# jie0530/act-plus-plus

Hardware: AMD Instinct MI355X
Metric: policy steps/sec (4x480x640 cams, chunk=100, bs=8) (higher is better)
Workload: dtype f32 (f16x3 split products: 3 fp16 MFMAs per fp32 product, fp32 accumulate); 1 GPU; ACT eval policy query: 4 cams 480x640 u8, chunk 100, hidden 512, ff 3200, 4 enc + 7 dec layers (layer 0 live), per-GPU batch 8, + temporal ensemble; per_gpu_batch=8, global_batch=8, parallelism=replicas x1

## Files before the change

act-plus-plus_amd/actmi/lib.py:

```python
import ctypes as C
import os

import torch

_HERE = os.path.dirname(os.path.abspath(__file__))
LIB_PATH = os.environ.get("ACTMI_LIB") or os.path.join(_HERE, "libactmi.so")

IMG_U8_NHWC = 0
IMG_F32_NCHW = 1


class ActmiConfig(C.Structure):
    _fields_ = [("struct_size", C.c_uint32)] + [(n, C.c_int32) for n in (
        "num_cams", "image_h", "image_w", "base_width", "hidden_dim", "nheads", "dim_feedforward", "enc_layers",
        "dec_layers", "num_queries", "state_dim", "action_dim", "latent_dim", "has_cvae_encoder", "max_batch",
        "enable_training")] + [("kl_weight", C.c_float)] + [(n, C.c_int32) for n in ("vq", "vq_class", "vq_dim")]


class GemmDesc(C.Structure):
    _fields_ = [
        ("A", C.c_void_p), ("lda", C.c_int64), ("mode", C.c_int32),
        ("H", C.c_int32), ("W", C.c_int32), ("Cin", C.c_int32), ("KH", C.c_int32), ("KW", C.c_int32),
        ("stride", C.c_int32), ("pad", C.c_int32), ("Ho", C.c_int32), ("Wo", C.c_int32),
        ("img_stride", C.c_int64),
        ("A_add", C.c_void_p), ("ld_add", C.c_int64), ("add_mod", C.c_int32), ("add_ncols", C.c_int32),
        ("Bw", C.c_void_p), ("ldb", C.c_int64),
        ("scale", C.c_void_p), ("bias", C.c_void_p), ("res", C.c_void_p), ("ldres", C.c_int64),
        ("res_mod", C.c_int32), ("relu", C.c_int32),
        ("C", C.c_void_p), ("ldc", C.c_int64), ("rowmap", C.c_void_p),
        ("M", C.c_int32), ("N", C.c_int32), ("K", C.c_int32), ("groups", C.c_int32),
        ("gA", C.c_int64), ("gB", C.c_int64), ("gSB", C.c_int64), ("gC", C.c_int64), ("gRes", C.c_int64),
        ("ta", C.c_int32), ("tb", C.c_int32), ("a_rowmap", C.c_void_p),
        ("B_add", C.c_void_p), ("ld_badd", C.c_int64), ("badd_mod", C.c_int32), ("splitk", C.c_int32),
        ("mask", C.c_void_p), ("ldmask", C.c_int64), ("C2", C.c_void_p), ("scale2", C.c_void_p),
        ("alpha", C.c_float), ("groups_inner", C.c_int32),
        ("gA2", C.c_int64), ("gB2", C.c_int64), ("gC2", C.c_int64), ("gRes2", C.c_int64),
        ("gMask", C.c_int64), ("gC2out", C.c_int64),
        ("drop_p", C.c_float), ("drop_seed", C.c_uint64), ("stamps", C.c_void_p), ("prec", C.c_int32), ("b_split", C.c_int32), ("b_scale", C.c_float), ("a_scale", C.c_float), ("a_scale_dev", C.c_void_p), ("b_scale_dev", C.c_void_p),
        ("split_stride", C.c_int64), ("amax_out", C.c_void_p),
        ("epi", C.c_int32), ("epi_scale", C.c_float), ("epi_row", C.c_void_p), ("gRow", C.c_int64), ("gRow2", C.c_int64),
        ("epi_colkill", C.c_void_p), ("gColkill", C.c_int64), ("tile_hint", C.c_int32),
        ("finite_flag", C.c_void_p), ("finite_bit", C.c_uint32),
        ("Ax", C.c_void_p), ("kx_begin", C.c_int32), ("Hx", C.c_int32), ("Wx", C.c_int32), ("Cx", C.c_int32),
        ("stride_x", C.c_int32), ("gAx", C.c_int64),
        ("A_alt", C.c_void_p), ("alt_ncols", C.c_int32), ("k_tap_inner", C.c_int32),
    ]


class AttnBwdDesc(C.Structure):
    _fields_ = [("q", C.c_void_p), ("k", C.c_void_p), ("v", C.c_void_p), ("o", C.c_void_p), ("d_o", C.c_void_p), ("lse", C.c_void_p),
                ("dq", C.c_void_p), ("dk", C.c_void_p), ("dv", C.c_void_p)] + \
               [(n, C.c_int64) for n in ("q_bs", "q_rs", "k_bs", "k_rs", "v_bs", "v_rs", "dq_bs", "dq_rs", "dk_bs", "dk_rs", "dv_bs", "dv_rs")] + \
               [("kpm", C.c_void_p), ("kpm_bs", C.c_int64)] + [(n, C.c_int32) for n in ("B", "H", "Nq", "Nk", "HD")] + \
               [("drop_p", C.c_float), ("drop_seed", C.c_uint64), ("delta_ws", C.c_void_p), ("do_scale", C.c_void_p), ("amax_out", C.c_void_p)]


class AttnDesc(C.Structure):
    _fields_ = [
        ("Q", C.c_void_p), ("q_bs", C.c_int64), ("q_rs", C.c_int64),
        ("K", C.c_void_p), ("k_bs", C.c_int64), ("k_rs", C.c_int64),
        ("V", C.c_void_p), ("v_bs", C.c_int64), ("v_rs", C.c_int64),
        ("O", C.c_void_p), ("o_bs", C.c_int64), ("o_rs", C.c_int64),
        ("kpm", C.c_void_p), ("kpm_bs", C.c_int64), ("lse", C.c_void_p),
        ("B", C.c_int32), ("H", C.c_int32), ("Nq", C.c_int32), ("Nk", C.c_int32), ("HD", C.c_int32),
        ("scale", C.c_float), ("ws", C.c_void_p), ("ws_floats", C.c_int64),
        ("drop_p", C.c_float), ("drop_seed", C.c_uint64), ("prec", C.c_int32), ("causal", C.c_int32),
    ]


_lib = None


def load():
    global _lib
    if _lib is not None:
        return _lib
    if not os.path.isfile(LIB_PATH):
        raise RuntimeError(
            f"{LIB_PATH} is missing: build the HIP extension first (python -c 'import __graft_entry__ as g; g.build()' "
            "or make -C act-plus-plus_amd/csrc). There is no CPU fallback for the ACT path.")
    lib = C.CDLL(LIB_PATH)
    vp, i32, i64, f32, f64 = C.c_void_p, C.c_int32, C.c_int64, C.c_float, C.c_double
    sigs = {
        "actmi_version": ([], i32),
        "actmi_create": ([C.POINTER(ActmiConfig), C.POINTER(vp)], i32),
        "actmi_destroy": ([vp], i32),
        "actmi_last_error": ([vp], C.c_char_p),
        "actmi_num_params": ([vp], i32),
        "actmi_param_info": ([vp, i32, C.POINTER(C.c_char_p), C.POINTER(i64), C.POINTER(i32), C.POINTER(i32)], i32),
        "actmi_set_param": ([vp, C.c_char_p, vp, C.POINTER(i64), i32, i32], i32),
        "actmi_get_param": ([vp, C.c_char_p, vp, i64, i32], i32),
        "actmi_param_ptr": ([vp, C.c_char_p, C.POINTER(vp), C.POINTER(i64)], i32),
        "actmi_finalize": ([vp, vp], i32),
        "actmi_set_forward_phase": ([vp, i32], i32),
        "actmi_forward_infer_vq": ([vp, vp, vp, i32, i32, vp, vp, vp], i32),
        "actmi_forward_infer": ([vp, vp, vp, i32, i32, vp, vp], i32),
        "actmi_forward_train": ([vp, vp, vp, i32, vp, vp, vp, C.c_uint64, f32, i32, vp, vp, vp, vp, vp], i32),
        "actmi_backward": ([vp, f32, vp], i32),
        "actmi_zero_grad": ([vp, vp], i32),
        "actmi_adamw_step": ([vp, f32, f32, f32, f32, f32, f32, i64, vp], i32),
        "actmi_adamw_step_range": ([vp, f32, f32, f32, f32, f32, f32, i64, i64, i64, vp], i32),
        "actmi_refresh_weights": ([vp, vp], i32),
        "actmi_param_arena": ([vp, C.POINTER(vp), C.POINTER(i64)], i32),
        "actmi_grad_ptr": ([vp, C.c_char_p, C.POINTER(vp), C.POINTER(i64)], i32),
        "actmi_grad_arena": ([vp, C.POINTER(vp), C.POINTER(i64)], i32),
        "actmi_grad_phase_range": ([vp, i32, C.POINTER(i64), C.POINTER(i64)], i32),
        "actmi_wait_grad_phase": ([vp, i32, vp], i32),
        "actmi_ensemble_step": ([vp, vp, vp, f64, vp, vp, i32, i32, i32, vp], i32),
        "actmi_op_gemm": ([C.POINTER(GemmDesc), vp], i32),
        "actmi_op_split16": ([vp, vp, C.c_int64, C.c_float, vp], i32),
        "actmi_op_permute_conv_k": ([vp, vp, C.c_int64, i32, i32, i32, vp], i32),
        "actmi_op_sample_onehot": ([vp, i32, i32, C.c_float, C.c_uint64, vp, vp, vp], i32),
        "actmi_op_pow2_scale": ([vp, C.c_int64, i32, i32, vp, vp], i32),
        "actmi_op_splitk_combine": ([vp, i32, C.c_int64, C.c_int64, i32, i32, vp, vp, vp, C.c_int64, i32, vp, C.c_int64, vp], i32),
        "actmi_op_attention": ([C.POINTER(AttnDesc), vp], i32),
        "actmi_op_attention_bwd": ([C.POINTER(AttnBwdDesc), vp], i32),
        "actmi_op_layernorm": ([vp, vp, i32, vp, vp, vp, vp, vp, i32, i32, f32, vp], i32),
        "actmi_op_maxpool3x3s2": ([vp, vp, i32, i32, i32, i32, vp], i32),
        "actmi_op_conv1": ([vp, i32, vp, vp, vp, vp, vp, i32, i32, i32, i32, i32, i32, vp], i32),
        "actmi_op_conv1_workspace_floats": ([i32, i32], C.c_int64),
        "actmi_op_conv1_prepare": ([vp, vp, i32, i32, i32, vp], i32),
        "actmi_op_conv1_prepared": ([vp, vp, vp, vp, vp, i32, i32, i32, i32, i32, i32, vp], i32),
        "actmi_op_conv3x3_c64": ([vp, vp, C.c_float, vp, vp, vp, vp, i32, i32, i32, i32, i32, vp], i32),
        "actmi_op_wgrad7x7s2": ([vp, vp, vp, vp, C.c_int64, vp, i32, i32, i32, i32, vp], i32),
        "actmi_op_wgrad3x3_c64": ([vp, vp, vp, vp, C.c_int64, vp, i32, i32, i32, i32, vp], i32),
        "actmi_op_groupnorm": ([vp, vp, vp, vp, vp, vp, vp, i32, i32, i32, i32, f32, i32, i32, vp, C.c_int64, vp], i32),
        "actmi_op_spatial_softmax": ([vp, vp, i32, i32, i32, i32, f32, vp], i32),
        "actmi_op_unfold1d": ([vp, vp, i32, i32, i32, i32, i32, i32, i32, i32, vp], i32),
        "actmi_op_ddim_step": ([vp, vp, C.c_int64, f32, f32, f32, f32, i32, vp], i32),
        "actmi_op_mish": ([vp, vp, C.c_int64, vp], i32),
        "actmi_op_gelu": ([vp, vp, C.c_int64, vp], i32),
        "actmi_op_gelu_bwd": ([vp, vp, vp, C.c_int64, vp], i32),
        "actmi_op_dropout": ([vp, vp, C.c_int64, C.c_float, C.c_uint64, vp], i32),
        "actmi_op_small_attention": ([vp, vp, i32, i32, i32, i32, i32, C.c_float, C.c_uint64, vp], i32),
        "actmi_op_small_attention_bwd": ([vp, vp, vp, i32, i32, i32, i32, i32, C.c_float, C.c_uint64, vp], i32),
        "actmi_op_soft_ce_dim1": ([vp, vp, i32, i32, i32, vp, vp, vp, vp], i32),
        "actmi_op_argmax_l1": ([vp, vp, i32, i32, vp, vp, vp], i32),
        "actmi_op_layernorm_bwd": ([vp, vp, vp, vp, vp, vp, vp, i32, i32, C.c_float, vp, C.c_int64, vp], i32),
        "actmi_op_colsum": ([vp, C.c_int64, vp, i32, i32, vp, C.c_int64, vp], i32),
        "actmi_op_sum_batch": ([vp, C.c_int64, C.c_int64, vp, i32, i32, i32, i32, vp], i32),
        "actmi_op_adamw": ([vp, vp, vp, vp, C.c_int64, C.c_float, C.c_float, C.c_float, C.c_float, C.c_float, C.c_int64, vp], i32),
        "actmi_op_u8_to_nhwc4": ([vp, vp, i32, i32, i32, i32, vp], i32),
        "actmi_op_last_error": ([], C.c_char_p),
        "actmi_debug_tensor": ([vp, C.c_char_p, C.POINTER(vp), C.POINTER(i64)], i32),
        "actmi_debug_stop_after": ([vp, C.c_char_p], i32),
        "actmi_set_gemm_prec": ([vp, i32], i32),
        "actmi_set_train_prec": ([vp, i32], i32),
        "actmi_get_flags": ([vp, C.POINTER(C.c_uint32), i32, vp], i32),
        "actmi_flags_ptr": ([vp, C.POINTER(vp)], i32),
        "actmi_profile_enable": ([i32], i32),
        "actmi_profile_reset": ([], i32),
        "actmi_profile_report": ([C.c_char_p, i32], i32),
    }
    for name, (args, res) in sigs.items():
        fn = getattr(lib, name)
        fn.argtypes = args
        fn.restype = res
    _lib = lib
    return lib


def declared_symbols(header_path):
    import re
    txt = open(header_path).read()
    return sorted(set(re.findall(r"\b(actmi_[a-z0-9_]+)\s*\(", txt)))


def current_stream_ptr():
    return C.c_void_p(torch.cuda.current_stream().cuda_stream)


def check(rc, handle=None, what=""):
    if rc != 0:
        lib = load()
        msg = lib.actmi_last_error(handle) if handle is not None else lib.actmi_op_last_error()
        raise RuntimeError(f"libactmi {what} failed (code {rc}): {msg.decode() if msg else ''}")


def profile_enable(on: bool):
    lib = load()
    lib.actmi_profile_reset() if on else None
    lib.actmi_profile_enable(1 if on else 0)


def profile_report():
    import json
    lib = load()
    buf = C.create_string_buffer(1 << 18)
    rc = lib.actmi_profile_report(buf, len(buf))
    if rc != 0:
        raise RuntimeError(f"actmi_profile_report failed ({rc})")
    return json.loads(buf.value.decode())
```

act-plus-plus_amd/actmi/ops.py:

```python
import ctypes as C

import torch

from . import lib as L


def _p(t):
    return C.c_void_p(t.data_ptr()) if t is not None else C.c_void_p(0)


PREC = {None: 0, "f32": 1, "f16x3": 2, "bf16": 3}


def split16(w, scale=1.0):
    lib = L.load()
    w = w.contiguous()
    out = torch.empty_like(w)
    L.check(lib.actmi_op_split16(_p(w), _p(out), w.numel(), float(scale), L.current_stream_ptr()), None, "op_split16")
    return out


def permute_conv_k(w_rows, taps, cin):
    lib = L.load()
    w_rows = w_rows.contiguous()
    out = torch.empty_like(w_rows)
    rows, ld = w_rows.numel() // w_rows.shape[-1], w_rows.shape[-1]
    L.check(lib.actmi_op_permute_conv_k(_p(w_rows), _p(out), rows, int(taps), int(cin), int(ld), L.current_stream_ptr()), None,
            "op_permute_conv_k")
    return out


def pow2_scale(x):
    lib = L.load()
    assert x.dim() == 2 and x.stride(1) == 1
    out = torch.zeros(2, dtype=torch.float32, device=x.device)
    L.check(lib.actmi_op_pow2_scale(_p(x), x.stride(0), x.shape[0], x.shape[1], _p(out), L.current_stream_ptr()), None,
            "op_pow2_scale")
    return out


def auto_splitk(M, N, K):
    tiles = ((M + 63) // 64) * ((N + 63) // 64)
    nk = (K + 31) // 32
    if tiles >= 768 or nk < 24:
        return 0
    s = min(8, (1536 + tiles - 1) // tiles, nk // 12)
    while s >= 2 and (s - 1) * ((nk + s - 1) // s) >= nk:
        s -= 1
    return s if s >= 2 else 0


def gemm(A, W, bias=None, scale=None, res=None, res_mod=0, relu=False, a_add=None, add_mod=0, add_ncols=0, rowmap=None,
         out=None, out_rows=None, drop_p=0.0, drop_seed=0, prec=None, w_split=False, a_scale=0.0, b_scale=0.0,
         a_scale_dev=None, b_scale_dev=None, splitk=0):
    lib = L.load()
    M, K = A.shape
    N = W.shape[0]
    if splitk == "auto":
        splitk = auto_splitk(M, N, K) if (rowmap is None and not res_mod and not drop_p and N % 4 == 0 and a_scale_dev is None
                                          and b_scale_dev is None) else 0
    if splitk and splitk > 1:
        assert rowmap is None and not res_mod and not drop_p
        part = torch.empty((splitk, M, N), dtype=torch.float32, device=A.device)
        d = L.GemmDesc()
        d.A, d.lda, d.mode = A.data_ptr(), A.stride(0), 0
        if a_add is not None:
            d.A_add, d.ld_add, d.add_mod, d.add_ncols = a_add.data_ptr(), a_add.stride(0), add_mod, add_ncols
        d.Bw, d.ldb = W.data_ptr(), W.stride(0)
        d.C, d.ldc = part.data_ptr(), N
        d.M, d.N, d.K, d.groups = M, N, K, 1
        d.splitk, d.split_stride = int(splitk), M * N
        d.prec, d.b_split, d.b_scale = PREC[prec], 1 if w_split else 0, float(w_split) if w_split else float(b_scale)
        d.a_scale = float(a_scale)
        L.check(lib.actmi_op_gemm(C.byref(d), L.current_stream_ptr()), None, "op_gemm")
        if out is None:
            out = torch.empty((M, N), dtype=torch.float32, device=A.device)
        L.check(lib.actmi_op_splitk_combine(part.data_ptr(), int(splitk), M * N, N, M, N, _p(scale), _p(bias), _p(res),
                                            res.stride(0) if res is not None else 0,
                                            2 if relu == "gelu" else (1 if relu else 0), out.data_ptr(), out.stride(0),
                                            L.current_stream_ptr()), None, "op_splitk_combine")
        return out
    if out is None:
        out = torch.zeros((out_rows or M, N), dtype=torch.float32, device=A.device)
    d = L.GemmDesc()
    d.A, d.lda, d.mode = A.data_ptr(), A.stride(0), 0
    if a_add is not None:
        d.A_add, d.ld_add, d.add_mod, d.add_ncols = a_add.data_ptr(), a_add.stride(0), add_mod, add_ncols
    d.Bw, d.ldb = W.data_ptr(), W.stride(0)
    d.scale = scale.data_ptr() if scale is not None else None
    d.bias = bias.data_ptr() if bias is not None else None
    if res is not None:
        d.res, d.ldres, d.res_mod = res.data_ptr(), res.stride(0), res_mod
    d.relu = 2 if relu == "gelu" else (1 if relu else 0)
    d.C, d.ldc = out.data_ptr(), out.stride(0)
    d.rowmap = rowmap.data_ptr() if rowmap is not None else None
    d.M, d.N, d.K, d.groups = M, N, K, 1
    d.drop_p, d.drop_seed = float(drop_p), int(drop_seed)
    d.prec, d.b_split, d.b_scale = PREC[prec], 1 if w_split else 0, float(w_split) if w_split else float(b_scale)
    d.a_scale = float(a_scale)
    d.a_scale_dev = a_scale_dev.data_ptr() if a_scale_dev is not None else None
    d.b_scale_dev = b_scale_dev.data_ptr() if b_scale_dev is not None else None
    L.check(lib.actmi_op_gemm(C.byref(d), L.current_stream_ptr()), None, "op_gemm")
    return out


def conv2d_with_second_source(y1, x, wf_split, w_scale, bias, stride_x=2, relu=True, splitk=0, k_tap_inner=False):
    lib = L.load()
    G, B, H, W, Cc = y1.shape
    _, _, Hx, Wx, Cx = x.shape
    Cout = wf_split.shape[1]
    Kf = 9 * Cc + Cx
    assert wf_split.numel() == G * Cout * Kf
    M = B * H * W

    def desc(C_ptr, ldc, gC):
        d = L.GemmDesc()
        d.A, d.mode = y1.data_ptr(), 1
        d.H, d.W, d.Cin, d.KH, d.KW, d.stride, d.pad, d.Ho, d.Wo = H, W, Cc, 3, 3, 1, 1, H, W
        d.img_stride = H * W * Cc
        d.Ax, d.kx_begin, d.Hx, d.Wx, d.Cx, d.stride_x, d.gAx = x.data_ptr(), 9 * Cc, Hx, Wx, Cx, stride_x, B * Hx * Wx * Cx
        d.Bw, d.ldb = wf_split.data_ptr(), Kf
        d.C, d.ldc = C_ptr, ldc
        d.M, d.N, d.K, d.groups = M, Cout, Kf, G
        d.gA, d.gB, d.gSB, d.gC = B * H * W * Cc, Cout * Kf, Cout, gC
        d.prec, d.b_split, d.b_scale = PREC["f16x3"], 1, float(w_scale)
        d.k_tap_inner = 1 if k_tap_inner else 0
        return d
    out = torch.empty((G, B, H, W, Cout), dtype=torch.float32, device=y1.device)
    if splitk and splitk > 1:
        part = torch.empty((G, splitk, M, Cout), dtype=torch.float32, device=y1.device)
        d = desc(part.data_ptr(), Cout, splitk * M * Cout)
        d.splitk, d.split_stride = int(splitk), M * Cout
        L.check(lib.actmi_op_gemm(C.byref(d), L.current_stream_ptr()), None, "op_gemm(conv + second source, split)")
        for g in range(G):
            L.check(lib.actmi_op_splitk_combine(part[g].data_ptr(), int(splitk), M * Cout, Cout, M, Cout, None, _p(bias[g]), None, 0,
                                                1 if relu else 0, out[g].data_ptr(), Cout, L.current_stream_ptr()), None, "combine")
        return out
    d = desc(out.data_ptr(), Cout, M * Cout)
    d.bias = bias.data_ptr()
    d.relu = 1 if relu else 0
    L.check(lib.actmi_op_gemm(C.byref(d), L.current_stream_ptr()), None, "op_gemm(conv + second source)")
    return out


def conv2d_nhwc(x, w_ohwi, scale=None, bias=None, res=None, relu=False, stride=1, pad=1, prec=None, w_split=False, b_scale=0.0,
                k_tap_inner=False):
    lib = L.load()
    G, B, H, W, Cin = x.shape
    _, Cout, KH, KW, _ = w_ohwi.shape
    Ho, Wo = (H + 2 * pad - KH) // stride + 1, (W + 2 * pad - KW) // stride + 1
    out = torch.empty((G, B, Ho, Wo, Cout), dtype=torch.float32, device=x.device)
    d = L.GemmDesc()
    d.A, d.mode = x.data_ptr(), 1
    d.H, d.W, d.Cin, d.KH, d.KW, d.stride, d.pad, d.Ho, d.Wo = H, W, Cin, KH, KW, stride, pad, Ho, Wo
    d.img_stride = H * W * Cin
    d.Bw, d.ldb = w_ohwi.data_ptr(), KH * KW * Cin
    d.scale = scale.data_ptr() if scale is not None else None
    d.bias = bias.data_ptr() if bias is not None else None
    if res is not None:
        d.res, d.ldres = res.data_ptr(), Cout
    d.relu = 1 if relu else 0
    d.C, d.ldc = out.data_ptr(), Cout
    d.M, d.N, d.K, d.groups = B * Ho * Wo, Cout, KH * KW * Cin, G
    d.gA, d.gB, d.gSB = B * H * W * Cin, Cout * KH * KW * Cin, Cout
    d.gC = d.gRes = B * Ho * Wo * Cout
    d.prec, d.b_split, d.b_scale = PREC[prec], 1 if w_split else 0, float(w_split) if w_split else float(b_scale)
    d.k_tap_inner = 1 if k_tap_inner else 0
    L.check(lib.actmi_op_gemm(C.byref(d), L.current_stream_ptr()), None, "op_gemm(conv)")
    return out


def sample_onehot(logits, temperature=1.0, seed=0, want_probs=False):
    lib = L.load()
    logits = logits.contiguous()
    n, V = logits.shape
    code = torch.empty_like(logits)
    probs = torch.empty_like(logits) if want_probs else None
    L.check(lib.actmi_op_sample_onehot(_p(logits), n, V, float(temperature), C.c_uint64(int(seed)), _p(probs), _p(code),
                                       L.current_stream_ptr()), None, "op_sample_onehot")
    return (code, probs) if want_probs else code


def conv1_prepare(w_oihw, lut_mode=1):
    lib = L.load()
    w_oihw = w_oihw.contiguous()
    Cc, Cout = w_oihw.shape[0], w_oihw.shape[1]
    ws = torch.zeros(int(lib.actmi_op_conv1_workspace_floats(Cc, Cout)), dtype=torch.float32, device=w_oihw.device)
    L.check(lib.actmi_op_conv1_prepare(_p(w_oihw), _p(ws), Cc, Cout, int(lut_mode), L.current_stream_ptr()), None, "op_conv1_prepare")
    return ws


def conv1_prepared(image_u8, ws, Cout, relu=False, scale=None, bias=None):
    lib = L.load()
    image_u8 = image_u8.contiguous()
    B, Cc, H, W, _ = image_u8.shape
    out = torch.empty((Cc, B, (H - 1) // 2 + 1, (W - 1) // 2 + 1, Cout), dtype=torch.float32, device=image_u8.device)
    L.check(lib.actmi_op_conv1_prepared(_p(image_u8), _p(ws), _p(scale), _p(bias), _p(out), B, Cc, H, W, Cout, 1 if relu else 0,
                                        L.current_stream_ptr()), None, "op_conv1_prepared")
    return out


def conv3x3_c64(x, w_ohwi, scale=None, bias=None, res=None, relu=False, w_scale=256.0, w16=None):
    lib = L.load()
    G, B, H, W, Cin = x.shape
    assert Cin == 64 and tuple(w_ohwi.shape[1:]) == (64, 3, 3, 64)
    out = torch.empty_like(x)
    if w16 is None:
        w16 = split16(w_ohwi, w_scale)
    scale = scale if scale is not None else torch.ones(G, 64, device=x.device)
    bias = bias if bias is not None else torch.zeros(G, 64, device=x.device)
    L.check(lib.actmi_op_conv3x3_c64(_p(x.contiguous()), _p(w16), float(w_scale), _p(scale.contiguous()), _p(bias.contiguous()),
                                     _p(res), _p(out), G, B, H, W, 1 if relu else 0, L.current_stream_ptr()), None,
            "op_conv3x3_c64")
    return out


def wgrad3x3_c64(dy, x, dy_scale=None):
    G, B, H, W, Cc = x.shape
    assert Cc == 64 and dy.shape == x.shape
    nwg = max(1, min(256 // G, B * ((W + 31) // 32)))
    ws = torch.empty(G * nwg * 64 * 576, device=x.device, dtype=torch.float32)
    dw = torch.empty(G, 64, 3, 3, 64, device=x.device, dtype=torch.float32)
    lib = L.load()
    L.check(lib.actmi_op_wgrad3x3_c64(_p(dy.contiguous()), _p(x.contiguous()), _p(dw), _p(ws), ws.numel(),
                                      _p(dy_scale) if dy_scale is not None else None, G, B, H, W, L.current_stream_ptr()),
            None, "op_wgrad3x3_c64")
    return dw


def wgrad7x7s2(dy, x4, dy_scale=None):
    G, B, H, W, Cc = x4.shape
    Ho, Wo = (H - 1) // 2 + 1, (W - 1) // 2 + 1
    assert Cc == 4 and tuple(dy.shape) == (G, B, Ho, Wo, 64)
    nwg = max(1, min(512 // G, B * ((Wo + 31) // 32)))
    ws = torch.empty(G * nwg * 64 * 196, device=x4.device, dtype=torch.float32)
    dw = torch.empty(G, 64, 7, 7, 4, device=x4.device, dtype=torch.float32)
    lib = L.load()
    L.check(lib.actmi_op_wgrad7x7s2(_p(dy.contiguous()), _p(x4.contiguous()), _p(dw), _p(ws), ws.numel(),
                                    _p(dy_scale) if dy_scale is not None else None, G, B, H, W, L.current_stream_ptr()),
            None, "op_wgrad7x7s2")
    return dw



def attention(q, k, v, nheads, kpm=None, q_shared=False, want_lse=False, split=True, drop_p=0.0, drop_seed=0, prec=None,
              causal=False):
    lib = L.load()
    B, Nk, D = k.shape
    Nq = q.shape[-2]
    hd = D // nheads
    out = torch.zeros((B, Nq, D), dtype=torch.float32, device=k.device)
    lse = torch.zeros((B, nheads, Nq), dtype=torch.float32, device=k.device) if want_lse else None
    d = L.AttnDesc()
    d.Q, d.q_bs, d.q_rs = q.data_ptr(), (0 if q_shared else q.stride(0)), q.stride(-2)
    d.K, d.k_bs, d.k_rs = k.data_ptr(), k.stride(0), k.stride(1)
    d.V, d.v_bs, d.v_rs = v.data_ptr(), v.stride(0), v.stride(1)
    d.O, d.o_bs, d.o_rs = out.data_ptr(), out.stride(0), out.stride(1)
    if kpm is not None:
        d.kpm, d.kpm_bs = kpm.data_ptr(), kpm.stride(0)
    d.lse = lse.data_ptr() if lse is not None else None
    if split:
        ws = torch.empty(8 * B * Nq * (D + 2 * nheads), dtype=torch.float32, device=k.device)
        d.ws, d.ws_floats = ws.data_ptr(), ws.numel()
    d.B, d.H, d.Nq, d.Nk, d.HD = B, nheads, Nq, Nk, hd
    d.scale = 1.0 / (hd ** 0.5)
    d.drop_p, d.drop_seed = float(drop_p), int(drop_seed)
    d.prec = PREC[prec]
    d.causal = 1 if causal else 0
    L.check(lib.actmi_op_attention(C.byref(d), L.current_stream_ptr()), None, "op_attention")
    return (out, lse) if want_lse else out


def attention_bwd(q, k, v, out, lse, dout, nheads, kpm=None, drop_p=0.0, drop_seed=0, do_scale=None, want_amax=False):
    lib = L.load()
    B, Nk, D = k.shape
    Nq = q.shape[1]
    dq = torch.empty((B, Nq, D), dtype=torch.float32, device=k.device)
    dk = torch.empty((B, Nk, D), dtype=torch.float32, device=k.device)
    dv = torch.empty((B, Nk, D), dtype=torch.float32, device=k.device)
    ws = torch.empty(B * nheads * Nq, dtype=torch.float32, device=k.device)
    amax = torch.zeros(1, dtype=torch.int32, device=k.device) if want_amax else None
    d = L.AttnBwdDesc()
    d.q, d.q_bs, d.q_rs = q.data_ptr(), q.stride(0), q.stride(1)
    d.k, d.k_bs, d.k_rs = k.data_ptr(), k.stride(0), k.stride(1)
    d.v, d.v_bs, d.v_rs = v.data_ptr(), v.stride(0), v.stride(1)
    d.o, d.d_o, d.lse = out.data_ptr(), dout.data_ptr(), lse.data_ptr()
    d.dq, d.dq_bs, d.dq_rs = dq.data_ptr(), dq.stride(0), dq.stride(1)
    d.dk, d.dk_bs, d.dk_rs = dk.data_ptr(), dk.stride(0), dk.stride(1)
    d.dv, d.dv_bs, d.dv_rs = dv.data_ptr(), dv.stride(0), dv.stride(1)
    if kpm is not None:
        d.kpm, d.kpm_bs = kpm.data_ptr(), kpm.stride(0)
    d.B, d.H, d.Nq, d.Nk, d.HD = B, nheads, Nq, Nk, D // nheads
    d.drop_p, d.drop_seed = float(drop_p), int(drop_seed)
    d.delta_ws = ws.data_ptr()
    d.do_scale = do_scale.data_ptr() if do_scale is not None else None
    d.amax_out = amax.data_ptr() if amax is not None else None
    L.check(lib.actmi_op_attention_bwd(C.byref(d), L.current_stream_ptr()), None, "op_attention_bwd")
    return (dq, dk, dv, amax) if want_amax else (dq, dk, dv)


def layernorm(x, w, b, res=None, res_mod=0, w2=None, b2=None, eps=1e-5):
    lib = L.load()
    M, D = x.shape
    y = torch.empty_like(x)
    L.check(lib.actmi_op_layernorm(_p(x), _p(res), res_mod, _p(w), _p(b), _p(w2), _p(b2), _p(y), M, D, eps,
                                   L.current_stream_ptr()), None, "op_layernorm")
    return y


def maxpool3x3s2(x):
    lib = L.load()
    n, H, W, Cc = x.shape
    Ho, Wo = (H + 2 - 3) // 2 + 1, (W + 2 - 3) // 2 + 1
    y = torch.empty((n, Ho, Wo, Cc), dtype=torch.float32, device=x.device)
    L.check(lib.actmi_op_maxpool3x3s2(_p(x), _p(y), n, H, W, Cc, L.current_stream_ptr()), None, "op_maxpool")
    return y


def conv1(image, w_oihw, scale, bias, prec=None):
    lib = L.load()
    image = image.contiguous()
    if image.dtype == torch.uint8:
        B, Cn, H, W, _ = image.shape
        fmt = L.IMG_U8_NHWC
    else:
        B, Cn, _, H, W = image.shape
        fmt = L.IMG_F32_NCHW
    Cout = w_oihw.shape[1]
    Ho, Wo = (H + 6 - 7) // 2 + 1, (W + 6 - 7) // 2 + 1
    out = torch.zeros((Cn, B, Ho, Wo, Cout), dtype=torch.float32, device=image.device)
    ws = torch.empty(Cn * Cout * 148 + 768, dtype=torch.float32, device=image.device)
    L.check(lib.actmi_op_conv1(_p(image), fmt, _p(w_oihw), _p(scale), _p(bias), _p(out), _p(ws), B, Cn, H, W, Cout,
                               PREC[prec], L.current_stream_ptr()), None, "op_conv1")
    return out


ACT = {None: 0, "none": 0, "relu": 1, "mish": 2}


_GN_WS = {}


def groupnorm(x, weight, bias, groups, eps=1e-5, act=None, res=None, res_after=False, film=None, out=None):
    lib = L.load()
    x = x.contiguous()
    n, Cc = x.shape[0], x.shape[-1]
    P = x.numel() // (n * Cc)
    if out is None:
        out = torch.empty_like(x)
    assert out.is_contiguous() and out.shape == x.shape
    fs, fb = (film[0].contiguous(), film[1].contiguous()) if film is not None else (None, None)
    rm = 0 if res is None else (2 if res_after else 1)
    key = (x.device, torch.cuda.current_stream(x.device).cuda_stream)
    ws = _GN_WS.get(key)
    if ws is None:
        ws = _GN_WS[key] = torch.empty(1 << 20, dtype=torch.float32, device=x.device)
    L.check(lib.actmi_op_groupnorm(_p(x), _p(res.contiguous() if res is not None else None), _p(fs), _p(fb), _p(weight), _p(bias),
                                   _p(out), n, P, Cc, int(groups), float(eps), ACT[act], rm, _p(ws), ws.numel(),
                                   L.current_stream_ptr()), None, "op_groupnorm")
    return out


def spatial_softmax(logits, H, W, temperature=1.0):
    lib = L.load()
    logits = logits.contiguous()
    n, P, K = logits.shape
    assert P == H * W
    out = torch.empty((n, K, 2), dtype=torch.float32, device=logits.device)
    L.check(lib.actmi_op_spatial_softmax(_p(logits), _p(out), n, H, W, K, float(temperature), L.current_stream_ptr()), None,
            "op_spatial_softmax")
    return out


def unfold1d(x, k, stride=1, pad=0, transposed=False):
    lib = L.load()
    x = x.contiguous()
    B, T, Cc = x.shape
    To = (T - 1) * stride - 2 * pad + k if transposed else (T + 2 * pad - k) // stride + 1
    out = torch.empty((B, To, k * Cc), dtype=torch.float32, device=x.device)
    L.check(lib.actmi_op_unfold1d(_p(x), _p(out), B, T, Cc, k, stride, pad, To, 1 if transposed else 0, L.current_stream_ptr()),
            None, "op_unfold1d")
    return out


def ddim_step(x, eps, alpha_t, alpha_prev, clip=True):
    lib = L.load()
    assert x.is_contiguous() and eps.is_contiguous() and x.numel() == eps.numel()
    L.check(lib.actmi_op_ddim_step(_p(x), _p(eps), x.numel(), float(alpha_t ** -0.5), float((1.0 - alpha_t) ** 0.5),
                                   float(alpha_prev ** 0.5), float(max(0.0, 1.0 - alpha_prev) ** 0.5), 1 if clip else 0,
                                   L.current_stream_ptr()), None, "op_ddim_step")
    return x


def mish(x):
    lib = L.load()
    x = x.contiguous()
    y = torch.empty_like(x)
    L.check(lib.actmi_op_mish(_p(x), _p(y), x.numel(), L.current_stream_ptr()), None, "op_mish")
    return y


def u8_to_nhwc4(image_u8):
    lib = L.load()
    image_u8 = image_u8.contiguous()
    B, Cam, H, W, _ = image_u8.shape
    out = torch.empty((Cam, B, H, W, 4), dtype=torch.float32, device=image_u8.device)
    L.check(lib.actmi_op_u8_to_nhwc4(_p(image_u8), _p(out), B, Cam, H, W, L.current_stream_ptr()), None, "op_u8_to_nhwc4")
    return out


def gemm_t(A, Bm, ta=False, tb=False, bias=None, res=None, out=None, prec="f32"):
    lib = L.load()
    if ta:
        K, M = A.shape
    else:
        M, K = A.shape
    N = Bm.shape[1] if tb else Bm.shape[0]
    assert (Bm.shape[0] if tb else Bm.shape[1]) == K, (A.shape, Bm.shape, ta, tb)
    if out is None:
        out = torch.empty((M, N), dtype=torch.float32, device=A.device)
    d = L.GemmDesc()
    d.A, d.lda, d.mode, d.ta = A.data_ptr(), A.stride(0), 0, 1 if ta else 0
    d.Bw, d.ldb, d.tb = Bm.data_ptr(), Bm.stride(0), 1 if tb else 0
    d.bias = bias.data_ptr() if bias is not None else None
    if res is not None:
        d.res, d.ldres = res.data_ptr(), res.stride(0)
    d.C, d.ldc = out.data_ptr(), out.stride(0)
    d.M, d.N, d.K, d.groups = M, N, K, 1
    d.prec = PREC[prec]
    L.check(lib.actmi_op_gemm(C.byref(d), L.current_stream_ptr()), None, "op_gemm")
    return out


def gelu(x):
    y = torch.empty_like(x)
    L.check(L.load().actmi_op_gelu(_p(x), _p(y), x.numel(), L.current_stream_ptr()), None, "op_gelu")
    return y


def gelu_bwd(x, dy):
    dx = torch.empty_like(x)
    L.check(L.load().actmi_op_gelu_bwd(_p(x), _p(dy), _p(dx), x.numel(), L.current_stream_ptr()), None, "op_gelu_bwd")
    return dx


def dropout(x, p, seed):
    y = torch.empty_like(x)
    L.check(L.load().actmi_op_dropout(_p(x), _p(y), x.numel(), float(p), int(seed), L.current_stream_ptr()), None, "op_dropout")
    return y
# ... 87 lines not shown
```

act-plus-plus_amd/csrc/attn.hip:

```cpp
#include "common.h"
#include "dropout.h"
#include "split16.h"
#include <cstdio>
#include <cstdlib>

namespace {

constexpr bool ATTN_NOPF = true;
constexpr int KT = 64;
typedef _Float16 h16x8 __attribute__((ext_vector_type(8)));

__device__ __forceinline__ void attn_block_coords(int& bx, int& by, int& bz) {
    const int gx = gridDim.x, gy = gridDim.y;
    const int total = gx * gy * (int)gridDim.z;
    const int lin = ((int)blockIdx.z * gy + (int)blockIdx.y) * gx + (int)blockIdx.x;
    const int xcd = lin & 7, q = total >> 3, r = total & 7;
    const int base = (xcd < r) ? xcd * (q + 1) : r * (q + 1) + (xcd - r) * q;
    const int flat = base + (lin >> 3);
    bx = flat % gx;
    const int rest = flat / gx;
    by = rest % gy;
    bz = rest / gy;
}

template <int HD>
__global__ __launch_bounds__(256) void attn_f32_kernel(AttnArgs p, int nsplit, int chunk) {
    constexpr int HH = HD / 2;
    constexpr int DT = (HD + 31) / 32;
    constexpr int VD = DT * 32;
    constexpr int KS = HD + 4;
    __shared__ __attribute__((aligned(16))) float s_k[KT * KS];
    __shared__ __attribute__((aligned(16))) float s_v[KT * VD];

    const int t = threadIdx.x, lane = t & 63, wave = t >> 6;
    const int li = lane & 31, lh = lane >> 5;
    int bx, h, b;
    attn_block_coords(bx, h, b);
    const int split = bx % nsplit;
    const int q = (bx / nsplit) * 128 + wave * 32 + li;
    const int k_begin = split * chunk;
    const int k_end = (k_begin + chunk < p.Nk) ? k_begin + chunk : p.Nk;
    const bool qok = q < p.Nq;

    const float qscale = p.scale * 1.4426950408889634f;
    const float* Qp = p.Q + (int64_t)b * p.q_bs + (int64_t)(qok ? q : 0) * p.q_rs + h * HD + lh * HH;
    float qreg[HH];
#pragma unroll
    for (int s = 0; s < HH; s += 4) {
        f32x4 v = *reinterpret_cast<const f32x4*>(Qp + s);
#pragma unroll
        for (int j = 0; j < 4; ++j) qreg[s + j] = qok ? v[j] * qscale : 0.f;
    }
    const float* Kb = p.K + (int64_t)b * p.k_bs + h * HD;
    const float* Vb = p.V + (int64_t)b * p.v_bs + h * HD;
    const uint8_t* kpm = p.kpm ? p.kpm + (int64_t)b * p.kpm_bs : nullptr;

    f32x16 O[DT];
#pragma unroll
    for (int d = 0; d < DT; ++d)
#pragma unroll
        for (int e = 0; e < 16; ++e) O[d][e] = 0.f;
    float m_run = -INFINITY, l_run = 0.f;

    if (HD < VD) {
        for (int e = t; e < KT * VD; e += 256) s_v[e] = 0.f;
        __syncthreads();
    }

    __shared__ uint8_t s_dead[KT];
    constexpr int C4 = HD / 4;
    constexpr int NLD = (KT * C4 + 255) / 256;
    f32x4 pk[NLD], pv[NLD];
    auto fetch = [&](int kt0) {
#pragma unroll
        for (int i = 0; i < NLD; ++i) {
            const int e = t + 256 * i;
            const int kr = e / C4, c = e - kr * C4;
            const int key = kt0 + kr;
            const bool ok = e < KT * C4 && key < k_end;
            const int64_t koff = ok ? (int64_t)key * p.k_rs + c * 4 : 0;
            const int64_t voff = ok ? (int64_t)key * p.v_rs + c * 4 : 0;
            const f32x4 kv = *reinterpret_cast<const f32x4*>(Kb + koff);
            const f32x4 vv = *reinterpret_cast<const f32x4*>(Vb + voff);
            const f32x4 z = {0.f, 0.f, 0.f, 0.f};
            pk[i] = ok ? kv : z;
            pv[i] = ok ? vv : z;
        }
    };
    fetch(k_begin);
    for (int kt0 = k_begin; kt0 < k_end; kt0 += KT) {
#pragma unroll
        for (int i = 0; i < NLD; ++i) {
            const int e = t + 256 * i;
            if (e < KT * C4) {
                const int kr = e / C4, c = e - kr * C4;
                *reinterpret_cast<f32x4*>(&s_k[kr * KS + c * 4]) = pk[i];
                *reinterpret_cast<f32x4*>(&s_v[kr * VD + c * 4]) = pv[i];
            }
        }
        const bool ragged = kt0 + KT > k_end || kpm != nullptr;
        if (ragged && t < KT) {
            const int key = kt0 + t;
            s_dead[t] = (key >= k_end) || (kpm && kpm[key] != 0);
        }
        __syncthreads();
        if (kt0 + KT < k_end) fetch(kt0 + KT);
#pragma unroll
        for (int sub = 0; sub < KT / 32; ++sub) {
            const int kb = kt0 + sub * 32;
            if (kb < k_end) {
                f32x16 S;
#pragma unroll
                for (int e = 0; e < 16; ++e) S[e] = 0.f;
                const float* krow = &s_k[(sub * 32 + li) * KS + lh * HH];
#pragma unroll
                for (int s = 0; s < HH; s += 4) {
                    const f32x4 kv = *reinterpret_cast<const f32x4*>(krow + s);
#pragma unroll
                    for (int j = 0; j < 4; ++j)
                        S = __builtin_amdgcn_mfma_f32_32x32x2f32(kv[j], qreg[s + j], S, 0, 0, 0);
                }
                if (ragged) {
#pragma unroll
                    for (int e = 0; e < 16; ++e)
                        if (s_dead[sub * 32 + (e & 3) + 8 * (e >> 2) + 4 * lh]) S[e] = -INFINITY;
                }
                if (p.causal) {
#pragma unroll
                    for (int e = 0; e < 16; ++e)
                        if (kb + (e & 3) + 8 * (e >> 2) + 4 * lh > q) S[e] = -INFINITY;
                }
                float mt = S[0];
#pragma unroll
                for (int e = 1; e < 16; ++e) mt = fmaxf(mt, S[e]);
                mt = fmaxf(mt, __shfl_xor(mt, 32, 64));
                const float m_new = fmaxf(m_run, mt);
                const float m_safe = (m_new == -INFINITY) ? 0.f : m_new;
                const float alpha = __builtin_amdgcn_exp2f(m_run - m_safe);
                float rs = 0.f;
#pragma unroll
                for (int e = 0; e < 16; ++e) {
                    S[e] = __builtin_amdgcn_exp2f(S[e] - m_safe);
                    rs += S[e];
                }
                rs += __shfl_xor(rs, 32, 64);
                l_run = l_run * alpha + rs;
                m_run = m_new;
                if (p.drop_p > 0.f) {
                    const float ds = 1.f / (1.f - p.drop_p);
                    const uint64_t rowbase = (((uint64_t)b * p.H + h) * p.Nq + (qok ? q : 0)) * (uint64_t)p.Nk;
#pragma unroll
                    for (int e = 0; e < 16; ++e) {
                        const int key = kb + (e & 3) + 8 * (e >> 2) + 4 * lh;
                        S[e] = actmi_keep(p.drop_seed, rowbase + key, p.drop_p) ? S[e] * ds : 0.f;
                    }
                }
#pragma unroll
                for (int d = 0; d < DT; ++d)
#pragma unroll
                    for (int e = 0; e < 16; ++e) O[d][e] *= alpha;
#pragma unroll
                for (int e = 0; e < 16; ++e) {
                    const int kl = sub * 32 + (e & 3) + 8 * (e >> 2) + 4 * lh;
#pragma unroll
                    for (int d = 0; d < DT; ++d) {
                        const float vv = s_v[kl * VD + d * 32 + li];
                        O[d] = __builtin_amdgcn_mfma_f32_32x32x2f32(vv, S[e], O[d], 0, 0, 0);
                    }
                }
            }
        }
        __syncthreads();
    }
    if (qok) {
        if (nsplit == 1) {
            const float inv = 1.f / l_run;
            float* Op = p.O + (int64_t)b * p.o_bs + (int64_t)q * p.o_rs + h * HD;
#pragma unroll
            for (int d = 0; d < DT; ++d)
#pragma unroll
                for (int g = 0; g < 4; ++g) {
                    const int d0 = d * 32 + 8 * g + 4 * lh;
                    if (d0 < HD) {
                        f32x4 o = {O[d][4 * g] * inv, O[d][4 * g + 1] * inv, O[d][4 * g + 2] * inv, O[d][4 * g + 3] * inv};
                        *reinterpret_cast<f32x4*>(Op + d0) = o;
                    }
                }
            if (p.lse && lh == 0) p.lse[((int64_t)b * p.H + h) * p.Nq + q] = m_run * 0.6931471805599453f + logf(l_run);
        } else {
            const int64_t row = (((int64_t)split * p.B + b) * p.H + h) * p.Nq + q;
            float* Op = p.ws + row * HD;
            float* ml = p.ws + (int64_t)nsplit * p.B * p.H * p.Nq * HD + row * 2;
#pragma unroll
            for (int d = 0; d < DT; ++d)
#pragma unroll
                for (int g = 0; g < 4; ++g) {
                    const int d0 = d * 32 + 8 * g + 4 * lh;
                    if (d0 < HD) {
                        f32x4 o = {O[d][4 * g], O[d][4 * g + 1], O[d][4 * g + 2], O[d][4 * g + 3]};
                        *reinterpret_cast<f32x4*>(Op + d0) = o;
                    }
                }
            if (lh == 0) { ml[0] = m_run; ml[1] = l_run; }
        }
    }
}

template <int HD>
__global__ __launch_bounds__(256, 3) void attn_f16x3_kernel(AttnArgs p, int nsplit, int chunk) {
    constexpr int NS = HD / 16;
    constexpr int DT = (HD + 31) / 32;
    constexpr int VD = DT * 32;
    constexpr int KROW = 4 * HD + 16;
    constexpr int VROW = 4 * KT + 16;
    __shared__ __attribute__((aligned(16))) unsigned char s_k[KT * KROW];
    __shared__ __attribute__((aligned(16))) unsigned char s_vt[VD * VROW];
    __shared__ uint8_t s_dead[KT];

    const int t = threadIdx.x, lane = t & 63, wave = t >> 6;
    const int li = lane & 31, lh = lane >> 5;
    int bx, h, b;
    attn_block_coords(bx, h, b);
    const int split = bx % nsplit;
    const int q = (bx / nsplit) * 128 + wave * 32 + li;
    const int k_begin = split * chunk;
    const int k_end = (k_begin + chunk < p.Nk) ? k_begin + chunk : p.Nk;
    const bool qok = q < p.Nq;

    const float qscale = p.scale * 1.4426950408889634f;
    const float* Qp = p.Q + (int64_t)b * p.q_bs + (int64_t)(qok ? q : 0) * p.q_rs + h * HD + lh * 8;
    h16x8 qh[NS], ql[NS];
#pragma unroll
    for (int s = 0; s < NS; ++s) {
        f32x4 v0 = *reinterpret_cast<const f32x4*>(Qp + s * 16);
        f32x4 v1 = *reinterpret_cast<const f32x4*>(Qp + s * 16 + 4);
        const float sc = qok ? qscale : 0.f;
        v0 *= sc; v1 *= sc;
        uint2 h0, l0, h1, l1;
        split16(v0, h0, l0);
        split16(v1, h1, l1);
        qh[s] = __builtin_bit_cast(h16x8, uint4{h0.x, h0.y, h1.x, h1.y});
        ql[s] = __builtin_bit_cast(h16x8, uint4{l0.x, l0.y, l1.x, l1.y});
    }
    const float* Kb = p.K + (int64_t)b * p.k_bs + h * HD;
    const float* Vb = p.V + (int64_t)b * p.v_bs + h * HD;
    const uint8_t* kpm = p.kpm ? p.kpm + (int64_t)b * p.kpm_bs : nullptr;

    f32x16 O[DT];
#pragma unroll
    for (int d = 0; d < DT; ++d)
#pragma unroll
        for (int e = 0; e < 16; ++e) O[d][e] = 0.f;
    float m_run = -INFINITY, l_run = 0.f;

    if (HD < VD) {
        for (int e = t; e < VD * VROW / 4; e += 256) reinterpret_cast<uint32_t*>(s_vt)[e] = 0u;
        __syncthreads();
    }

    constexpr int C4 = HD / 4;
    constexpr int NLK = (KT * C4 + 255) / 256;
    constexpr int NLV = (KT / 2 * C4 + 255) / 256;
    f32x4 pk[NLK], pv[NLV][2];
    auto vc = [&](int e) { return ((e >> 5) % (C4 / 4)) * 4 + (e & 3); };
    auto vkp = [&](int e) { return ((e >> 5) / (C4 / 4)) * 8 + ((e >> 2) & 7); };
    auto fetch = [&](int kt0) {
        const f32x4 z = {0.f, 0.f, 0.f, 0.f};
#pragma unroll
        for (int i = 0; i < NLK; ++i) {
            const int e = t + 256 * i;
            const int kr = e / C4, c = e - kr * C4;
            const int key = kt0 + kr;
            const bool ok = e < KT * C4 && key < k_end;
            const f32x4 kv = *reinterpret_cast<const f32x4*>(Kb + (ok ? (int64_t)key * p.k_rs + c * 4 : 0));
            pk[i] = ok ? kv : z;
        }
#pragma unroll
        for (int i = 0; i < NLV; ++i) {
            const int e = t + 256 * i;
            const int kp = vkp(e), c = vc(e);
#pragma unroll
            for (int u = 0; u < 2; ++u) {
                const int key = kt0 + 2 * kp + u;
                const bool ok = e < KT / 2 * C4 && key < k_end;
                const f32x4 vv = *reinterpret_cast<const f32x4*>(Vb + (ok ? (int64_t)key * p.v_rs + c * 4 : 0));
                pv[i][u] = ok ? vv : z;
            }
        }
    };
    if (!ATTN_NOPF) fetch(k_begin);
    for (int kt0 = k_begin; kt0 < k_end; kt0 += KT) {
        if (ATTN_NOPF) fetch(kt0);
#pragma unroll
        for (int i = 0; i < NLK; ++i) {
            const int e = t + 256 * i;
            if (e < KT * C4) {
                const int kr = e / C4, c = e - kr * C4;
                uint2 hi, lo;
                split16(pk[i], hi, lo);
                *reinterpret_cast<uint2*>(s_k + kr * KROW + c * 8) = hi;
                *reinterpret_cast<uint2*>(s_k + kr * KROW + 2 * HD + c * 8) = lo;
            }
        }
#pragma unroll
        for (int i = 0; i < NLV; ++i) {
            const int e = t + 256 * i;
            if (e < KT / 2 * C4) {
                const int kp = vkp(e), c = vc(e);
                uint2 ha, la, hb, lb;
                split16(pv[i][0], ha, la);
                split16(pv[i][1], hb, lb);
                const int kl = 2 * kp, r = kl & 15;
                const int pos = (kl & ~15) | (r & 3) | ((r & 8) >> 1) | ((r & 4) << 1);
                unsigned char* dst = s_vt + (c * 4) * VROW + pos * 2;
                *reinterpret_cast<uint32_t*>(dst + 0 * VROW) = (ha.x & 0xffffu) | (hb.x << 16);
                *reinterpret_cast<uint32_t*>(dst + 1 * VROW) = (ha.x >> 16) | (hb.x & 0xffff0000u);
                *reinterpret_cast<uint32_t*>(dst + 2 * VROW) = (ha.y & 0xffffu) | (hb.y << 16);
                *reinterpret_cast<uint32_t*>(dst + 3 * VROW) = (ha.y >> 16) | (hb.y & 0xffff0000u);
                *reinterpret_cast<uint32_t*>(dst + 0 * VROW + 2 * KT) = (la.x & 0xffffu) | (lb.x << 16);
                *reinterpret_cast<uint32_t*>(dst + 1 * VROW + 2 * KT) = (la.x >> 16) | (lb.x & 0xffff0000u);
                *reinterpret_cast<uint32_t*>(dst + 2 * VROW + 2 * KT) = (la.y & 0xffffu) | (lb.y << 16);
                *reinterpret_cast<uint32_t*>(dst + 3 * VROW + 2 * KT) = (la.y >> 16) | (lb.y & 0xffff0000u);
            }
        }
        const bool ragged = kt0 + KT > k_end || kpm != nullptr;
        if (ragged && t < KT) {
            const int key = kt0 + t;
            s_dead[t] = (key >= k_end) || (kpm && kpm[key] != 0);
        }
        __syncthreads();
        if (!ATTN_NOPF && kt0 + KT < k_end) fetch(kt0 + KT);
#pragma unroll
        for (int sub = 0; sub < KT / 32; ++sub) {
            const int kb = kt0 + sub * 32;
            if (kb < k_end) {
                f32x16 S;
#pragma unroll
                for (int e = 0; e < 16; ++e) S[e] = 0.f;
                const unsigned char* krow = s_k + (sub * 32 + li) * KROW + lh * 16;
#pragma unroll
                for (int s = 0; s < NS; ++s) {
                    const h16x8 kh = __builtin_bit_cast(h16x8, *reinterpret_cast<const f32x4*>(krow + s * 32));
                    const h16x8 kl = __builtin_bit_cast(h16x8, *reinterpret_cast<const f32x4*>(krow + 2 * HD + s * 32));
                    S = __builtin_amdgcn_mfma_f32_32x32x16_f16(kl, qh[s], S, 0, 0, 0);
                    S = __builtin_amdgcn_mfma_f32_32x32x16_f16(kh, ql[s], S, 0, 0, 0);
                    S = __builtin_amdgcn_mfma_f32_32x32x16_f16(kh, qh[s], S, 0, 0, 0);
                }
                if (ragged) {
#pragma unroll
                    for (int e = 0; e < 16; ++e)
                        if (s_dead[sub * 32 + (e & 3) + 8 * (e >> 2) + 4 * lh]) S[e] = -INFINITY;
                }
                if (p.causal) {
#pragma unroll
                    for (int e = 0; e < 16; ++e)
                        if (kb + (e & 3) + 8 * (e >> 2) + 4 * lh > q) S[e] = -INFINITY;
                }
                float mt = S[0];
#pragma unroll
                for (int e = 1; e < 16; ++e) mt = fmaxf(mt, S[e]);
                mt = fmaxf(mt, __shfl_xor(mt, 32, 64));
                const float m_new = fmaxf(m_run, mt);
                const float m_safe = (m_new == -INFINITY) ? 0.f : m_new;
                const float alpha = __builtin_amdgcn_exp2f(m_run - m_safe);
                float rs = 0.f;
#pragma unroll
                for (int e = 0; e < 16; ++e) {
                    S[e] = __builtin_amdgcn_exp2f(S[e] - m_safe);
                    rs += S[e];
                }
                rs += __shfl_xor(rs, 32, 64);
                l_run = l_run * alpha + rs;
                m_run = m_new;
                if (p.drop_p > 0.f) {
                    const float ds = 1.f / (1.f - p.drop_p);
                    const uint64_t rowbase = (((uint64_t)b * p.H + h) * p.Nq + (qok ? q : 0)) * (uint64_t)p.Nk;
#pragma unroll
                    for (int e = 0; e < 16; ++e) {
                        const int key = kb + (e & 3) + 8 * (e >> 2) + 4 * lh;
                        S[e] = actmi_keep(p.drop_seed, rowbase + key, p.drop_p) ? S[e] * ds : 0.f;
                    }
                }
                h16x8 ph[2], pl[2];
#pragma unroll
                for (int g2 = 0; g2 < 2; ++g2) {
                    const f32x4 a0 = {S[8 * g2], S[8 * g2 + 1], S[8 * g2 + 2], S[8 * g2 + 3]};
                    const f32x4 a1 = {S[8 * g2 + 4], S[8 * g2 + 5], S[8 * g2 + 6], S[8 * g2 + 7]};
                    uint2 h0, l0, h1, l1;
                    split16(a0, h0, l0);
                    split16(a1, h1, l1);
                    ph[g2] = __builtin_bit_cast(h16x8, uint4{h0.x, h0.y, h1.x, h1.y});
                    pl[g2] = __builtin_bit_cast(h16x8, uint4{l0.x, l0.y, l1.x, l1.y});
                }
#pragma unroll
                for (int d = 0; d < DT; ++d) {
#pragma unroll
                    for (int e = 0; e < 16; ++e) O[d][e] *= alpha;
                    const unsigned char* vrow = s_vt + (d * 32 + li) * VROW + sub * 64 + lh * 16;
#pragma unroll
                    for (int g2 = 0; g2 < 2; ++g2) {
                        const h16x8 vh = __builtin_bit_cast(h16x8, *reinterpret_cast<const f32x4*>(vrow + g2 * 32));
                        const h16x8 vl = __builtin_bit_cast(h16x8, *reinterpret_cast<const f32x4*>(vrow + 2 * KT + g2 * 32));
                        O[d] = __builtin_amdgcn_mfma_f32_32x32x16_f16(vl, ph[g2], O[d], 0, 0, 0);
                        O[d] = __builtin_amdgcn_mfma_f32_32x32x16_f16(vh, pl[g2], O[d], 0, 0, 0);
                        O[d] = __builtin_amdgcn_mfma_f32_32x32x16_f16(vh, ph[g2], O[d], 0, 0, 0);
                    }
                }
            }
        }
        __syncthreads();
    }
    if (qok) {
        if (nsplit == 1) {
            const float inv = 1.f / l_run;
            float* Op = p.O + (int64_t)b * p.o_bs + (int64_t)q * p.o_rs + h * HD;
#pragma unroll
            for (int d = 0; d < DT; ++d)
#pragma unroll
                for (int g = 0; g < 4; ++g) {
                    const int d0 = d * 32 + 8 * g + 4 * lh;
                    if (d0 < HD) {
                        f32x4 o = {O[d][4 * g] * inv, O[d][4 * g + 1] * inv, O[d][4 * g + 2] * inv, O[d][4 * g + 3] * inv};
                        *reinterpret_cast<f32x4*>(Op + d0) = o;
                    }
                }
            if (p.lse && lh == 0) p.lse[((int64_t)b * p.H + h) * p.Nq + q] = m_run * 0.6931471805599453f + logf(l_run);
        } else {
            const int64_t row = (((int64_t)split * p.B + b) * p.H + h) * p.Nq + q;
            float* Op = p.ws + row * HD;
            float* ml = p.ws + (int64_t)nsplit * p.B * p.H * p.Nq * HD + row * 2;
#pragma unroll
            for (int d = 0; d < DT; ++d)
#pragma unroll
                for (int g = 0; g < 4; ++g) {
                    const int d0 = d * 32 + 8 * g + 4 * lh;
                    if (d0 < HD) {
                        f32x4 o = {O[d][4 * g], O[d][4 * g + 1], O[d][4 * g + 2], O[d][4 * g + 3]};
                        *reinterpret_cast<f32x4*>(Op + d0) = o;
                    }
                }
            if (lh == 0) { ml[0] = m_run; ml[1] = l_run; }
        }
    }
}


__global__ void attn_combine_kernel(AttnArgs p, int nsplit, int HD) {
    const int64_t idx = (int64_t)blockIdx.x * blockDim.x + threadIdx.x;
    const int D4 = HD / 4;
    const int64_t total = (int64_t)p.B * p.H * p.Nq * D4;
    if (idx >= total) return;
    const int d4 = (int)(idx % D4);
    const int64_t bhq = idx / D4;
    const int q = (int)(bhq % p.Nq);
    const int h = (int)((bhq / p.Nq) % p.H);
    const int b = (int)(bhq / ((int64_t)p.Nq * p.H));
    const int64_t per = (int64_t)p.B * p.H * p.Nq;
    const float* mlb = p.ws + (int64_t)nsplit * per * HD;
    float m = -INFINITY;
    for (int s = 0; s < nsplit; ++s) m = fmaxf(m, mlb[(s * per + bhq) * 2]);
    const float msafe = (m == -INFINITY) ? 0.f : m;
    float L = 0.f;
    f32x4 acc = {0.f, 0.f, 0.f, 0.f};
    for (int s = 0; s < nsplit; ++s) {
        const float w = __builtin_amdgcn_exp2f(mlb[(s * per + bhq) * 2] - msafe);
        L += mlb[(s * per + bhq) * 2 + 1] * w;
        acc += *reinterpret_cast<const f32x4*>(p.ws + (s * per + bhq) * HD + d4 * 4) * w;
    }
    const float inv = 1.f / L;
    *reinterpret_cast<f32x4*>(p.O + (int64_t)b * p.o_bs + (int64_t)q * p.o_rs + h * HD + d4 * 4) = acc * inv;
    if (p.lse && d4 == 0) p.lse[bhq] = msafe * 0.6931471805599453f + logf(L);
}

}

int launch_attention(const AttnArgs& a, hipStream_t st, std::string* err) {
    auto fail = [&](const char* m) { if (err) *err = std::string("attention: ") + m; return -2; };
    if (a.B <= 0 || a.Nq <= 0) return 0;
    if (a.Nk <= 0) return fail("Nk must be positive");
    if (a.causal && a.Nq != a.Nk) return fail("causal needs Nq == Nk");
    if ((a.q_rs & 3) || (a.k_rs & 3) || (a.v_rs & 3) || (a.o_rs & 3) || (a.q_bs & 3) || (a.k_bs & 3) || (a.v_bs & 3) ||
        (a.o_bs & 3))
        return fail("strides must be multiples of 4 floats");
    if (((uintptr_t)a.Q & 15) || ((uintptr_t)a.K & 15) || ((uintptr_t)a.V & 15) || ((uintptr_t)a.O & 15))
        return fail("pointers must be 16-byte aligned");
    static const int env_prec = env_gemm_prec(ACTMI_PREC_F32);
    const int prec = a.prec ? a.prec : env_prec;
    if (prec != ACTMI_PREC_F32 && prec != ACTMI_PREC_F16X3) return fail("bad prec");
    const bool f16 = prec == ACTMI_PREC_F16X3;
    const int qblocks = (a.Nq + 127) / 128;
    const int tiles = (a.Nk + KT - 1) / KT;
    int nsplit = 1;
    if (a.ws) {
        const long blocks = (long)qblocks * a.H * a.B;
        static const long target = getenv("ACTMI_ATTN_SPLIT_TARGET") ? atol(getenv("ACTMI_ATTN_SPLIT_TARGET")) : 1024;
        nsplit = (int)((target + blocks - 1) / blocks);
        if (nsplit < 1) nsplit = 1;
        if (nsplit > 8) nsplit = 8;
        if (nsplit > tiles / 2) nsplit = tiles / 2 > 0 ? tiles / 2 : 1;
        while (nsplit > 1 && (int64_t)nsplit * a.B * a.Nq * ((int64_t)a.H * a.HD + 2 * a.H) > a.ws_floats) --nsplit;
    }
    const int chunk = ((tiles + nsplit - 1) / nsplit) * KT;
    dim3 grid(qblocks * nsplit, a.H, a.B);
    if (prof_enabled()) {
        char nm[48];
        snprintf(nm, sizeof(nm), "attn_%s_kernel<%d>", f16 ? "f16x3" : "f32", a.HD);
        prof_begin(nm, 4.0 * a.B * a.H * (double)a.Nq * a.Nk * a.HD,
                   4.0 * a.B * a.H * a.HD * (2.0 * a.Nq + 2.0 * a.Nk), st);
    }
    if (f16) {
        switch (a.HD) {
            case 64: hipLaunchKernelGGL(attn_f16x3_kernel<64>, grid, dim3(256), 0, st, a, nsplit, chunk); break;
            case 32: hipLaunchKernelGGL(attn_f16x3_kernel<32>, grid, dim3(256), 0, st, a, nsplit, chunk); break;
            case 16: hipLaunchKernelGGL(attn_f16x3_kernel<16>, grid, dim3(256), 0, st, a, nsplit, chunk); break;
            default: return fail("head_dim must be 16, 32 or 64");
        }
    } else
    switch (a.HD) {
        case 64: hipLaunchKernelGGL(attn_f32_kernel<64>, grid, dim3(256), 0, st, a, nsplit, chunk); break;
        case 32: hipLaunchKernelGGL(attn_f32_kernel<32>, grid, dim3(256), 0, st, a, nsplit, chunk); break;
        case 16: hipLaunchKernelGGL(attn_f32_kernel<16>, grid, dim3(256), 0, st, a, nsplit, chunk); break;
        default: return fail("head_dim must be 16, 32 or 64");
    }
    if (nsplit > 1) {
        const int64_t total = (int64_t)a.B * a.H * a.Nq * (a.HD / 4);
        hipLaunchKernelGGL(attn_combine_kernel, dim3((unsigned)((total + 255) / 256)), dim3(256), 0, st, a, nsplit, a.HD);
    }
    prof_end(st);
    hipError_t e = hipGetLastError();
    if (e != hipSuccess) { if (err) *err = std::string("attention launch: ") + hipGetErrorString(e); return -3; }
    return 0;
}
```

act-plus-plus_amd/csrc/capi.hip:

```cpp
#include "engine.h"

#include <cstring>
#include <vector>

namespace {
thread_local std::string g_op_error;
inline hipStream_t S(void* s) { return reinterpret_cast<hipStream_t>(s); }
int bad(actmi_ctx* h, const std::string& m, int code = ACTMI_E_INVALID) { h->err = m; return code; }
struct DevGuard {
    int prev = -1, want;
    explicit DevGuard(int dev) : want(dev) {
        if (hipGetDevice(&prev) != hipSuccess) prev = -1;
        if (prev != want) (void)hipSetDevice(want);
    }
    ~DevGuard() { if (prev >= 0 && prev != want) (void)hipSetDevice(prev); }
};
#define ENTER(h) (h)->err.clear(); DevGuard _dev_guard((h)->device)
}

extern "C" {

int actmi_version(void) { return ACTMI_VERSION; }

int actmi_create(const actmi_config* cfg, actmi_handle* out) {
// ... 96 lines not shown
    if (!h->cfg.vq) return bad(h, "handle was not created with vq = 1");
    return engine_forward_infer(h, qpos, image, image_fmt, B, a_hat, S(stream), vq_sample);
}

int actmi_forward_train(actmi_handle h, const float* qpos, const void* image, int image_fmt, const float* actions,
                        const uint8_t* is_pad, const float* eps, uint64_t dropout_seed, float dropout_p, int B, float* losses,
                        float* a_hat, float* mu, float* logvar, void* stream) {
    if (!h) return ACTMI_E_INVALID;
    ENTER(h);
    if (!qpos || !image || !actions || !is_pad) return bad(h, "null pointer");
    return train_forward(h, qpos, image, image_fmt, actions, is_pad, eps, dropout_seed, dropout_p, B, losses, a_hat, mu, logvar,
                         S(stream));
}
int actmi_backward(actmi_handle h, float loss_scale, void* stream) {
    if (!h) return ACTMI_E_INVALID;
    ENTER(h);
    return train_backward(h, loss_scale, S(stream));
}
int actmi_zero_grad(actmi_handle h, void* stream) {
    if (!h) return ACTMI_E_INVALID;
    ENTER(h);
    return train_zero_grad(h, S(stream));
}
int actmi_adamw_step(actmi_handle h, float lr, float lr_backbone, float weight_decay, float beta1, float beta2, float eps,
                     int64_t step, void* stream) {
    if (!h) return ACTMI_E_INVALID;
    ENTER(h);
    return train_adamw_step(h, lr, lr_backbone, weight_decay, beta1, beta2, eps, step, S(stream));
}
int actmi_adamw_step_range(actmi_handle h, float lr, float lr_backbone, float weight_decay, float beta1, float beta2, float eps,
                           int64_t step, int64_t offset, int64_t count, void* stream) {
    if (!h) return ACTMI_E_INVALID;
    ENTER(h);
    return train_adamw_range(h, lr, lr_backbone, weight_decay, beta1, beta2, eps, step, offset, count, S(stream));
}
int actmi_refresh_weights(actmi_handle h, void* stream) {
    if (!h) return ACTMI_E_INVALID;
    ENTER(h);
    if (!h->finalized) return bad(h, "refresh_weights before finalize", ACTMI_E_STATE);
    return engine_prepare_weights(h, S(stream), true);
}
int actmi_param_arena(actmi_handle h, void** dev_ptr, int64_t* nfloats) {
    if (!h) return ACTMI_E_INVALID;
    if (dev_ptr) *dev_ptr = h->pbase;
    if (nfloats) *nfloats = h->ptotal;
    return 0;
}
int actmi_grad_ptr(actmi_handle h, const char* key, void** dev_ptr, int64_t* numel) {
    if (!h || !key) return ACTMI_E_INVALID;
    ENTER(h);
    if (!h->train) return bad(h, "handle was created without enable_training", ACTMI_E_STATE);
    auto it = h->index.find(key);
    if (it == h->index.end()) return bad(h, std::string("unknown state_dict key: ") + key);
    const Param& p = h->params[it->second];
    if (dev_ptr) *dev_ptr = h->train->gbase + p.off;
    if (numel) *numel = p.numel;
    return 0;
}

int actmi_grad_arena(actmi_handle h, void** dev_ptr, int64_t* nfloats) {
    if (!h) return ACTMI_E_INVALID;
    ENTER(h);
    if (!h->train) return bad(h, "handle was created without enable_training", ACTMI_E_STATE);
    if (dev_ptr) *dev_ptr = h->train->gbase;
    if (nfloats) *nfloats = h->ptotal;
    return 0;
}

int actmi_grad_phase_range(actmi_handle h, int phase, int64_t* offset, int64_t* count) {
    if (!h || !offset || !count || (phase != 1 && phase != 2)) return ACTMI_E_INVALID;
    ENTER(h);
    if (!h->train) return bad(h, "handle was created without enable_training", ACTMI_E_STATE);
    int64_t split = h->ptotal;
    for (const Param& p : h->params)
        if (p.key != "pos_table" && p.key.rfind("transformer.", 0) != 0) { split = p.off; break; }
    *offset = phase == 1 ? 0 : split;
    *count = phase == 1 ? split : h->ptotal - split;
    return 0;
}

int actmi_wait_grad_phase(actmi_handle h, int phase, void* stream) {
    if (!h || phase != 1) return ACTMI_E_INVALID;
    ENTER(h);
    if (!h->train || !h->train->ev_phase1) return bad(h, "handle was created without enable_training", ACTMI_E_STATE);
    hipError_t e = hipStreamWaitEvent(S(stream), h->train->ev_phase1, 0);
    if (e != hipSuccess) return bad(h, std::string("hipStreamWaitEvent: ") + hipGetErrorString(e), ACTMI_E_LAUNCH);
    return 0;
}

int actmi_ensemble_step(float* ring, int32_t* tcount, const float* chunk, double k, double* out, uint8_t* populated, int E,
                        int Q, int A, void* stream) {
    if (!ring || !tcount || !chunk || !out || Q < 1 || A < 1 || A > 64) return ACTMI_E_INVALID;
    return launch_ensemble(ring, tcount, chunk, k, out, populated, E, Q, A, S(stream));
}

int actmi_op_gemm(const actmi_gemm_desc* d, void* stream) {
    if (!d) return ACTMI_E_INVALID;
    g_op_error.clear();
    return launch_gemm(*d, S(stream), &g_op_error);
}

int actmi_op_split16(const float* src, float* dst, int64_t nfloats, float scale, void* stream) {
    g_op_error.clear();
    const int rc = launch_split16(src, dst, nfloats, scale, S(stream));
    if (rc != 0) g_op_error = "split16: nfloats must be a multiple of 4 and both pointers 16-byte aligned";
    return rc == 0 ? 0 : ACTMI_E_INVALID;
}

int actmi_op_permute_conv_k(const float* src, float* dst, int64_t rows, int taps, int cin, int ld, void* stream) {
    g_op_error.clear();
    const int rc = launch_permute_conv_k(src, dst, rows, taps, cin, ld, S(stream));
    if (rc != 0) g_op_error = "permute_conv_k: cin must be a multiple of 32, ld >= taps*cin, src != dst";
    return rc == 0 ? 0 : (rc == -2 ? ACTMI_E_INVALID : ACTMI_E_LAUNCH);
}




int actmi_op_pow2_scale(const float* x, int64_t ld, int M, int N, float* out, void* stream) {
    g_op_error.clear();
    return launch_pow2_scale(x, ld, M, N, out, S(stream)) == 0 ? 0 : ACTMI_E_LAUNCH;
}

int actmi_op_splitk_combine(const float* part, int nsplit, int64_t split_stride, int64_t ldp, int M, int N, const float* scale,
                            const float* bias, const float* res, int64_t ldres, int relu, float* out, int64_t ldc, void* stream) {
    g_op_error.clear();
    if (!part || !out || nsplit < 1 || M < 0 || N < 0 || ldp < N || ldc < N || (res && ldres < N) || relu < 0 || relu > 2) {
        g_op_error = "splitk_combine: bad argument";
        return ACTMI_E_INVALID;
    }
    SplitCombineArgs c{};
    c.part = part; c.nsplit = nsplit; c.split_stride = split_stride; c.ldp = ldp;
    c.scale = scale; c.bias = bias; c.res = res; c.ldres = ldres; c.relu = relu;
    c.C = out; c.ldc = ldc; c.M = M; c.N = N; c.groups = 1;
    return launch_splitk_combine(c, S(stream)) == 0 ? 0 : ACTMI_E_LAUNCH;
}

int actmi_op_sample_onehot(const float* logits, int n, int V, float temperature, uint64_t seed, float* probs, float* code,
                           void* stream) {
    g_op_error.clear();
    if (!logits || !code || n < 1 || V < 1 || !(temperature > 0.f)) { g_op_error = "sample_onehot: bad argument"; return ACTMI_E_INVALID; }
    return launch_vq_code(logits, nullptr, seed, probs, code, n, 1, V, S(stream), temperature) == 0 ? 0 : ACTMI_E_LAUNCH;
}

int actmi_op_attention(const actmi_attn_desc* d, void* stream) {
    if (!d) return ACTMI_E_INVALID;
    g_op_error.clear();
    return launch_attention(*d, S(stream), &g_op_error);
}

int actmi_op_attention_bwd(const actmi_attn_bwd_desc* d, void* stream) {
    g_op_error.clear();
    if (!d || !d->o || !d->delta_ws) { g_op_error = "attention_bwd: null descriptor / output / scratch"; return ACTMI_E_INVALID; }
    AttnBwdArgs a{};
    a.Q = d->q; a.K = d->k; a.V = d->v; a.dO = d->d_o; a.lse = d->lse; a.dO_scale = d->do_scale;
    a.dQ = d->dq; a.dK = d->dk; a.dV = d->dv;
    a.q_bs = d->q_bs; a.q_rs = d->q_rs; a.k_bs = d->k_bs; a.k_rs = d->k_rs; a.v_bs = d->v_bs; a.v_rs = d->v_rs;
    a.dq_bs = d->dq_bs; a.dq_rs = d->dq_rs; a.dk_bs = d->dk_bs; a.dk_rs = d->dk_rs; a.dv_bs = d->dv_bs; a.dv_rs = d->dv_rs;
    a.kpm = d->kpm; a.kpm_bs = d->kpm_bs;
    a.B = d->B; a.H = d->H; a.Nq = d->Nq; a.Nk = d->Nk; a.HD = d->HD;
    a.drop_p = d->drop_p; a.drop_seed = d->drop_seed; a.amax_out = d->amax_out;
    const int rc = launch_attention_bwd_dense(a, d->o, d->delta_ws, S(stream), &g_op_error);
    return rc == 0 ? ACTMI_OK : (rc == -2 ? ACTMI_E_SHAPE : ACTMI_E_LAUNCH);
}

int actmi_op_layernorm(const float* x, const float* res, int res_mod, const float* w, const float* b, const float* w2,
                       const float* b2, float* y, int M, int D, float eps, void* stream) {
    g_op_error.clear();
    return launch_layernorm(x, res, res_mod, w, b, w2, b2, y, M, D, eps, S(stream), &g_op_error);
}

int actmi_op_maxpool3x3s2(const float* in, float* out, int nimg, int H, int W, int C, void* stream) {
    return launch_maxpool(in, out, nimg, H, W, C, (H + 2 - 3) / 2 + 1, (W + 2 - 3) / 2 + 1, S(stream));
}

int actmi_op_conv1(const void* image, int image_fmt, const float* w_oihw, const float* scale, const float* bias,
                   float* out, float* workspace, int B, int C, int H, int W, int Cout, int prec, void* stream) {
    g_op_error.clear();
    float* wp = workspace;
    float* lut = workspace + (int64_t)C * Cout * 148;
    int rc = launch_repack_conv_w(w_oihw, wp, C, Cout, 3, 7, 7, (int64_t)Cout * 147, (int64_t)Cout * 148, 148, S(stream));
    if (rc) return rc;
    float hl[768];
    u8_lut(hl, true);
    if (hipMemcpyAsync(lut, hl, sizeof(hl), hipMemcpyHostToDevice, S(stream)) != hipSuccess) return ACTMI_E_LAUNCH;
    if (hipStreamSynchronize(S(stream)) != hipSuccess) return ACTMI_E_LAUNCH;
    Conv1Args a;
    a.image = image; a.fmt = image_fmt; a.lut = lut; a.w = wp; a.scale = scale; a.bias = bias; a.out = out;
    a.B = B; a.C = C; a.H = H; a.W = W; a.Ho = (H + 6 - 7) / 2 + 1; a.Wo = (W + 6 - 7) / 2 + 1; a.Cout = Cout;
    a.prec = prec;
    return launch_conv1(a, S(stream), &g_op_error);
}

static int64_t conv1_ws_off_lut(int C, int Cout) { return (int64_t)C * Cout * 148; }
int64_t actmi_op_conv1_workspace_floats(int C, int Cout) {
    return conv1_ws_off_lut(C, Cout) + 768 + 2 * (int64_t)C * Cout + (int64_t)C * ((conv1_wimg_bytes() + 3) / 4) + 16;
}
int actmi_op_conv1_prepare(const float* w_oihw, float* workspace, int C, int Cout, int lut_mode, void* stream) {
    g_op_error.clear();
    if (!w_oihw || !workspace || C < 1 || Cout < 1 || Cout > 64) { g_op_error = "conv1_prepare: bad argument"; return ACTMI_E_INVALID; }
    float* lut = workspace + conv1_ws_off_lut(C, Cout);
    float* ones = lut + 768;
    float* zeros = ones + (int64_t)C * Cout;
    float* wimg = zeros + (int64_t)C * Cout;
    wimg = reinterpret_cast<float*>((reinterpret_cast<uintptr_t>(wimg) + 15) & ~(uintptr_t)15);
    int rc = launch_repack_conv_w(w_oihw, workspace, C, Cout, 3, 7, 7, (int64_t)Cout * 147, (int64_t)Cout * 148, 148, S(stream));
    if (rc) return ACTMI_E_LAUNCH;
    std::vector<float> host(768 + 2 * (size_t)C * Cout);
    u8_lut(host.data(), lut_mode == 0);
    for (int i = 0; i < C * Cout; ++i) { host[768 + i] = 1.f; host[768 + C * Cout + i] = 0.f; }
    if (hipMemcpyAsync(lut, host.data(), host.size() * sizeof(float), hipMemcpyHostToDevice, S(stream)) != hipSuccess) return ACTMI_E_LAUNCH;
    rc = launch_conv1_wimg(workspace, wimg, C, Cout, S(stream), 256.f);
    if (rc) return ACTMI_E_LAUNCH;
    if (hipStreamSynchronize(S(stream)) != hipSuccess) return ACTMI_E_LAUNCH;
    return 0;
}
int actmi_op_conv1_prepared(const void* image_u8, const float* workspace, const float* scale, const float* bias, float* out, int B,
                            int C, int H, int W, int Cout, int relu, void* stream) {
    g_op_error.clear();
    if (!image_u8 || !workspace || !out) { g_op_error = "conv1_prepared: null pointer"; return ACTMI_E_INVALID; }
    const float* lut = workspace + conv1_ws_off_lut(C, Cout);
    const float* ones = lut + 768;
    const float* zeros = ones + (int64_t)C * Cout;
    const float* wimg = zeros + (int64_t)C * Cout;
    wimg = reinterpret_cast<const float*>((reinterpret_cast<uintptr_t>(wimg) + 15) & ~(uintptr_t)15);
    Conv1Args a;
    a.image = image_u8; a.fmt = ACTMI_IMG_U8_NHWC; a.lut = lut; a.w = workspace; a.scale = scale ? scale : ones; a.bias = bias ? bias : zeros;
    a.out = out; a.B = B; a.C = C; a.H = H; a.W = W; a.Ho = (H + 6 - 7) / 2 + 1; a.Wo = (W + 6 - 7) / 2 + 1; a.Cout = Cout;
    a.prec = ACTMI_PREC_F16X3; a.wimg = reinterpret_cast<const unsigned char*>(wimg); a.wscale = 256.f;
    a.relu_floor = relu ? 0.f : -__builtin_inff();
    return launch_conv1(a, S(stream), &g_op_error);
}

int actmi_op_conv3x3_c64(const float* x, const float* w16, float w_scale, const float* scale, const float* bias,
                         const float* res, float* out, int G, int B, int H, int W, int relu, void* stream) {
    g_op_error.clear();
    Conv3Args a;
    a.x = x; a.w16 = w16; a.scale = scale; a.bias = bias; a.res = res; a.out = out;
    a.G = G; a.B = B; a.H = H; a.W = W; a.relu = relu; a.w_scale = w_scale;
    return launch_conv3x3_c64(a, S(stream), &g_op_error);
}


int actmi_op_wgrad3x3_c64(const float* dy, const float* x, float* dw, float* ws, int64_t ws_floats, const float* dy_scale_dev, int G,
                          int B, int H, int W, void* stream) {
    g_op_error.clear();
    const int rc = launch_wgrad3x3_c64(dy, x, dw, 0, ws, ws_floats, dy_scale_dev, G, B, H, W, S(stream));
    if (rc != 0) { g_op_error = "wgrad3x3_c64: bad arguments or launch failure"; return rc == -2 ? ACTMI_E_INVALID : ACTMI_E_LAUNCH; }
    return 0;
}

int actmi_op_wgrad7x7s2(const float* dy, const float* x4, float* dw, float* ws, int64_t ws_floats, const float* dy_scale_dev, int G,
                        int B, int H, int W, void* stream) {
    g_op_error.clear();
    const int Ho = (H - 1) / 2 + 1, Wo = (W - 1) / 2 + 1;
    const int rc = launch_wgrad7x7s2(dy, x4, dw, 0, ws, ws_floats, dy_scale_dev, G, B, H, W, Ho, Wo, S(stream));
    if (rc != 0) { g_op_error = "wgrad7x7s2: bad arguments or launch failure"; return rc == -2 ? ACTMI_E_INVALID : ACTMI_E_LAUNCH; }
    return 0;
}

const char* actmi_op_last_error(void) { return g_op_error.c_str(); }

int actmi_set_gemm_prec(actmi_handle h, int prec) {
    if (!h) return ACTMI_E_INVALID;
    ENTER(h);
    if (prec != ACTMI_PREC_F32 && prec != ACTMI_PREC_F16X3) { h->err = "prec must be ACTMI_PREC_F32 or ACTMI_PREC_F16X3"; return ACTMI_E_INVALID; }
    h->gemm_prec = prec;
    h->finalized = false;
    return 0;
}

int actmi_set_train_prec(actmi_handle h, int prec) {
    if (!h) return ACTMI_E_INVALID;
    ENTER(h);
    if (prec != 0 && prec != ACTMI_PREC_BF16 && prec != ACTMI_PREC_F16X3 && prec != ACTMI_PREC_F32) { h->err = "train prec must be 0 or ACTMI_PREC_*"; return ACTMI_E_INVALID; }
    h->train_prec = (prec == h->gemm_prec) ? 0 : prec;
    if (h->train_prec != 0 && h->train_prec != ACTMI_PREC_BF16) { h->err = "only ACTMI_PREC_BF16 differs from the handle precision"; h->train_prec = 0; return ACTMI_E_INVALID; }
    return 0;
}

int actmi_get_flags(actmi_handle h, uint32_t* host_flags, int clear, void* stream) {
    if (!h || !host_flags) return ACTMI_E_INVALID;
    ENTER(h);
    hipError_t e = hipMemcpyAsync(host_flags, h->flags, sizeof(uint32_t), hipMemcpyDeviceToHost, S(stream));
    if (e == hipSuccess) e = hipStreamSynchronize(S(stream));
    if (e == hipSuccess && clear && *host_flags) e = hipMemsetAsync(h->flags, 0, sizeof(uint32_t), S(stream));
    if (e != hipSuccess) return bad(h, std::string("get_flags: ") + hipGetErrorString(e), ACTMI_E_LAUNCH);
    return 0;
}

int actmi_flags_ptr(actmi_handle h, void** dev_ptr) {
    if (!h || !dev_ptr) return ACTMI_E_INVALID;
    *dev_ptr = h->flags;
    return 0;
}

int actmi_debug_stop_after(actmi_handle h, const char* stage) {
    if (!h) return ACTMI_E_INVALID;
    h->stop_stage = stage ? stage : "";
    return 0;
}

int actmi_debug_tensor(actmi_handle h, const char* name, const float** dev_ptr, int64_t* numel) {
    if (!h || !name) return ACTMI_E_INVALID;
    ENTER(h);
    auto it = h->dbg.find(name);
// ... 66 lines not shown
```

act-plus-plus_amd/csrc/engine.hip:

```cpp
#include "engine.h"

#include <algorithm>
#include <cmath>
#include <cstdio>
#include <cstring>

namespace {

thread_local std::string g_create_error;

int conv_out(int x, int k, int s, int p) { return (x + 2 * p - k) / s + 1; }

void add_param(actmi_ctx* c, const std::string& key, std::vector<int64_t> shape, bool is_buffer) {
    Param p;
    p.key = key;
    p.shape = shape;
    p.numel = 1;
    for (auto d : shape) p.numel *= d;
    p.off = c->ptotal;
    p.is_buffer = is_buffer;
    c->ptotal += (p.numel + 63) & ~int64_t(63);
    c->index[key] = (int)c->params.size();
    c->params.push_back(p);
}

void add_mha(actmi_ctx* c, const std::string& p, int D) {
    add_param(c, p + "in_proj_weight", {3 * D, D}, false);
    add_param(c, p + "in_proj_bias", {3 * D}, false);
    add_param(c, p + "out_proj.weight", {D, D}, false);
    add_param(c, p + "out_proj.bias", {D}, false);
}

void add_ffn_norms(actmi_ctx* c, const std::string& p, int D, int F, int nnorm) {
    add_param(c, p + "linear1.weight", {F, D}, false);
    add_param(c, p + "linear1.bias", {F}, false);
    add_param(c, p + "linear2.weight", {D, F}, false);
    add_param(c, p + "linear2.bias", {D}, false);
    for (int i = 1; i <= nnorm; ++i) {
        add_param(c, p + "norm" + std::to_string(i) + ".weight", {D}, false);
        add_param(c, p + "norm" + std::to_string(i) + ".bias", {D}, false);
    }
}

void add_fbn(actmi_ctx* c, const std::string& p, int n) {
    for (const char* s : {"weight", "bias", "running_mean", "running_var"}) add_param(c, p + s, {n}, true);
}

void build_spec(actmi_ctx* c) {
    const actmi_config& g = c->cfg;
    const int D = g.hidden_dim, F = g.dim_feedforward, Q = g.num_queries, S = g.state_dim, A = g.action_dim,
              L = g.latent_dim, w0 = g.base_width;
    add_param(c, "pos_table", {1, Q + 2, D}, true);
    for (int i = 0; i < g.enc_layers; ++i) {
        std::string p = "transformer.encoder.layers." + std::to_string(i) + ".";
        add_mha(c, p + "self_attn.", D);
        add_ffn_norms(c, p, D, F, 2);
    }
    for (int i = 0; i < g.dec_layers; ++i) {
        std::string p = "transformer.decoder.layers." + std::to_string(i) + ".";
        add_mha(c, p + "self_attn.", D);
        add_mha(c, p + "multihead_attn.", D);
        add_ffn_norms(c, p, D, F, 3);
    }
    add_param(c, "transformer.decoder.norm.weight", {D}, false);
    add_param(c, "transformer.decoder.norm.bias", {D}, false);
    if (g.has_cvae_encoder) {
        for (int i = 0; i < g.enc_layers; ++i) {
            std::string p = "encoder.layers." + std::to_string(i) + ".";
            add_mha(c, p + "self_attn.", D);
            add_ffn_norms(c, p, D, F, 2);
        }
    }
    add_param(c, "action_head.weight", {A, D}, false);
    add_param(c, "action_head.bias", {A}, false);
    add_param(c, "is_pad_head.weight", {1, D}, false);
    add_param(c, "is_pad_head.bias", {1}, false);
    add_param(c, "query_embed.weight", {Q, D}, false);
    add_param(c, "input_proj.weight", {D, 8 * w0, 1, 1}, false);
    add_param(c, "input_proj.bias", {D}, false);
    for (int cam = 0; cam < g.num_cams; ++cam) {
        std::string p = "backbones." + std::to_string(cam) + ".0.body.";
        add_param(c, p + "conv1.weight", {w0, 3, 7, 7}, false);
        add_fbn(c, p + "bn1.", w0);
        int cin = w0;
        for (int li = 1; li <= 4; ++li) {
            const int cout = w0 << (li - 1);
            for (int bi = 0; bi < 2; ++bi) {
                std::string bp = p + "layer" + std::to_string(li) + "." + std::to_string(bi) + ".";
                add_param(c, bp + "conv1.weight", {cout, cin, 3, 3}, false);
                add_fbn(c, bp + "bn1.", cout);
                add_param(c, bp + "conv2.weight", {cout, cout, 3, 3}, false);
                add_fbn(c, bp + "bn2.", cout);
                if (bi == 0 && li > 1) {
                    add_param(c, bp + "downsample.0.weight", {cout, cin, 1, 1}, false);
                    add_fbn(c, bp + "downsample.1.", cout);
                }
                cin = cout;
            }
        }
    }
    add_param(c, "input_proj_robot_state.weight", {D, S}, false);
    add_param(c, "input_proj_robot_state.bias", {D}, false);
    add_param(c, "cls_embed.weight", {1, D}, false);
    add_param(c, "encoder_action_proj.weight", {D, A}, false);
    add_param(c, "encoder_action_proj.bias", {D}, false);
    add_param(c, "encoder_joint_proj.weight", {D, S}, false);
    add_param(c, "encoder_joint_proj.bias", {D}, false);
    const int Lp = g.vq ? g.vq_class * g.vq_dim : 2 * L, Li = g.vq ? g.vq_class * g.vq_dim : L;
    add_param(c, "latent_proj.weight", {Lp, D}, false);
    add_param(c, "latent_proj.bias", {Lp}, false);
    add_param(c, "latent_out_proj.weight", {D, Li}, false);
    add_param(c, "latent_out_proj.bias", {D}, false);
    add_param(c, "additional_pos_embed.weight", {2, D}, false);
}

}

int dev_alloc(actmi_ctx* ctx, float** p, int64_t nfloats) {
    void* q = nullptr;
    hipError_t e = hipMalloc(&q, (size_t)(nfloats > 0 ? nfloats : 1) * sizeof(float));
    if (e != hipSuccess) {
        ctx->err = std::string("hipMalloc: ") + hipGetErrorString(e);
        return ACTMI_E_NOMEM;
    }
    ctx->allocs.push_back(q);
    *p = reinterpret_cast<float*>(q);
    return 0;
}

int ctx_gemm(actmi_ctx* ctx, GemmArgs a, hipStream_t st, int ws_half, LnFuse* ln) {
    if (ln) ln->done = false;
    a.prec = ctx->prec_override ? ctx->prec_override : ctx->gemm_prec;
    const int64_t ws_part = (ctx->splitk_ws_floats / ctx->nbranch) & ~(int64_t)3;
    float* const ws = ctx->splitk_ws ? ctx->splitk_ws + (ws_half > 0 ? ws_half * ws_part : 0) : nullptr;
    const int64_t ws_floats = ws_half >= 0 ? ws_part : ctx->splitk_ws_floats;
    if (a.prec == ACTMI_PREC_F16X3 && a.tb == 0) {
        if (a.Bw >= ctx->pbase && a.Bw < ctx->pbase + ctx->ptotal) {
            a.b_scale = engine_weight_scale(ctx, a.Bw);
            a.Bw = ctx->p16base + (a.Bw - ctx->pbase);
            a.b_split = 1;
        } else {
            for (const ConvLayer& cl : ctx->convs) {
                if (a.Bw >= cl.w && a.Bw < cl.w + (int64_t)ctx->cfg.num_cams * cl.cout * cl.K) {
                    a.Bw = cl.w16 + (a.Bw - cl.w); a.b_split = 1; a.b_scale = cl.w16_scale; a.k_tap_inner = cl.k_tap_inner ? 1 : 0; break;
                }
                if (cl.wf && a.Bw >= cl.wf && a.Bw < cl.wf + (int64_t)ctx->cfg.num_cams * cl.cout * (cl.K + cl.Kx)) {
                    a.Bw = cl.wf16 + (a.Bw - cl.wf); a.b_split = 1; a.b_scale = cl.wf16_scale; a.k_tap_inner = cl.k_tap_inner ? 1 : 0; break;
                }
            }
        }
    }
    constexpr int sk_target = 1536, sk_minnk = 12, sk_maxtiles = 768;
    constexpr int sk_target_long = 4864, sk_maxtiles_long = 1300, sk_long_nk = 128;
    if (ctx->fwd_splitk && ctx->splitk_ws && a.splitk <= 1 && a.tb == 0 && a.ta == 0 && (a.mode == 0 || a.mode == 1) &&
        !a.rowmap && !a.C2 && !a.mask && a.drop_p == 0.f && a.res_mod == 0 && a.groups_inner == 0 && !a.stamps) {
        const int groups = a.groups > 0 ? a.groups : 1;
        const int64_t tiles = (int64_t)((a.M + 63) / 64) * ((a.N + 63) / 64) * groups * (ws_half >= 0 ? ctx->policy_mult : 1);
        const int nk = (a.K + 31) / 32;
        int S = tiles < sk_maxtiles ? (int)((sk_target + tiles - 1) / tiles) : 1;
        if (S == 1 && tiles < sk_maxtiles_long && nk >= sk_long_nk) S = (int)((sk_target_long + tiles - 1) / tiles);
        if (ln && S == 1 && ctx->ln_split > 1 && nk >= 64 && tiles < 2 * sk_maxtiles) S = ctx->ln_split;
        if (S > 8) S = 8;
        if (S > nk / sk_minnk) S = nk / sk_minnk;
        while (S >= 2 && (S - 1) * ((nk + S - 1) / S) >= nk) --S;
        if (S >= 2 && (int64_t)a.M * a.N * groups * S <= ws_floats && (a.N & 3) == 0) return gemm_slices(ctx, a, S, ws, st, ln);
    }
    return launch_gemm(a, st, &ctx->err);
}

int gemm_slices(actmi_ctx* ctx, const GemmArgs& a, int S, float* ws, hipStream_t st, LnFuse* ln) {
    const int groups = a.groups > 0 ? a.groups : 1;
    const int64_t slice = (int64_t)a.M * a.N;
    GemmArgs p = a;
    p.scale = p.bias = p.res = nullptr;
    p.relu = 0;
    p.C = ws;
    p.ldc = a.N;
    p.gC = slice * S;
    p.splitk = S;
    p.split_stride = slice;
    int rc = launch_gemm(p, st, &ctx->err);
    if (rc) return rc;
    if (ln && groups == 1 && !a.scale && !a.relu && (!a.res || a.ldres == a.N)) {
        rc = launch_layernorm(ws, a.res, 0, ln->w, ln->b, ln->w2, ln->b2, ln->out, a.M, a.N, ln->eps, st, &ctx->err, S, slice,
                              a.bias, ln->extra);
        ln->done = rc == 0;
        return rc;
    }
    SplitCombineArgs c{};
    c.part = ws; c.nsplit = S; c.split_stride = slice; c.gP = slice * S; c.ldp = a.N;
    c.scale = a.scale; c.bias = a.bias; c.gSB = a.gSB;
    c.res = a.res; c.ldres = a.ldres; c.gRes = a.gRes;
    c.relu = a.relu;
    c.C = a.C; c.ldc = a.ldc; c.gC = a.gC;
    c.M = a.M; c.N = a.N; c.groups = groups;
    rc = launch_splitk_combine(c, st);
    if (rc) ctx->err = "splitk combine launch failed";
    return rc;
}

float engine_weight_scale(const actmi_ctx* ctx, const float* w) {
    const int64_t off = w - ctx->pbase;
    size_t lo = 0, hi = ctx->params.size();
    while (hi - lo > 1) {
        const size_t mid = (lo + hi) / 2;
        if (ctx->params[mid].off <= off) lo = mid; else hi = mid;
    }
    return lo < ctx->pscale.size() ? ctx->pscale[lo] : W16_SCALE;
}

int engine_calibrate_weight_scales(actmi_ctx* ctx, hipStream_t st) {
    const int np = (int)ctx->params.size();
    ctx->pscale.assign(np, W16_SCALE);
    if (ctx->gemm_prec != ACTMI_PREC_F16X3) return 0;
    CHK(launch_seg_amax(ctx->pbase, ctx->poff_dev, ctx->pnumel_dev, np, ctx->pamax_dev, st));
    std::vector<unsigned> bits(np);
    HIPCHK(hipMemcpyAsync(bits.data(), ctx->pamax_dev, np * sizeof(unsigned), hipMemcpyDeviceToHost, st));
    HIPCHK(hipStreamSynchronize(st));
    float gmax = 0.f;
    for (int i = 0; i < np; ++i) {
        float amax;
        memcpy(&amax, &bits[i], 4);
        if (!(amax <= 3.0e38f)) {
            ctx->err = "parameter " + ctx->params[i].key + " is not finite";
            return ACTMI_E_INVALID;
        }
        float sc = 4096.f;
        if (amax > 0.f) {
            int e;
            frexpf(amax, &e);
            const float fit = ldexpf(1.f, 14 - e);
            sc = fit < 4096.f ? fit : 4096.f;
        }
        if (!(sc >= 1.17549435e-38f) || !(amax * sc < 65504.f)) {
            ctx->err = "parameter " + ctx->params[i].key + " is too large for the f16x3 path (use gemm_prec f32)";
            return ACTMI_E_INVALID;
        }
        ctx->pscale[i] = sc;
        if (!ctx->params[i].is_buffer && amax > gmax) gmax = amax;
    }
    HIPCHK(hipMemcpyAsync(ctx->pscale_dev, ctx->pscale.data(), np * sizeof(float), hipMemcpyHostToDevice, st));
    auto key_scale = [&](const std::string& key) {
        auto it = ctx->index.find(key);
        return it == ctx->index.end() ? W16_SCALE : ctx->pscale[it->second];
    };
    ctx->conv1_wscale = 4096.f;
    for (auto& cl : ctx->convs) cl.w16_scale = 4096.f;
    for (int cam = 0; cam < ctx->cfg.num_cams; ++cam) {
        const std::string p = "backbones." + std::to_string(cam) + ".0.body.";
        ctx->conv1_wscale = std::min(ctx->conv1_wscale, key_scale(p + "conv1.weight"));
        for (auto& cl : ctx->convs) cl.w16_scale = std::min(cl.w16_scale, key_scale(p + cl.name + ".weight"));
    }
    ctx->bwd_wscale = W16_SCALE;
    while (gmax * ctx->bwd_wscale >= 16384.f && ctx->bwd_wscale > 1.f / 65536.f) ctx->bwd_wscale *= 0.5f;
    HIPCHK(hipStreamSynchronize(st));
    return 0;
}

namespace {

MhaW mha_w(actmi_ctx* c, const std::string& p) {
    MhaW m;
    m.in_w = c->P(p + "in_proj_weight");
    m.in_b = c->P(p + "in_proj_bias");
    m.out_w = c->P(p + "out_proj.weight");
    m.out_b = c->P(p + "out_proj.bias");
    return m;
}

void resolve_layers(actmi_ctx* c) {
    const actmi_config& g = c->cfg;
    auto enc = [&](const std::string& p) {
        EncW e;
        e.attn = mha_w(c, p + "self_attn.");
        e.l1w = c->P(p + "linear1.weight"); e.l1b = c->P(p + "linear1.bias");
        e.l2w = c->P(p + "linear2.weight"); e.l2b = c->P(p + "linear2.bias");
        e.n1w = c->P(p + "norm1.weight"); e.n1b = c->P(p + "norm1.bias");
        e.n2w = c->P(p + "norm2.weight"); e.n2b = c->P(p + "norm2.bias");
        return e;
    };
    c->enc.clear(); c->cvae.clear(); c->dec.clear();
    for (int i = 0; i < g.enc_layers; ++i) c->enc.push_back(enc("transformer.encoder.layers." + std::to_string(i) + "."));
    if (g.has_cvae_encoder)
        for (int i = 0; i < g.enc_layers; ++i) c->cvae.push_back(enc("encoder.layers." + std::to_string(i) + "."));
    for (int i = 0; i < g.dec_layers; ++i) {
        std::string p = "transformer.decoder.layers." + std::to_string(i) + ".";
        DecW d;
        d.self_attn = mha_w(c, p + "self_attn.");
        d.cross = mha_w(c, p + "multihead_attn.");
        d.l1w = c->P(p + "linear1.weight"); d.l1b = c->P(p + "linear1.bias");
        d.l2w = c->P(p + "linear2.weight"); d.l2b = c->P(p + "linear2.bias");
        d.n1w = c->P(p + "norm1.weight"); d.n1b = c->P(p + "norm1.bias");
        d.n2w = c->P(p + "norm2.weight"); d.n2b = c->P(p + "norm2.bias");
        d.n3w = c->P(p + "norm3.weight"); d.n3b = c->P(p + "norm3.bias");
        c->dec.push_back(d);
    }
}

}

GemmArgs linear_args(const float* A, int64_t lda, int M, int K, const float* W, int N, const float* bias, float* C,
                     int64_t ldc) {
    GemmArgs a;
    memset(&a, 0, sizeof(a));
    a.A = A; a.lda = lda; a.M = M; a.K = K; a.N = N; a.Bw = W; a.ldb = K; a.bias = bias; a.C = C; a.ldc = ldc;
    a.groups = 1;
    return a;
}
// ... 495 lines not shown

int engine_backbone(actmi_ctx* ctx, const void* image, int fmt, int B, hipStream_t st) {
    const actmi_config& g = ctx->cfg;
    const int C = g.num_cams, w0 = g.base_width, D = g.hidden_dim;
    Conv1Args c1 = stem_args(ctx, image, fmt, B);
    const bool vpool = ctx->conv1_vpool && ctx->stop_stage != "conv1" && ctx->gemm_prec == ACTMI_PREC_F16X3 && (ctx->H1 & 1) == 0 &&
                       (w0 & 3) == 0 && ctx->H2 == ctx->H1 / 2;
    c1.vpool = vpool ? 1 : 0;
    CHK(launch_conv1(c1, st, &ctx->err));
    if (vpool) CHK(launch_hpool(ctx->act1, ctx->buf[0], C * B * ctx->H2, ctx->W1, w0, ctx->W2, st));
    else CHK(launch_maxpool(ctx->act1, ctx->buf[0], C * B, ctx->H1, ctx->W1, w0, ctx->H2, ctx->W2, st));
    ctx->dbg.clear();
    ctx->dbg["conv1"] = {ctx->act1, (int64_t)C * B * ctx->H1 * ctx->W1 * w0};
    ctx->dbg["maxpool"] = {ctx->buf[0], (int64_t)C * B * ctx->H2 * ctx->W2 * w0};
    if (ctx->stop_stage == "conv1" || ctx->stop_stage == "maxpool") return 1;
    auto run_conv_on = [&](const ConvLayer& cl, const float* in, float* out, const float* res, int relu, hipStream_t cs, int c0,
                           int nc, int half) -> int {
        const int cl_index = (int)(&cl - ctx->convs.data());
        if (ctx->calibrating) {
            float sc = 1.f;
            CHK(engine_measure_act_scale(ctx, in, (int64_t)nc * B * cl.H * cl.W, cl.cin, cs, &sc));
            const_cast<ConvLayer&>(cl).a_scale = sc;
            HIPCHK(hipMemcpyAsync(ctx->act_scale_dev + cl_index, &cl.a_scale, sizeof(float), hipMemcpyHostToDevice, cs));
            HIPCHK(hipStreamSynchronize(cs));
        }
        if (ctx->gemm_prec == ACTMI_PREC_F16X3 && cl.direct) {
            Conv3Args c3 = conv3_args(cl, B, c0, nc, in, out, res, relu);
            if (cl.a_scale != 1.f) c3.x_scale_dev = ctx->act_scale_dev + cl_index;
            return launch_conv3x3_c64(c3, cs, &ctx->err);
        }
        GemmArgs a = conv_gemm_args(cl, B, c0, nc, in, out, res, relu);
        if (ctx->gemm_prec == ACTMI_PREC_F16X3 && cl.a_scale != 1.f) a.a_scale = cl.a_scale;
        return ctx_gemm(ctx, a, cs, half);
    };
    const bool pipe = ctx->cam_pipe && ctx->pipe_stream && C >= 2 && !prof_enabled() && ctx->stop_stage.empty() && !ctx->calibrating;
    const bool fork_ds = ctx->side_stream != nullptr && !pipe && !ctx->calibrating;
    float* final_cur = nullptr;
    auto run_layers = [&](int c0, int nc, hipStream_t ls, int half) -> int {
        const int64_t hb = (int64_t)c0 * B * ctx->H2 * ctx->W2 * w0;
        float *cur = ctx->buf[0] + hb, *s1 = ctx->buf[1] + hb, *s2 = ctx->buf[2] + hb;
        auto run_conv = [&](const ConvLayer& cl, const float* in, float* out, const float* res, int relu) -> int {
            return run_conv_on(cl, in, out, res, relu, ls, c0, nc, half);
        };
        auto run_conv_fused = [&](const ConvLayer& cl, const float* y1, const float* x, float* out) -> int {
            const ConvLayer& ds = ctx->convs[cl.ds_index];
            const int Kf = cl.K + cl.Kx;
            GemmArgs a;
            memset(&a, 0, sizeof(a));
            a.mode = 1;
            a.A = y1; a.H = cl.H; a.W = cl.W; a.Cin = cl.cin; a.KH = a.KW = cl.k; a.stride = cl.stride; a.pad = cl.pad;
            a.Ho = cl.Ho; a.Wo = cl.Wo; a.img_stride = (int64_t)cl.H * cl.W * cl.cin;
            a.M = B * cl.Ho * cl.Wo; a.N = cl.cout; a.K = Kf;
            a.Ax = x; a.kx_begin = cl.K; a.Hx = ds.H; a.Wx = ds.W; a.Cx = ds.cin; a.stride_x = ds.stride;
            a.gAx = (int64_t)B * ds.H * ds.W * ds.cin;
            a.Bw = cl.wf + (int64_t)c0 * cl.cout * Kf; a.ldb = Kf; a.bias = cl.bias_f + (int64_t)c0 * cl.cout; a.relu = 1;
            a.C = out; a.ldc = cl.cout;
            a.groups = nc;
            a.gA = (int64_t)B * cl.H * cl.W * cl.cin; a.gB = (int64_t)cl.cout * Kf; a.gSB = cl.cout;
            a.gC = (int64_t)a.M * cl.cout;
            return ctx_gemm(ctx, a, ls, half);
        };
        size_t ci = 0;
        for (int li = 1; li <= 4; ++li) {
            for (int bi = 0; bi < 2; ++bi) {
                const ConvLayer& k1 = ctx->convs[ci++];
                const ConvLayer& k2 = ctx->convs[ci++];
                const bool has_ds = (bi == 0 && li > 1);
                if (has_ds && k2.wf && ctx->gemm_prec == ACTMI_PREC_F16X3 && !ctx->calibrating && k2.a_scale == 1.f &&
                    ctx->convs[k2.ds_index].a_scale == 1.f) {
                    ++ci;
                    CHK(run_conv(k1, cur, s1, nullptr, 1));
                    CHK(run_conv_fused(k2, s1, cur, s2));
                    std::swap(cur, s2);
                } else if (has_ds) {
                    const ConvLayer& ds = ctx->convs[ci++];
                    if (fork_ds) {
                        HIPCHK(hipEventRecord(ctx->ev_fork, ls));
                        HIPCHK(hipStreamWaitEvent(ctx->side_stream, ctx->ev_fork, 0));
                        const int r1 = run_conv_on(ds, cur, s2, nullptr, 0, ctx->side_stream, c0, nc, half);
                        const hipError_t e1 = hipEventRecord(ctx->ev_join, ctx->side_stream);
                        const int r2 = r1 == 0 ? run_conv(k1, cur, s1, nullptr, 1) : 0;
                        const hipError_t e2 = e1 == hipSuccess ? hipStreamWaitEvent(ls, ctx->ev_join, 0) : e1;
                        CHK(r1);
                        CHK(r2);
                        HIPCHK(e1);
                        HIPCHK(e2);
                    } else {
                        CHK(run_conv(k1, cur, s1, nullptr, 1));
                        CHK(run_conv(ds, cur, s2, nullptr, 0));
                    }
                    CHK(run_conv(k2, s1, cur, s2, 1));
                } else {
                    CHK(run_conv(k1, cur, s1, nullptr, 1));
                    CHK(run_conv(k2, s1, s2, cur, 1));
                    std::swap(cur, s2);
                }
                if (bi == 1 && c0 == 0) {
                    const std::string nm = "layer" + std::to_string(li);
                    ctx->dbg[nm] = {cur, (int64_t)C * B * k2.Ho * k2.Wo * k2.cout};
                    if (ctx->stop_stage == nm) { final_cur = cur; return 1; }
                }
            }
        }
        final_cur = cur;
        GemmArgs ip = linear_args(cur, 8 * w0, nc * B * ctx->P_, 8 * w0, ctx->P("input_proj.weight"), D, ctx->P("input_proj.bias"),
                                  ctx->X, D);
        ip.rowmap = ctx->rowmap + (int64_t)c0 * B * ctx->P_;
        if (ctx->calibrating) {
            CHK(engine_measure_act_scale(ctx, cur, (int64_t)nc * B * ctx->P_, 8 * w0, ls, &ctx->ip_a_scale));
            HIPCHK(hipStreamSynchronize(ls));
        }
        if (ctx->gemm_prec == ACTMI_PREC_F16X3 && ctx->ip_a_scale != 1.f) ip.a_scale = ctx->ip_a_scale;
        return ctx_gemm(ctx, ip, ls, half);
    };
    if (ctx->rowmap_B != B) {
        CHK(launch_build_rowmap(ctx->rowmap, B, C, ctx->fh, ctx->fw, ctx->N, st));
        ctx->rowmap_B = B;
    }
    if (pipe) {
        const int nb = C < ctx->nbranch ? C : ctx->nbranch;
        const int rc = run_branches(ctx, nb, st, [&](int i, hipStream_t bs) -> int {
            const int c0 = i * C / nb, c1 = (i + 1) * C / nb;
            return run_layers(c0, c1 - c0, bs, i);
        });
        if (rc != 0) return rc;
    } else {
        const int rc = run_layers(0, C, st, -1);
        if (rc != 0) return rc;
    }
    (void)final_cur;
    return 0;
}

struct TView {
    float *X, *XP, *QKV, *ATT, *Y, *X1, *Hb, *dO, *dY, *dT2, *dH, *hs, *attn_ws;
    int64_t attn_ws_floats;
    int half;
};
static TView make_view(const actmi_ctx* ctx, int b0, int nb, int half) {
    const actmi_config& g = ctx->cfg;
    const int64_t D = g.hidden_dim, F = g.dim_feedforward, Q = g.num_queries, N = ctx->N;
    const int64_t ws_per = ctx->attn_ws_floats / g.max_batch;
    TView v;
    v.X = ctx->X + b0 * N * D; v.XP = ctx->XP + b0 * N * D; v.QKV = ctx->QKV + b0 * N * 3 * D; v.ATT = ctx->ATT + b0 * N * D; v.Y = ctx->Y + b0 * N * D;
    v.X1 = ctx->X1 + b0 * N * D; v.Hb = ctx->Hb + b0 * N * F;
    v.dO = ctx->dO + b0 * Q * D; v.dY = ctx->dY + b0 * Q * D; v.dT2 = ctx->dT2 + b0 * Q * D; v.dH = ctx->dH + b0 * Q * F;
    v.hs = ctx->hs + b0 * Q * D;
    v.attn_ws = ctx->attn_ws + b0 * ws_per; v.attn_ws_floats = (half < 0) ? ctx->attn_ws_floats : nb * ws_per;
    v.half = half;
    return v;
}

int engine_encoder_layer(actmi_ctx* ctx, const EncW& w, const TView& V, const float* pos, int B, int n, const uint8_t* kpm,
                         hipStream_t st, bool xp_in, bool xp_out) {
    float* x = V.X;
    const actmi_config& g = ctx->cfg;
    const int D = g.hidden_dim, F = g.dim_feedforward, M = B * n;
    GemmArgs qkv = linear_args(x, D, M, D, w.attn.in_w, 3 * D, w.attn.in_b, V.QKV, 3 * D);
    if (xp_in) { qkv.A_alt = V.XP; qkv.alt_ncols = 2 * D; }
    else { qkv.A_add = pos; qkv.ld_add = D; qkv.add_mod = n; qkv.add_ncols = 2 * D; }
    CHK(ctx_gemm(ctx, qkv, st, V.half));
    AttnArgs at = packed_self_attn_args(ctx, V.QKV, V.ATT, B, n);
    at.kpm = kpm;
    at.ws = V.attn_ws; at.ws_floats = V.attn_ws_floats;
    at.prec = ctx->gemm_prec;
    CHK(launch_attention(at, st, &ctx->err));
    GemmArgs op = linear_args(V.ATT, D, M, D, w.attn.out_w, D, w.attn.out_b, V.Y, D);
    op.res = x; op.ldres = D;
    LnFuse ln1{w.n1w, w.n1b, nullptr, nullptr, V.X1, 1e-5f, false};
    CHK(ctx_gemm(ctx, op, st, V.half, &ln1));
    if (!ln1.done) CHK(launch_layernorm(V.Y, nullptr, 0, w.n1w, w.n1b, nullptr, nullptr, V.X1, M, D, 1e-5f, st, &ctx->err));
    GemmArgs f1 = linear_args(V.X1, D, M, D, w.l1w, F, w.l1b, V.Hb, F);
    f1.relu = 1;
    CHK(ctx_gemm(ctx, f1, st, V.half));
    GemmArgs f2 = linear_args(V.Hb, F, M, F, w.l2w, D, w.l2b, V.Y, D);
    f2.res = V.X1; f2.ldres = D;
    LnExtra ex;
    if (xp_out) { ex.y2 = V.XP; ex.add2 = pos; ex.add2_mod = n; }
    LnFuse ln2{w.n2w, w.n2b, nullptr, nullptr, x, 1e-5f, false, xp_out ? &ex : nullptr};
    CHK(ctx_gemm(ctx, f2, st, V.half, &ln2));
    if (!ln2.done)
        CHK(launch_layernorm(V.Y, nullptr, 0, w.n2w, w.n2b, nullptr, nullptr, x, M, D, 1e-5f, st, &ctx->err, 1, 0, nullptr,
                             xp_out ? &ex : nullptr));
    return 0;
}

int engine_decoder_infer(actmi_ctx* ctx, const TView& V, int B, float* a_hat, hipStream_t st, bool xp_in) {
    const actmi_config& g = ctx->cfg;
    const int D = g.hidden_dim, F = g.dim_feedforward, Q = g.num_queries, N = ctx->N;
    const DecW& d = ctx->dec[0];
    float* KV = V.QKV;
    GemmArgs kv = linear_args(V.X, D, B * N, D, d.cross.in_w + (int64_t)D * D, 2 * D, d.cross.in_b + D, KV, 2 * D);
    if (xp_in) { kv.A_alt = V.XP; kv.alt_ncols = D; }
    else { kv.A_add = ctx->pos_tokens; kv.ld_add = D; kv.add_mod = N; kv.add_ncols = D; }
    CHK(ctx_gemm(ctx, kv, st, V.half));
    AttnArgs at = cross_attn_args(ctx, ctx->dec_q, false, KV, V.dO, B);
    at.ws = V.attn_ws; at.ws_floats = V.attn_ws_floats;
    at.prec = ctx->gemm_prec;
    CHK(launch_attention(at, st, &ctx->err));
    const int M = B * Q;
    GemmArgs op = linear_args(V.dO, D, M, D, d.cross.out_w, D, d.cross.out_b, V.dY, D);
    op.res = ctx->dec_t1; op.ldres = D; op.res_mod = 1;
    CHK(ctx_gemm(ctx, op, st, V.half));
    CHK(launch_layernorm(V.dY, nullptr, 0, d.n2w, d.n2b, nullptr, nullptr, V.dT2, M, D, 1e-5f, st, &ctx->err));
    GemmArgs f1 = linear_args(V.dT2, D, M, D, d.l1w, F, d.l1b, V.dH, F);
    f1.relu = 1;
    CHK(ctx_gemm(ctx, f1, st, V.half));
    GemmArgs f2 = linear_args(V.dH, F, M, F, d.l2w, D, d.l2b, V.dY, D);
    f2.res = V.dT2; f2.ldres = D;
    LnExtra hx;
    const bool head_in_ln = g.action_dim <= 64;
    if (head_in_ln) {
        hx.head_out = a_hat; hx.head_w = ctx->P("action_head.weight"); hx.head_b = ctx->P("action_head.bias"); hx.head_n = g.action_dim;
        hx.flag = ctx->flags; hx.flag_bit = ACTMI_FLAG_OUTPUT;
    }
    LnFuse ln3{d.n3w, d.n3b, ctx->P("transformer.decoder.norm.weight"), ctx->P("transformer.decoder.norm.bias"), V.hs, 1e-5f, false,
               head_in_ln ? &hx : nullptr};
    CHK(ctx_gemm(ctx, f2, st, V.half, &ln3));
    if (!ln3.done)
        CHK(launch_layernorm(V.dY, nullptr, 0, d.n3w, d.n3b, ctx->P("transformer.decoder.norm.weight"),
                             ctx->P("transformer.decoder.norm.bias"), V.hs, M, D, 1e-5f, st, &ctx->err, 1, 0, nullptr,
                             head_in_ln ? &hx : nullptr));
    if (!head_in_ln) {
        GemmArgs ah = linear_args(V.hs, D, M, D, ctx->P("action_head.weight"), g.action_dim, ctx->P("action_head.bias"),
                                  a_hat, g.action_dim);
        ah.finite_flag = ctx->flags; ah.finite_bit = ACTMI_FLAG_OUTPUT;
        CHK(ctx_gemm(ctx, ah, st, V.half));
    }
    if (V.half <= 0) ctx->dbg["hs"] = {ctx->hs, (int64_t)ctx->last_B * Q * D};
    return 0;
}

int engine_forward_infer(actmi_ctx* ctx, const float* qpos, const void* image, int fmt, int B, float* a_hat,
                         hipStream_t st, const float* vq_sample) {
    ctx->err.clear();
    if (!ctx->finalized) { ctx->err = "forward before finalize"; return ACTMI_E_STATE; }
    if (B < 1 || B > ctx->cfg.max_batch) { ctx->err = "batch exceeds max_batch"; return ACTMI_E_INVALID; }
    if (fmt != ACTMI_IMG_U8_NHWC && fmt != ACTMI_IMG_F32_NCHW) { ctx->err = "bad image format"; return ACTMI_E_INVALID; }
    const actmi_config& g = ctx->cfg;
    const int D = g.hidden_dim, N = ctx->N;
    if (ctx->fwd_phase != 2) {
        const int rc = engine_backbone(ctx, image, fmt, B, st);
        if (rc == 1) return 0;
        if (rc != 0) return rc;
        float* fill_dst = nullptr;
        if (g.vq && vq_sample) {
            const int K = g.vq_class * g.vq_dim;
            GemmArgs lz = linear_args(vq_sample, K, B, K, ctx->P("latent_out_proj.weight"), D, ctx->P("latent_out_proj.bias"),
                                      ctx->X, (int64_t)N * D);
            CHK(ctx_gemm(ctx, lz, st));
        } else {
            fill_dst = ctx->X;
        }
        CHK(launch_small_linear(qpos, g.state_dim, ctx->P("input_proj_robot_state.weight"),
                                ctx->P("input_proj_robot_state.bias"), ctx->X + D, (int64_t)N * D, B, D, g.state_dim, st, fill_dst,
                                ctx->P("latent_out_proj.bias"), 0));
        if (ctx->fwd_phase == 1) { ctx->last_B = B; return 0; }
    } else if (B != ctx->last_B) {
        ctx->err = "forward phase 2 without a phase 1 of the same batch before it";
        return ACTMI_E_STATE;
    }
    ctx->dbg["src"] = {ctx->X, (int64_t)B * N * D};
    if (ctx->stop_stage == "src") return 0;
    ctx->last_B = B;
    auto run_transformer = [&](int b0, int nb, hipStream_t ts, int half) -> int {
        const TView V = make_view(ctx, b0, nb, half);
        const bool xp_qkv = ((2 * D) % 128) == 0, xp_kv = (D % 128) == 0;
        for (int l = 0; l < g.enc_layers; ++l)
            CHK(engine_encoder_layer(ctx, ctx->enc[l], V, ctx->pos_tokens, nb, N, nullptr, ts, l > 0 && xp_qkv,
                                     l + 1 < g.enc_layers ? xp_qkv : xp_kv));
        return engine_decoder_infer(ctx, V, nb, a_hat + (int64_t)b0 * g.num_queries * g.action_dim, ts, xp_kv);
    };
    const bool tpipe = ctx->cam_pipe && ctx->pipe_stream && B >= 2 && !prof_enabled() && ctx->stop_stage.empty();
    ctx->dbg["memory"] = {ctx->X, (int64_t)B * N * D};
    if (tpipe) {
        const int nb = B < ctx->nbranch ? B : ctx->nbranch;
        const int rc = run_branches(ctx, nb, st, [&](int i, hipStream_t bs) -> int {
            const int b0 = i * B / nb, b1 = (i + 1) * B / nb;
            return run_transformer(b0, b1 - b0, bs, i);
        });
        if (rc != 0) return rc;
    } else {
        CHK(run_transformer(0, B, st, -1));
    }
    return 0;
}
```

act-plus-plus_amd/csrc/gemm.hip:

```cpp
#include "common.h"
#include "dropout.h"
#include "split16.h"
#include <cstdio>
#include <string>
#include <cstdlib>
#include <type_traits>

namespace {

constexpr int BK = 32;
constexpr int NPL = BK / 4;

enum { A_N = 0, A_CONV = 1, A_DGRAD = 2, A_T = 3, A_NADD = 4 };
enum { B_N = 0, B_T = 1, B_WGRAD = 2 };

enum { PREC_F32 = 0, PREC_F16X3 = 1, PREC_BF16 = 2 };
constexpr int ACTMI_PREC_DEFAULT_IS = ACTMI_PREC_F32;

#ifndef ACTMI_LDS_PAD
#define ACTMI_LDS_PAD 1
#endif
constexpr int LDS_PAD = ACTMI_LDS_PAD;

template <int BM, int BN, int PREC>
constexpr int stage_f4() { return NPL * ((BM + LDS_PAD) + (BN + LDS_PAD)); }

typedef _Float16 h16x4 __attribute__((ext_vector_type(4)));
typedef _Float16 h16x8 __attribute__((ext_vector_type(8)));
typedef __bf16 bf16x2 __attribute__((ext_vector_type(2)));
typedef __bf16 bf16x8 __attribute__((ext_vector_type(8)));

__device__ __forceinline__ uint2 pack_bf16x4(const f32x4 v) {
    const bf16x2 a = {(__bf16)v[0], (__bf16)v[1]}, b = {(__bf16)v[2], (__bf16)v[3]};
    return uint2{__builtin_bit_cast(unsigned, a), __builtin_bit_cast(unsigned, b)};
}

__device__ __forceinline__ int swz_row(int r) { return r ^ ((r >> 3) & 3); }

__device__ __forceinline__ f32x4 ld4(const float* p) { return *reinterpret_cast<const f32x4*>(p); }

template <int BM, int BN, int WM, int WN, int AMODE, int BMODE, int PREC, int BSPLIT, int UNMASKED, int XS = 0>
__global__ __launch_bounds__((BM / WM) * (BN / WN) * 64, (PREC && BM * BN <= 128 * 64 && (AMODE == 0  || AMODE == 3 ) && !(AMODE == 0 && BMODE == 1)) ? 3 : 2)
    void gemm_f32_kernel(GemmArgs p, int tiles_m, int tiles_n) {
    constexpr int NT = (BM / WM) * (BN / WN) * 64;
    constexpr int RPP = NT / 8;
    constexpr int TM = WM / 32, TN = WN / 32;
    constexpr int WAVES_N = BN / WN;
    constexpr int PSA = BM + LDS_PAD, PSB = BN + LDS_PAD;
    constexpr int STAGE = stage_f4<BM, BN, PREC>();
    constexpr int NLA = (AMODE == A_T) ? 4 : BM / RPP;
    constexpr int NLB = (BMODE != B_N) ? 4 : BN / RPP;
    static_assert(BM % RPP == 0 && BN % RPP == 0, "tile rows must be a multiple of the rows staged per pass");
    extern __shared__ __attribute__((aligned(16))) char smem_raw[];
    f32x4* smem = reinterpret_cast<f32x4*>(smem_raw);

    const int nwg = tiles_m * tiles_n;
    const int splitk = p.splitk > 1 ? p.splitk : 1;
    int bid, zz;
    {
        const int total = nwg * (int)gridDim.z;
        const int lin = blockIdx.z * gridDim.x + blockIdx.x;
        const int xcd = lin & 7, q = total >> 3, r = total & 7;
        const int base = (xcd < r) ? xcd * (q + 1) : r * (q + 1) + (xcd - r) * q;
        const int flat = base + (lin >> 3);
        zz = flat / nwg;
        bid = flat - zz * nwg;
    }
    constexpr int GROUP_M = 8;
    const int width = GROUP_M * tiles_n;
    const int group_id = bid / width;
    const int first_m = group_id * GROUP_M;
    const int gsz = (tiles_m - first_m < GROUP_M) ? tiles_m - first_m : GROUP_M;
    const int in_group = bid - group_id * width;
    const int m0 = (first_m + in_group % gsz) * BM;
    const int n0 = (in_group / gsz) * BN;
    const int split = zz % splitk;
    const int g = zz / splitk;
    int64_t offA, offB, offC, offRes;
    if (p.groups_inner > 0) {
        const int g1 = g / p.groups_inner, g2 = g % p.groups_inner;
        offA = g1 * p.gA + g2 * p.gA2; offB = g1 * p.gB + g2 * p.gB2;
        offC = g1 * p.gC + g2 * p.gC2; offRes = g1 * p.gRes + g2 * p.gRes2;
    } else {
        offA = (int64_t)g * p.gA; offB = (int64_t)g * p.gB; offC = (int64_t)g * p.gC; offRes = (int64_t)g * p.gRes;
    }
    const float* __restrict__ A = ((AMODE == A_N) && p.A_alt != nullptr && n0 < p.alt_ncols ? p.A_alt : p.A) + offA;
    const float* __restrict__ Bw = p.Bw + offB;

    uint64_t* stamp = p.stamps ? p.stamps + ((int64_t)blockIdx.z * gridDim.x + blockIdx.x) * 4 : nullptr;
    if (stamp && threadIdx.x == 0) {
        stamp[0] = __builtin_amdgcn_s_memtime();
        const unsigned hw = __builtin_amdgcn_s_getreg((4 ) | (0 << 6) | (31 << 11));
        const unsigned xcc = __builtin_amdgcn_s_getreg((20 ) | (0 << 6) | (31 << 11));
        stamp[1] = ((uint64_t)xcc << 32) | hw;
    }
    unsigned* const amax_out = UNMASKED ? nullptr : p.amax_out;
    unsigned* const fflag = UNMASKED ? nullptr : p.finite_flag;
    const bool track = amax_out != nullptr || fflag != nullptr;
    const unsigned amax_seen = amax_out ? __hip_atomic_load(amax_out, __ATOMIC_RELAXED, __HIP_MEMORY_SCOPE_AGENT) : 0u;
    const int nk_total = (p.K + BK - 1) / BK;
    const int tps = (nk_total + splitk - 1) / splitk;
    const int kt_begin = split * tps;
    const int kt_end = (kt_begin + tps < nk_total) ? kt_begin + tps : nk_total;
    if (kt_begin >= kt_end) return;
    const int t = threadIdx.x;
    const int lane = t & 63, wave = t >> 6;
    const int li = lane & 31, lh = lane >> 5;
    const int wrow0 = (wave / WAVES_N) * WM;
    const int wcol0 = (wave % WAVES_N) * WN;
    int arow[TM], bcol[TN];
#pragma unroll
    for (int i = 0; i < TM; ++i) arow[i] = (AMODE == A_T) ? swz_row(wrow0 + i * 32 + li) : wrow0 + i * 32 + li;
#pragma unroll
    for (int j = 0; j < TN; ++j) bcol[j] = (BMODE != B_N) ? swz_row(wcol0 + j * 32 + li) : wcol0 + j * 32 + li;
    const int cidx = t & 7;
    const int srow = t >> 3;

    const float* a_ptr[NLA];
    const float* add_ptr[NLA];
    int a_hi0[NLA], a_wi0[NLA];
    bool a_ok[NLA];
    const bool conv_fast = AMODE == A_CONV && (p.Cin % BK) == 0 && p.KH * p.KW <= 32 &&
                           (int64_t)p.H * p.W * p.Cin < ((int64_t)1 << 30);
    unsigned a_tapmask[AMODE == A_CONV ? NLA : 1];
    int a_off0[AMODE == A_CONV ? NLA : 1];
    int a_offx[XS ? NLA : 1];
    const float* __restrict__ Axg = XS ? p.Ax + (int64_t)g * p.gAx : nullptr;
    const int ktx = XS ? p.kx_begin / BK : 0x7fffffff;
    const float conv_inv_tpr = (AMODE == A_CONV && conv_fast) ? 1.0f / (float)(p.Cin / BK) : 0.f;
    const float conv_inv_kw = (AMODE == A_CONV || AMODE == A_DGRAD) ? 1.0f / (float)p.KW : 0.f;
    const float conv_inv_ntap = (AMODE == A_CONV) ? 1.0f / (float)(p.KH * p.KW) : 0.f;
    const int dg_cq = (AMODE == A_DGRAD) ? p.K / (p.KH * p.KW) : BK;
    const bool dgrad_fast = AMODE == A_DGRAD && (dg_cq % BK) == 0 && (p.stride == 1 || p.stride == 2) &&
                            (int64_t)p.Ho * p.Wo * dg_cq < ((int64_t)1 << 30);
    const float dg_inv_tpr = (AMODE == A_DGRAD) ? 1.0f / (float)(dg_cq / BK > 0 ? dg_cq / BK : 1) : 0.f;
    unsigned conv_rep = 0;
    if (AMODE == A_CONV && conv_fast)
        for (int r = 0; r < p.KH; ++r) conv_rep |= 1u << (r * p.KW);
    const bool use_add = (AMODE == A_NADD) && n0 < p.add_ncols;
    const int a_og = t % (BM / 4), a_kg = t / (BM / 4);
    if (AMODE == A_T) {
    } else {
#pragma unroll
        for (int i = 0; i < NLA; ++i) {
            const int m = m0 + srow + RPP * i;
            a_ok[i] = m < p.M;
            const int mm = a_ok[i] ? m : 0;
            add_ptr[i] = nullptr;
            a_hi0[i] = a_wi0[i] = 0;
            if (AMODE == A_N || AMODE == A_NADD) {
                const int64_t ar = p.a_rowmap ? p.a_rowmap[mm] : mm;
                a_ptr[i] = A + ar * p.lda;
                if (AMODE == A_NADD) add_ptr[i] = p.A_add + (int64_t)(mm % p.add_mod) * p.ld_add;
            } else if (AMODE == A_CONV) {
                const int hw = p.Ho * p.Wo;
                const int b = mm / hw, rem = mm - b * hw;
                const int ho = rem / p.Wo, wo = rem - ho * p.Wo;
                a_ptr[i] = A + (int64_t)b * p.img_stride;
                a_hi0[i] = ho * p.stride - p.pad;
                a_wi0[i] = wo * p.stride - p.pad;
                if (conv_fast) {
                    const int r_lo = a_hi0[i] < 0 ? -a_hi0[i] : 0, q_lo = a_wi0[i] < 0 ? -a_wi0[i] : 0;
                    int r_hi = p.H - a_hi0[i], q_hi = p.W - a_wi0[i];
                    r_hi = r_hi < p.KH ? (r_hi > 0 ? r_hi : 0) : p.KH;
                    q_hi = q_hi < p.KW ? (q_hi > 0 ? q_hi : 0) : p.KW;
                    const unsigned colmask = (r_lo < r_hi && q_lo < q_hi) ? (((1u << q_hi) - 1u) & ~((1u << q_lo) - 1u)) : 0u;
                    const unsigned rowsel = (unsigned)((((uint64_t)1 << (r_hi * p.KW)) - 1u) & ~(((uint64_t)1 << (r_lo * p.KW)) - 1u));
                    a_tapmask[i] = a_ok[i] ? (rowsel & (colmask * conv_rep)) : 0u;
                    a_off0[i] = (a_hi0[i] * p.W + a_wi0[i]) * p.Cin + cidx * 4;
                    if (XS) a_offx[i] = ((b * p.Hx + ho * p.stride_x) * p.Wx + wo * p.stride_x) * p.Cx + cidx * 4;
                }
            } else {
                const int hw = p.H * p.W;
                const int b = mm / hw, rem = mm - b * hw;
                const int hi = rem / p.W, wi = rem - hi * p.W;
                a_ptr[i] = A + (int64_t)b * p.img_stride;
                a_hi0[i] = hi + p.pad;
                a_wi0[i] = wi + p.pad;
            }
        }
    }
    const float* b_ptr[NLB];
    bool b_ok[NLB];
    const int b_og = t % (BN / 4), b_kg = t / (BN / 4);
    int wg_r = 0, wg_s = 0, wg_c = 0;
    const float wg_inv_hw = (BMODE == B_WGRAD) ? 1.0f / (float)(p.Ho * p.Wo) : 0.f;
    const float wg_inv_wo = (BMODE == B_WGRAD) ? 1.0f / (float)p.Wo : 0.f;
    if (BMODE == B_N) {
#pragma unroll
        for (int i = 0; i < NLB; ++i) {
            const int n = n0 + srow + RPP * i;
            b_ok[i] = n < p.N;
            b_ptr[i] = Bw + (int64_t)(b_ok[i] ? n : 0) * p.ldb;
        }
// ... 374 lines not shown
                    }
                }
            };
            ld(kt_begin, R0);
            ld(kt_begin + 1, R1);
            store16(0, R0, maskedc);
            __syncthreads();
            int s_ = 0;
            for (; s_ + 1 < nsteps; s_ += 2) {
                ld(kt_begin + s_ + 2, R0);
                compute16(0);
                store16(1, R1, maskedc);
                weave();
                __syncthreads();
                ld(kt_begin + s_ + 3, R1);
                compute16(1);
                store16(0, R0, maskedc);
                weave();
                __syncthreads();
            }
            if (s_ < nsteps) {
                compute16(0);
                __syncthreads();
            }
        };
        if constexpr (UNMASKED != 0) run(std::false_type{});
        else run(std::true_type{});
    } else {
    load_tile(kt_begin, R0);
    store_tile(0, R0);
    __syncthreads();
    auto kstep = [&](int s_, auto par, auto pf) {
        constexpr bool PF = decltype(pf)::value;
        constexpr int cur = decltype(par)::value;
        const int kt = kt_begin + s_;
        const f32x4* sa = smem + cur * STAGE;
        const f32x4* sb = sa + NPL * PSA;
        f32x4 af[2][TM], bf[2][TN];
#pragma unroll
        for (int i = 0; i < TM; ++i) af[0][i] = sa[lh * PSA + arow[i]];
#pragma unroll
        for (int j = 0; j < TN; ++j) bf[0][j] = sb[lh * PSB + bcol[j]];
        constexpr bool HOT = (AMODE == A_N || AMODE == A_NADD || AMODE == A_CONV) && BMODE == B_N;
        if (PF) load_tile(kt + 1, R0);
        auto kblock = [&](auto kbc) {
            constexpr int kb = decltype(kbc)::value;
            if (kb + 1 < NPL / 2) {
#pragma unroll
                for (int i = 0; i < TM; ++i) af[(kb + 1) & 1][i] = sa[(2 * (kb + 1) + lh) * PSA + arow[i]];
#pragma unroll
                for (int j = 0; j < TN; ++j) bf[(kb + 1) & 1][j] = sb[(2 * (kb + 1) + lh) * PSB + bcol[j]];
            }
#pragma unroll
            for (int e = 0; e < 4; ++e)
#pragma unroll
                for (int i = 0; i < TM; ++i)
#pragma unroll
                    for (int j = 0; j < TN; ++j)
                        acc[i][j] = __builtin_amdgcn_mfma_f32_32x32x2f32(af[kb & 1][i][e], bf[kb & 1][j][e], acc[i][j], 0, 0, 0);
            if (HOT) {
#pragma unroll
                for (int r = 0; r < 4 * TM * TN; ++r) {
                    __builtin_amdgcn_sched_group_barrier(0x008, 1, 0);
                    __builtin_amdgcn_sched_group_barrier(0x006, kb == 0 ? 10 : 2, 0);
                    __builtin_amdgcn_sched_group_barrier(0x020, 1, 0);
                    __builtin_amdgcn_sched_group_barrier(0x100, 1, 0);
                }
                __builtin_amdgcn_sched_barrier(0);
            }
        };
        kblock(std::integral_constant<int, 0>{});
        kblock(std::integral_constant<int, 1>{});
        kblock(std::integral_constant<int, 2>{});
        kblock(std::integral_constant<int, 3>{});
        static_assert(NPL / 2 == 4, "k-block unroll assumes BK = 32");
        if (PF) store_tile(cur ^ 1, R0);
        __syncthreads();
    };
    using P0 = std::integral_constant<int, 0>;
    using P1 = std::integral_constant<int, 1>;
    int s_ = 0;
    for (; s_ + 2 < nsteps; s_ += 2) {
        kstep(s_, P0{}, std::true_type{});
        kstep(s_ + 1, P1{}, std::true_type{});
    }
    if (nsteps - s_ == 2) {
        kstep(s_, P0{}, std::true_type{});
        kstep(s_ + 1, P1{}, std::false_type{});
    } else {
        kstep(s_, P0{}, std::false_type{});
    }
    }

    if (stamp && threadIdx.x == 0) stamp[2] = __builtin_amdgcn_s_memtime();
    const float* scale = p.scale ? p.scale + (int64_t)g * p.gSB : nullptr;
    const float* bias = p.bias ? p.bias + (int64_t)g * p.gSB : nullptr;
    const float* res = p.res ? p.res + offRes : nullptr;
    const float* mask = p.mask ? p.mask + (int64_t)g * p.gMask : nullptr;
    const int64_t ldmask = p.ldmask ? p.ldmask : p.ldc;
    float* C = p.C + offC + (int64_t)split * p.split_stride;
    float* C2 = p.C2 ? p.C2 + (int64_t)g * p.gC2out : nullptr;
    float alpha = p.alpha != 0.f ? p.alpha : 1.f;
    if (PREC != PREC_F32) {
        if (p.b_scale != 0.f) alpha /= p.b_scale;
        if (p.a_scale != 0.f) alpha /= p.a_scale;
        if (p.a_scale_dev) alpha /= *p.a_scale_dev;
        if (!BSPLIT && p.b_scale_dev) alpha /= *p.b_scale_dev;
    }
    const bool has_mask = mask != nullptr, has_map = p.rowmap != nullptr;
    const int epi = UNMASKED ? 0 : p.epi;
    const float* erow = nullptr;
    const uint8_t* ekill = nullptr;
    if (epi != 0) {
        if (p.groups_inner > 0) {
            const int g1 = g / p.groups_inner, g2 = g % p.groups_inner;
            erow = p.epi_row + g1 * p.gRow + g2 * p.gRow2;
            ekill = p.epi_colkill ? p.epi_colkill + g1 * p.gColkill : nullptr;
        } else {
            erow = p.epi_row + (int64_t)g * p.gRow;
            ekill = p.epi_colkill ? p.epi_colkill + (int64_t)g * p.gColkill : nullptr;
        }
    }
    const bool has_res = res != nullptr && epi != 2;
    const float drop_scale = p.drop_p > 0.f ? 1.f / (1.f - p.drop_p) : 1.f;
    const bool simple = !has_map && (splitk <= 1 || p.split_stride != 0) && !C2 && !(p.drop_p > 0.f) && p.res_mod == 0 &&
                        (!has_mask || (int64_t)p.M * ldmask < (int64_t)1 << 31) &&
                        (int64_t)p.M * p.ldc < (int64_t)1 << 31 && (!res || (int64_t)p.M * p.ldres < (int64_t)1 << 31);
    unsigned amx = 0;
    auto amax_flush = [&]() {
        if (!track) return;
        for (int o = 32; o > 0; o >>= 1) amx = max(amx, (unsigned)__shfl_xor((int)amx, o, 64));
        if (fflag && lane == 0 && amx >= 0x7f800000u) atomicOr(fflag, p.finite_bit);
        if (!amax_out) return;
        if (lane == 0 && amx > amax_seen) atomicMax(amax_out, amx);
    };
    if (simple) {
        const bool relu = p.relu == 1, gelu = p.relu == 2;

        const bool vec = n0 + BN <= p.N && (p.ldc & 3) == 0 && ((uintptr_t)C & 15) == 0 &&
                         (!res || ((p.ldres & 3) == 0 && ((uintptr_t)res & 15) == 0)) &&
                         (!has_mask || ((ldmask & 3) == 0 && ((uintptr_t)mask & 15) == 0)) &&
                         (!scale || ((uintptr_t)scale & 15) == 0) && (!bias || ((uintptr_t)bias & 15) == 0);
        if (vec) {
            constexpr int RS = WN + 8;
            constexpr int LPR = WN / 4;
            constexpr int RPI = 64 / LPR;
            static_assert(4 * 32 * RS * 4 <= 2 * STAGE * 16 || (BM / WM) * (BN / WN) * 32 * RS * 4 <= 2 * STAGE * 16, "epilogue scratch must fit the stage");
            float* scr = reinterpret_cast<float*>(smem) + wave * (32 * RS);
            const int c4 = lane % LPR, r0 = lane / LPR;
            const int ncol = n0 + wcol0 + c4 * 4;
            const f32x4 one4 = {1.f, 1.f, 1.f, 1.f};
            const f32x4 sc4 = scale ? ld4(scale + ncol) : one4;
            const f32x4 bi4 = bias ? ld4(bias + ncol) : zero4;
#pragma unroll
            for (int i = 0; i < TM; ++i) {
#pragma unroll
                for (int j = 0; j < TN; ++j)
#pragma unroll
                    for (int e = 0; e < 16; ++e)
                        scr[((e & 3) + 8 * (e >> 2) + 4 * lh) * RS + j * 32 + li] = acc[i][j][e];
                const int mbase = m0 + wrow0 + i * 32;
#pragma unroll
                for (int q = 0; q < 32 / RPI; ++q) {
                    const int r = q * RPI + r0;
                    const int m = mbase + r;
                    f32x4 v = *reinterpret_cast<const f32x4*>(scr + r * RS + c4 * 4);
                    v = v * alpha * sc4 + bi4;
                    if (m < p.M) {
                        if (epi == 1) {
                            const float rsub = erow[m];
#pragma unroll
                            for (int e = 0; e < 4; ++e) v[e] = (ekill && ekill[ncol + e] != 0) ? 0.f : expf(v[e] - rsub);
                        } else if (epi == 2) {
                            const f32x4 pr = ld4(res + (uint32_t)(m * (int)p.ldres + ncol));
                            v = pr * (v - erow[m]) * p.epi_scale;
                        }
                        if (has_res) v += ld4(res + (uint32_t)(m * (int)p.ldres + ncol));
                        if (has_mask) {
                            const f32x4 mk = ld4(mask + (uint32_t)(m * (int)ldmask + ncol));
#pragma unroll
                            for (int e = 0; e < 4; ++e) v[e] = mk[e] > 0.f ? v[e] : 0.f;
                        }
                        if (relu) {
#pragma unroll
                            for (int e = 0; e < 4; ++e) v[e] = fmaxf(v[e], 0.f);
                        }
                        if (gelu) {
#pragma unroll
                            for (int e = 0; e < 4; ++e) v[e] = 0.5f * v[e] * (1.f + erff(v[e] * 0.70710678118654752f));
                        }
                        *reinterpret_cast<f32x4*>(C + (uint32_t)(m * (int)p.ldc + ncol)) = v;
                        if (track) {
#pragma unroll
                            for (int e = 0; e < 4; ++e) amx = max(amx, __float_as_uint(v[e]) & 0x7fffffffu);
                        }
                    }
                }
            }
            amax_flush();
            if (stamp && threadIdx.x == 0) stamp[3] = __builtin_amdgcn_s_memtime();
            return;
        }
#pragma unroll
        for (int j = 0; j < TN; ++j) {
            const int n = n0 + wcol0 + j * 32 + li;
            const bool nok = n < p.N;
            const float sc = (scale && nok) ? scale[n] : 1.f;
            const float bi = (bias && nok) ? bias[n] : 0.f;
#pragma unroll
            for (int i = 0; i < TM; ++i) {
                const int mb = m0 + wrow0 + i * 32 + 4 * lh;
                float rv[16];
                if (has_res) {
#pragma unroll
                    for (int e = 0; e < 16; ++e) {
                        const int m = mb + (e & 3) + 8 * (e >> 2);
                        const int mc = m < p.M ? m : 0;
                        rv[e] = nok ? res[(uint32_t)(mc * (int)p.ldres + n)] : 0.f;
                    }
                }
#pragma unroll
                for (int e = 0; e < 16; ++e) {
                    const int m = mb + (e & 3) + 8 * (e >> 2);
                    float v = acc[i][j][e] * alpha * sc + bi;
                    if (epi != 0 && nok && m < p.M) {
                        if (epi == 1) v = (ekill && ekill[n] != 0) ? 0.f : expf(v - erow[m]);
                        else v = res[(uint32_t)(m * (int)p.ldres + n)] * (v - erow[m]) * p.epi_scale;
                    }
                    if (has_res) v += rv[e];
                    if (has_mask && nok && m < p.M) { if (!(mask[(uint32_t)(m * (int)ldmask + n)] > 0.f)) v = 0.f; }
                    v = relu ? fmaxf(v, 0.f) : v;
                    if (gelu) v = 0.5f * v * (1.f + erff(v * 0.70710678118654752f));
                    if (nok && m < p.M) {
                        C[(uint32_t)(m * (int)p.ldc + n)] = v;
                        if (track) amx = max(amx, __float_as_uint(v) & 0x7fffffffu);
                    }
                }
                __builtin_amdgcn_sched_barrier(0);
            }
        }
        amax_flush();
        if (stamp && threadIdx.x == 0) stamp[3] = __builtin_amdgcn_s_memtime();
        return;
    }
#pragma unroll
    for (int j = 0; j < TN; ++j) {
        const int n = n0 + wcol0 + j * 32 + li;
        const bool nok = n < p.N;
        const float sc = (scale && nok) ? scale[n] : 1.f;
        const float bi = (bias && nok) ? bias[n] : 0.f;
        const float sc2 = (C2 && nok) ? p.scale2[(int64_t)g * p.gSB + n] : 1.f;
#pragma unroll
        for (int i = 0; i < TM; ++i) {
            int orow[16];
            bool ok[16];
#pragma unroll
            for (int e = 0; e < 16; ++e) {
                const int m = m0 + wrow0 + i * 32 + (e & 3) + 8 * (e >> 2) + 4 * lh;
                ok[e] = nok && m < p.M;
                orow[e] = m;
                if (has_map && ok[e]) orow[e] = p.rowmap[m];
            }
            float rv[16], mv[16];
#pragma unroll
            for (int e = 0; e < 16; ++e) {
                const int m = m0 + wrow0 + i * 32 + (e & 3) + 8 * (e >> 2) + 4 * lh;
                rv[e] = 0.f;
                mv[e] = 1.f;
                if (has_res && ok[e]) rv[e] = res[(int64_t)(p.res_mod ? (m % p.res_mod) : m) * p.ldres + n];
                if (has_mask && ok[e]) mv[e] = mask[(int64_t)m * ldmask + n];
            }
#pragma unroll
            for (int e = 0; e < 16; ++e) {
                if (ok[e]) {
                    float v = acc[i][j][e] * alpha;
                    v = scale ? v * sc + bi : v + bi;
                    const int64_t o = (int64_t)orow[e] * p.ldc + n;
                    if (p.drop_p > 0.f) {
                        if (p.relu && !has_res) v = fmaxf(v, 0.f);
                        v = actmi_keep(p.drop_seed, (uint64_t)(offC + o), p.drop_p) ? v * drop_scale : 0.f;
                    }
                    v += rv[e];
                    if (!(mv[e] > 0.f)) v = 0.f;
                    if (p.relu) v = fmaxf(v, 0.f);
                    if (splitk > 1 && p.split_stride == 0) atomicAdd(&C[o], v);
                    else C[o] = v;
                    if (track) amx = max(amx, __float_as_uint(v) & 0x7fffffffu);
                    if (C2) C2[o] = v * sc2;
                }
            }
            __builtin_amdgcn_sched_barrier(0);
        }
    }
    amax_flush();
    if (stamp && threadIdx.x == 0) stamp[3] = __builtin_amdgcn_s_memtime();
}

template <int BM, int BN, int WM, int WN, int AMODE, int BMODE, int PREC, int BSPLIT, int UNMASKED, int XS = 0>
int launch_cfg_u(const GemmArgs& a, hipStream_t st) {
    const int tiles_m = (a.M + BM - 1) / BM, tiles_n = (a.N + BN - 1) / BN;
    static const int lds_pad = getenv("ACTMI_GEMM_LDSPAD") ? atoi(getenv("ACTMI_GEMM_LDSPAD")) : 0;
    const int smem = 2 * stage_f4<BM, BN, PREC>() * 16 + lds_pad;
    auto kern = gemm_f32_kernel<BM, BN, WM, WN, AMODE, BMODE, PREC, BSPLIT, UNMASKED, XS>;
    static bool attr_set = false;
    if (!attr_set) {
        hipError_t e = hipFuncSetAttribute(reinterpret_cast<const void*>(kern),
                                           hipFuncAttributeMaxDynamicSharedMemorySize, smem);
        if (e != hipSuccess) return (int)e;
        attr_set = true;
    }
    const int splitk = a.splitk > 1 ? a.splitk : 1;
    dim3 grid(tiles_m * tiles_n, 1, (a.groups > 0 ? a.groups : 1) * splitk);
    if (prof_enabled()) {
        char nm[128];
        static const bool by_shape = getenv("ACTMI_PROF_SHAPES") && getenv("ACTMI_PROF_SHAPES")[0] == '1';
        if (by_shape)
            snprintf(nm, sizeof(nm), "gemm_%s_kernel<%d,%d,%d,%d,%d,%d%s>[M=%d,N=%d,K=%d,g=%d,sk=%d,wgs=%d]", PREC == PREC_BF16 ? "bf16" : PREC ? "f16x3" : "f32",
                     BM, BN, WM, WN, AMODE, BMODE, XS ? ",xs" : "", a.M, a.N, a.K, a.groups, splitk, tiles_m * tiles_n * a.groups * splitk);
        else
            snprintf(nm, sizeof(nm), "gemm_%s_kernel<%d,%d,%d,%d,%d,%d%s>", PREC == PREC_BF16 ? "bf16" : PREC ? "f16x3" : "f32", BM, BN, WM, WN, AMODE, BMODE, XS ? ",xs" : "");
        const double g = a.groups;
        double abytes;
        if (AMODE == A_CONV) abytes = (double)(a.M / (a.Ho * a.Wo)) * a.H * a.W * a.Cin + (XS ? (double)a.M * a.Cx : 0.0);
        else if (AMODE == A_DGRAD) abytes = (double)(a.M / (a.H * a.W)) * a.Ho * a.Wo * (a.K / (a.KH * a.KW));
        else abytes = (double)a.M * a.K;
        const double bbytes = (BMODE == B_WGRAD) ? (double)(a.K / (a.Ho * a.Wo)) * a.H * a.W * a.Cin : (double)a.N * a.K;
        prof_begin(nm, 2.0 * a.M * a.N * a.K * g, 4.0 * g * ((double)a.M * a.N + abytes + bbytes), st);
    }
    hipLaunchKernelGGL(kern, grid, dim3((BM / WM) * (BN / WN) * 64), smem, st, a, tiles_m, tiles_n);
    prof_end(st);
    return (int)hipGetLastError();
}

template <int BM, int BN, int WM, int WN, int AMODE, int BMODE, int PREC, int BSPLIT>
int launch_cfg_b(const GemmArgs& a, hipStream_t st) {
    constexpr bool HOT = PREC != PREC_F32 && BMODE == B_N && (AMODE == A_N || AMODE == A_NADD || AMODE == A_CONV);
    if constexpr (HOT) {
        const bool one_a = (a.a_scale == 0.f || a.a_scale == 1.f) && !a.a_scale_dev;
        const bool one_b = BSPLIT || ((a.b_scale == 0.f || a.b_scale == 1.f) && !a.b_scale_dev);
        const bool unmasked_ok = (a.K % BK) == 0 && one_a && one_b && a.epi == 0 && !a.amax_out && !a.finite_flag;
        if constexpr (AMODE == A_CONV && BSPLIT == 1) {
            if (a.Ax) return unmasked_ok ? launch_cfg_u<BM, BN, WM, WN, AMODE, BMODE, PREC, BSPLIT, 1, 1>(a, st) : -1001;
        }
        if (unmasked_ok) return launch_cfg_u<BM, BN, WM, WN, AMODE, BMODE, PREC, BSPLIT, 1>(a, st);
    }
    if (a.Ax) return -1001;
    return launch_cfg_u<BM, BN, WM, WN, AMODE, BMODE, PREC, BSPLIT, 0>(a, st);
}

template <int BM, int BN, int WM, int WN, int AMODE, int BMODE, int PREC>
int launch_cfg(const GemmArgs& a, hipStream_t st) {
    constexpr bool CAN_BSPLIT = PREC == PREC_F16X3 && BMODE == B_N && (AMODE == A_N || AMODE == A_NADD || AMODE == A_CONV);
    if constexpr (CAN_BSPLIT) {
        if (a.b_split) return launch_cfg_b<BM, BN, WM, WN, AMODE, BMODE, PREC, 1>(a, st);
    }
    return launch_cfg_b<BM, BN, WM, WN, AMODE, BMODE, PREC, 0>(a, st);
}

double tile_cost(int M, int N, int K, int nz, int BM, int BN, double eff, double fixed) {
    const long tiles = (long)((M + BM - 1) / BM) * ((N + BN - 1) / BN) * nz;
    const long full = tiles / 512, f = tiles - full * 512;
    double rounds = 2.0 * full + (f == 0 ? 0.0 : (f <= 256 ? 1.0 : 1.0 + (double)(f - 256) / 256.0));
    if (tiles <= 256) rounds *= 1.3;
    const double nk = (double)((K + BK - 1) / BK);
    return rounds * ((double)BM * BN / (128.0 * 128.0)) * (fixed + nk / eff);
}

template <int AMODE, int BMODE, int PREC>
int launch_modes(const GemmArgs& a, hipStream_t st) {
    const int nz = a.groups > 0 ? a.groups : 1;
    const int Ks = a.splitk > 1 ? (a.K + a.splitk - 1) / a.splitk : a.K;
    const int nzs = nz * (a.splitk > 1 ? a.splitk : 1);
    const double fixed = PREC ? 10.0 : 2.5;
    const double cL = tile_cost(a.M, a.N, Ks, nzs, 128, 128, 1.00, fixed);
    const double cM = tile_cost(a.M, a.N, Ks, nzs, 128, 64, PREC ? ((AMODE == A_N || AMODE == A_T) ? 0.83 : 0.74) : 0.95, fixed);
    const double cS = tile_cost(a.M, a.N, Ks, nzs, 64, 64, PREC ? 0.68 : 0.88, fixed);
    double eL = -cL, eM = -cM, eS = -cS;
    if (!PREC) {
        auto eff = [&](int BM, int BN, double factor) {
            const long tiles = (long)((a.M + BM - 1) / BM) * ((a.N + BN - 1) / BN) * nzs;
            const long rounds = (tiles + 255) / 256;
            return factor * ((double)a.M * a.N * nzs) / ((double)rounds * 256 * BM * BN);
        };
        eL = eff(128, 128, 1.00); eM = eff(128, 64, 0.95); eS = eff(64, 64, 0.88);
    }
    static const std::string hints = getenv("ACTMI_TILE_HINTS") ? getenv("ACTMI_TILE_HINTS") : "";
    if (!hints.empty() && a.tile_hint == 0) {
        char key[64];
        snprintf(key, sizeof(key), "%d,%d,%d=", a.M, a.N, a.K);
        const size_t pos = hints.find(key);
        if (pos != std::string::npos && (pos == 0 || hints[pos - 1] == ';')) {
            const char c = hints[pos + strlen(key)];
            if (c == 'L') return launch_cfg<128, 128, 64, 64, AMODE, BMODE, PREC>(a, st);
            if (c == 'M') return launch_cfg<128, 64, 64, 32, AMODE, BMODE, PREC>(a, st);
            if (c == 'S') return launch_cfg<64, 64, 32, 32, AMODE, BMODE, PREC>(a, st);
        }
    }
    static const char* force = getenv("ACTMI_GEMM_CFG");
    if (force && force[0] == 'L') return launch_cfg<128, 128, 64, 64, AMODE, BMODE, PREC>(a, st);
    if (force && force[0] == 'M') return launch_cfg<128, 64, 64, 32, AMODE, BMODE, PREC>(a, st);
    if (force && force[0] == 'S') return launch_cfg<64, 64, 32, 32, AMODE, BMODE, PREC>(a, st);
    if (a.tile_hint == 1) return launch_cfg<128, 128, 64, 64, AMODE, BMODE, PREC>(a, st);
    if (a.tile_hint == 2) return launch_cfg<128, 64, 64, 32, AMODE, BMODE, PREC>(a, st);
    if (a.tile_hint == 3) return launch_cfg<64, 64, 32, 32, AMODE, BMODE, PREC>(a, st);
    if (eL >= eM && eL >= eS) return launch_cfg<128, 128, 64, 64, AMODE, BMODE, PREC>(a, st);
    if (eM >= eS) return launch_cfg<128, 64, 64, 32, AMODE, BMODE, PREC>(a, st);
    return launch_cfg<64, 64, 32, 32, AMODE, BMODE, PREC>(a, st);
}

}

#ifdef ACTMI_GEMM_TU_BF16
int launch_gemm_bf16(int amode, int bmode, bool has_add, const GemmArgs& a, hipStream_t st) {
    int rc;
#define ACTMI_DISPATCH(PREC)                                                                                       \
    if (amode == A_N && bmode == B_N && has_add) rc = launch_modes<A_NADD, B_N, PREC>(a, st);                      \
    else if (amode == A_N && bmode == B_N) rc = launch_modes<A_N, B_N, PREC>(a, st);                               \
    else if (amode == A_CONV && bmode == B_N) rc = launch_modes<A_CONV, B_N, PREC>(a, st);                         \
    else if (amode == A_DGRAD && bmode == B_N) rc = launch_modes<A_DGRAD, B_N, PREC>(a, st);                       \
    else if (amode == A_N && bmode == B_T) rc = launch_modes<A_N, B_T, PREC>(a, st);                               \
    else if (amode == A_T && bmode == B_T) rc = launch_modes<A_T, B_T, PREC>(a, st);                               \
    else if (amode == A_T && bmode == B_WGRAD) rc = launch_modes<A_T, B_WGRAD, PREC>(a, st);                       \
    else if (amode == A_T && bmode == B_N) rc = launch_modes<A_T, B_N, PREC>(a, st);                               \
    else rc = -1002;
    ACTMI_DISPATCH(PREC_BF16)
#undef ACTMI_DISPATCH
    return rc;
}
#else
int launch_gemm_bf16(int amode, int bmode, bool has_add, const GemmArgs& a, hipStream_t st);

int env_gemm_prec(int unset) {
    const char* e = getenv("ACTMI_GEMM_PREC");
    if (!e) return unset;
    return (e[0] == 'f' && e[1] == '3') ? ACTMI_PREC_F32 : ACTMI_PREC_F16X3;
}

int launch_gemm(const GemmArgs& a_in, hipStream_t st, std::string* err) {
    GemmArgs a = a_in;
    if (a.groups <= 0) a.groups = 1;
    if (a.M <= 0 || a.N <= 0) return 0;
    auto fail = [&](const char* m) { if (err) *err = std::string("gemm: ") + m; return -2; };
    if (a.K <= 0) return fail("K must be positive");
    if (((uintptr_t)a.A & 15) || ((uintptr_t)a.Bw & 15)) return fail("A/B must be 16-byte aligned");
    if (a.splitk > 1 && (a.bias || a.res || a.mask || a.relu || a.C2 || a.scale)) return fail("split-K supports a plain accumulate only");
    if (a.split_stride != 0) {
        if (a.splitk <= 1) return fail("split_stride needs splitk > 1");
        const int nk = (a.K + BK - 1) / BK, tps = (nk + a.splitk - 1) / a.splitk;
        if ((a.splitk - 1) * tps >= nk) return fail("split_stride: every split must own at least one K tile");
    }
    if (a.relu == 2 && (a.rowmap || a.C2 || a.drop_p > 0.f || a.res_mod != 0)) return fail("GELU is only available in the plain epilogue");
    if (a.relu < 0 || a.relu > 2) return fail("bad activation");
    if (a.C2 && !a.scale2) return fail("C2 needs scale2");
    int amode, bmode = a.tb;
    if (a.ta) {
        if (a.mode != 0) return fail("ta requires mode 0");
        if (a.lda & 3) return fail("lda must be a multiple of 4");
        if (a.A_add || a.a_rowmap) return fail("addend / row gather not supported with ta");
        amode = A_T;
    } else {
        if (a.mode == 0) {
            if (a.lda & 3) return fail("lda must be a multiple of 4");
            if ((a.K & 3) && a.lda < ((a.K + 3) & ~3)) return fail("K % 4 != 0 needs rows padded to a multiple of 4");
            if (a.A_add && ((a.ld_add & 3) || a.add_mod <= 0 || ((uintptr_t)a.A_add & 15))) return fail("bad addend");
            if (a.A_alt && (a.A_add || a.a_rowmap || (a.alt_ncols % 128) || ((uintptr_t)a.A_alt & 15))) return fail("A_alt: no addend / row gather, alt_ncols a multiple of 128");
            amode = A_N;
        } else if (a.mode == 1) {
            if (a.K & 3) return fail("K must be a multiple of 4");
            if (a.Cin & 3) return fail("Cin must be a multiple of 4");
            if (a.Ax) {
                if (a.kx_begin != a.KH * a.KW * a.Cin || a.K != a.kx_begin + a.Cx) return fail("second source: K must be KH*KW*Cin + Cx, kx_begin = KH*KW*Cin");
                if ((a.Cin % BK) || (a.Cx % BK) || a.KH * a.KW > 32) return fail("second source: Cin and Cx must be multiples of 32");
                if (a.stride_x < 1 || (a.Ho - 1) * a.stride_x >= a.Hx || (a.Wo - 1) * a.stride_x >= a.Wx) return fail("second source: the strided pixel grid leaves the map");
                const int64_t nimg = a.M / ((int64_t)a.Ho * a.Wo);
                if (nimg * a.Hx * a.Wx * a.Cx >= ((int64_t)1 << 31) || (int64_t)a.H * a.W * a.Cin >= ((int64_t)1 << 30)) return fail("second source: map too large for 32-bit offsets");
                if ((uintptr_t)a.Ax & 15) return fail("second source must be 16-byte aligned");
            } else if (a.K != a.KH * a.KW * a.Cin) return fail("K != KH*KW*Cin");
            if (a.A_add || a.a_rowmap) return fail("addend not supported in conv mode");
            if (a.M % (a.Ho * a.Wo)) return fail("M must be images*Ho*Wo");
            if (a.k_tap_inner && ((a.Cin % BK) || a.KH * a.KW > 32 || (int64_t)a.H * a.W * a.Cin >= ((int64_t)1 << 30)))
                return fail("k_tap_inner needs Cin % 32 == 0 (the uniform-tap loader)");
            amode = A_CONV;
        } else if (a.mode == 2) {
            if (a.K % (a.KH * a.KW) || ((a.K / (a.KH * a.KW)) & 3)) return fail("dgrad: K must be KH*KW*Cout, Cout % 4 == 0");
            if (a.M % (a.H * a.W)) return fail("dgrad: M must be images*H*W");
            amode = A_DGRAD;
        } else return fail("bad mode");
    }
    if (bmode == 0) {
        if ((a.ldb & 3) || (a.K & 3)) return fail("ldb and K must be multiples of 4 for a contraction-contiguous B");
    } else if (bmode == 1) {
        if (a.ldb & 3) return fail("ldb must be a multiple of 4");
        if (a.B_add && ((a.ld_badd & 3) || a.badd_mod <= 0)) return fail("bad B addend");
    } else if (bmode == 2) {
        if ((a.Cin & 3) || a.N != a.KH * a.KW * a.Cin) return fail("wgrad: N must be KH*KW*Cin, Cin % 4 == 0");
        if (a.K % (a.Ho * a.Wo)) return fail("wgrad: K must be images*Ho*Wo");
        if (!a.ta) return fail("wgrad: A (dY) must be given in [m][n] storage (ta=1)");
    } else return fail("bad tb");
    int rc;
    static const int env_prec = env_gemm_prec(ACTMI_PREC_DEFAULT_IS);
    const int prec = a.prec ? a.prec : env_prec;
    if (prec != ACTMI_PREC_F32 && prec != ACTMI_PREC_F16X3 && prec != ACTMI_PREC_BF16) return fail("bad prec");
    if (a.b_split && (prec != ACTMI_PREC_F16X3 || bmode != B_N || !(amode == A_N || amode == A_CONV)))
        return fail("b_split needs prec f16x3 and the forward operand forms");
#define ACTMI_DISPATCH(PREC)                                                                                       \
    if (amode == A_N && bmode == B_N && a.A_add) rc = launch_modes<A_NADD, B_N, PREC>(a, st);                      \
    else if (amode == A_N && bmode == B_N) rc = launch_modes<A_N, B_N, PREC>(a, st);                               \
    else if (amode == A_CONV && bmode == B_N) rc = launch_modes<A_CONV, B_N, PREC>(a, st);                         \
    else if (amode == A_DGRAD && bmode == B_N) rc = launch_modes<A_DGRAD, B_N, PREC>(a, st);                       \
    else if (amode == A_N && bmode == B_T) rc = launch_modes<A_N, B_T, PREC>(a, st);                               \
    else if (amode == A_T && bmode == B_T) rc = launch_modes<A_T, B_T, PREC>(a, st);                               \
    else if (amode == A_T && bmode == B_WGRAD) rc = launch_modes<A_T, B_WGRAD, PREC>(a, st);                       \
    else if (amode == A_T && bmode == B_N) rc = launch_modes<A_T, B_N, PREC>(a, st);                               \
    else return fail("operand form combination not instantiated");
    if (prec == ACTMI_PREC_BF16) {
        if (a.Ax) return fail("a second source (Ax) needs prec f16x3");
        rc = launch_gemm_bf16(amode, bmode, a.A_add != nullptr, a, st);
        if (rc == -1002) return fail("operand form combination not instantiated");
    } else if (prec == ACTMI_PREC_F16X3) { ACTMI_DISPATCH(PREC_F16X3) } else { ACTMI_DISPATCH(PREC_F32) }
#undef ACTMI_DISPATCH
    if (rc == -1001) return fail("a second source (Ax) needs prec f16x3, pre-split weights (b_split), K % 32 == 0 and a plain epilogue");
    if (rc != 0 && err) *err = std::string("gemm launch: ") + hipGetErrorString((hipError_t)rc);
    return rc == 0 ? 0 : -3;
}
#endif
```

include/actmi.h:

```cpp
#ifndef ACTMI_H
#define ACTMI_H

#include <stdint.h>

#ifdef __cplusplus
extern "C" {
#endif

#define ACTMI_VERSION 110

#define ACTMI_OK 0
#define ACTMI_E_INVALID (-1)
#define ACTMI_E_SHAPE (-2)
#define ACTMI_E_LAUNCH (-3)
#define ACTMI_E_STATE (-4)
#define ACTMI_E_NOMEM (-5)

#define ACTMI_IMG_U8_NHWC 0
#define ACTMI_IMG_F32_NCHW 1

typedef struct actmi_ctx* actmi_handle;

typedef struct actmi_config {
    uint32_t struct_size;
    int32_t num_cams;
    int32_t image_h, image_w;
    int32_t base_width;
    int32_t hidden_dim, nheads, dim_feedforward;
    int32_t enc_layers, dec_layers;
    int32_t num_queries, state_dim, action_dim, latent_dim;
    int32_t has_cvae_encoder;
    int32_t max_batch;
    int32_t enable_training;
    float kl_weight;
    int32_t vq, vq_class, vq_dim;
} actmi_config;

#define ACTMI_PREC_F32 1
#define ACTMI_PREC_F16X3 2
#define ACTMI_PREC_BF16 3

typedef struct actmi_gemm_desc {
    const float* A;
    int64_t lda;
    int32_t mode;
    int32_t H, W, Cin, KH, KW, stride, pad, Ho, Wo;
    int64_t img_stride;
    const float* A_add;
    int64_t ld_add;
    int32_t add_mod;
    int32_t add_ncols;
    const float* Bw;
    int64_t ldb;
    const float* scale;
    const float* bias;
    const float* res;
    int64_t ldres;
    int32_t res_mod;
    int32_t relu;
    float* C;
    int64_t ldc;
    const int32_t* rowmap;
    int32_t M, N, K;
    int32_t groups;
    int64_t gA, gB, gSB, gC, gRes;
    int32_t ta;
    int32_t tb;
    const int32_t* a_rowmap;
    const float* B_add;
    int64_t ld_badd;
    int32_t badd_mod;
    int32_t splitk;
    const float* mask;
    int64_t ldmask;
    float* C2;
    const float* scale2;
    float alpha;
    int32_t groups_inner;
    int64_t gA2, gB2, gC2, gRes2;
    int64_t gMask, gC2out;
    float drop_p;
    uint64_t drop_seed;
    uint64_t* stamps;
    int32_t prec;
    int32_t b_split;
    float b_scale;
    float a_scale;
    const float* a_scale_dev;
    const float* b_scale_dev;
    int64_t split_stride;
    uint32_t* amax_out;
    int32_t epi;
    float epi_scale;
    const float* epi_row;
    int64_t gRow, gRow2;
    const uint8_t* epi_colkill;
    int64_t gColkill;
    int32_t tile_hint;
    uint32_t* finite_flag;
    uint32_t finite_bit;
    const float* Ax;
    int32_t kx_begin, Hx, Wx, Cx, stride_x;
    int64_t gAx;
    const float* A_alt;
    int32_t alt_ncols;
    int32_t k_tap_inner;
} actmi_gemm_desc;

typedef struct actmi_attn_desc {
    const float* Q; int64_t q_bs, q_rs;
    const float* K; int64_t k_bs, k_rs;
    const float* V; int64_t v_bs, v_rs;
    float* O; int64_t o_bs, o_rs;
    const uint8_t* kpm; int64_t kpm_bs;
    float* lse;
    int32_t B, H, Nq, Nk, HD;
    float scale;
    float* ws;
    int64_t ws_floats;
    float drop_p;
    uint64_t drop_seed;
    int32_t prec;
    int32_t causal;
} actmi_attn_desc;

int actmi_version(void);

int actmi_create(const actmi_config* cfg, actmi_handle* out);
int actmi_destroy(actmi_handle h);
const char* actmi_last_error(actmi_handle h);

int actmi_num_params(actmi_handle h);
int actmi_param_info(actmi_handle h, int index, const char** key, int64_t* shape4, int* ndim, int* is_buffer);
int actmi_set_param(actmi_handle h, const char* key, const void* src, const int64_t* shape, int ndim, int is_device);
int actmi_get_param(actmi_handle h, const char* key, void* dst, int64_t nbytes, int is_device);
int actmi_param_ptr(actmi_handle h, const char* key, void** dev_ptr, int64_t* numel);
int actmi_finalize(actmi_handle h, void* stream);

int actmi_forward_infer(actmi_handle h, const float* qpos , const void* image, int image_fmt, int B,
                        float* a_hat , void* stream);

int actmi_set_forward_phase(actmi_handle h, int phase);

int actmi_forward_infer_vq(actmi_handle h, const float* qpos, const void* image, int image_fmt, int B,
                           const float* vq_sample, float* a_hat, void* stream);

int actmi_forward_train(actmi_handle h, const float* qpos, const void* image, int image_fmt,
                        const float* actions , const uint8_t* is_pad ,
                        const float* eps , uint64_t dropout_seed, float dropout_p, int B,
                        float* losses , float* a_hat, float* mu, float* logvar, void* stream);
int actmi_backward(actmi_handle h, float loss_scale, void* stream);
int actmi_zero_grad(actmi_handle h, void* stream);
int actmi_adamw_step(actmi_handle h, float lr, float lr_backbone, float weight_decay, float beta1, float beta2,
                     float eps, int64_t step, void* stream);
int actmi_adamw_step_range(actmi_handle h, float lr, float lr_backbone, float weight_decay, float beta1, float beta2,
                           float eps, int64_t step, int64_t offset, int64_t count, void* stream);
int actmi_refresh_weights(actmi_handle h, void* stream);
int actmi_param_arena(actmi_handle h, void** dev_ptr, int64_t* nfloats);
int actmi_grad_ptr(actmi_handle h, const char* key, void** dev_ptr, int64_t* numel);
int actmi_grad_arena(actmi_handle h, void** dev_ptr, int64_t* nfloats);

int actmi_grad_phase_range(actmi_handle h, int phase, int64_t* offset, int64_t* count);
int actmi_wait_grad_phase(actmi_handle h, int phase, void* stream);

int actmi_ensemble_step(float* ring, int32_t* tcount, const float* chunk, double k, double* out, uint8_t* populated,
                        int E, int Q, int A, void* stream);

int actmi_op_gemm(const actmi_gemm_desc* d, void* stream);
int actmi_op_split16(const float* src, float* dst, int64_t nfloats, float scale, void* stream);
int actmi_op_permute_conv_k(const float* src, float* dst, int64_t rows, int taps, int cin, int ld, void* stream);
int actmi_op_pow2_scale(const float* x, int64_t ld, int M, int N, float* out, void* stream);
int actmi_op_splitk_combine(const float* part, int nsplit, int64_t split_stride, int64_t ldp, int M, int N, const float* scale,
                            const float* bias, const float* res, int64_t ldres, int relu, float* out, int64_t ldc, void* stream);
int actmi_op_sample_onehot(const float* logits, int n, int V, float temperature, uint64_t seed, float* probs, float* code,
                           void* stream);
int actmi_op_attention(const actmi_attn_desc* d, void* stream);
typedef struct actmi_attn_bwd_desc {
    const float *q, *k, *v, *o, *d_o, *lse;
    float *dq, *dk, *dv;
    int64_t q_bs, q_rs, k_bs, k_rs, v_bs, v_rs, dq_bs, dq_rs, dk_bs, dk_rs, dv_bs, dv_rs;
    const uint8_t* kpm;
    int64_t kpm_bs;
    int32_t B, H, Nq, Nk, HD;
    float drop_p;
    uint64_t drop_seed;
    float* delta_ws;
    const float* do_scale;
    uint32_t* amax_out;
} actmi_attn_bwd_desc;
int actmi_op_attention_bwd(const actmi_attn_bwd_desc* d, void* stream);
int actmi_op_layernorm(const float* x, const float* res, int res_mod, const float* w, const float* b, const float* w2,
                       const float* b2, float* y, int M, int D, float eps, void* stream);
int actmi_op_maxpool3x3s2(const float* in_nhwc, float* out_nhwc, int nimg, int H, int W, int C, void* stream);
int actmi_op_conv1(const void* image, int image_fmt, const float* w_oihw, const float* scale, const float* bias,
                   float* out, float* workspace , int B, int C, int H, int W, int Cout,
                   int prec , void* stream);
int64_t actmi_op_conv1_workspace_floats(int C, int Cout);
int actmi_op_conv1_prepare(const float* w_oihw, float* workspace, int C, int Cout, int lut_mode, void* stream);
int actmi_op_conv1_prepared(const void* image_u8, const float* workspace, const float* scale, const float* bias, float* out,
                            int B, int C, int H, int W, int Cout, int relu, void* stream);
int actmi_op_conv3x3_c64(const float* x, const float* w16, float w_scale, const float* scale, const float* bias,
                         const float* res, float* out, int G, int B, int H, int W, int relu, void* stream);
int actmi_op_wgrad3x3_c64(const float* dy, const float* x, float* dw, float* ws, int64_t ws_floats, const float* dy_scale_dev, int G,
                          int B, int H, int W, void* stream);

int actmi_op_wgrad7x7s2(const float* dy, const float* x4, float* dw, float* ws, int64_t ws_floats, const float* dy_scale_dev, int G,
                        int B, int H, int W, void* stream);

int actmi_op_groupnorm(const float* x, const float* res, const float* film_scale, const float* film_bias, const float* w,
                       const float* b, float* out, int n, int P, int C, int G, float eps, int act, int res_mode, float* ws,
                       int64_t ws_floats, void* stream);
int actmi_op_spatial_softmax(const float* logits, float* out, int n, int H, int W, int K, float temperature, void* stream);
int actmi_op_unfold1d(const float* x, float* out, int B, int T, int C, int k, int stride, int pad, int To, int transposed,
                      void* stream);
int actmi_op_ddim_step(float* x, const float* eps, int64_t n, float inv_sqrt_at, float sqrt_1m_at, float sqrt_aprev,
                       float sqrt_1m_aprev, int clip, void* stream);
int actmi_op_mish(const float* x, float* y, int64_t n, void* stream);
int actmi_op_u8_to_nhwc4(const uint8_t* image, float* out, int B, int Cam, int H, int W, void* stream);
int actmi_op_gelu(const float* x, float* y, int64_t n, void* stream);
int actmi_op_gelu_bwd(const float* x, const float* dy, float* dx, int64_t n, void* stream);
int actmi_op_dropout(const float* x, float* y, int64_t n, float p, uint64_t seed, void* stream);
int actmi_op_small_attention(const float* qkv, float* out, int n, int T, int H, int HD, int causal, float drop_p, uint64_t seed,
                             void* stream);
int actmi_op_small_attention_bwd(const float* qkv, const float* dout, float* dqkv, int n, int T, int H, int HD, int causal,
                                 float drop_p, uint64_t seed, void* stream);
int actmi_op_soft_ce_dim1(const float* logits, const float* target, int B, int T, int V, float* loss, float* dlogits, float* ws,
                          void* stream);
int actmi_op_argmax_l1(const float* logits, const float* target, int rows, int V, float* out, float* ws, void* stream);
int actmi_op_layernorm_bwd(const float* x, const float* w, const float* dy, const float* dx_add, float* dx, float* dw, float* db,
                           int M, int D, float eps, float* ws, int64_t ws_floats, void* stream);
int actmi_op_colsum(const float* src, int64_t ld, float* out, int M, int N, float* ws, int64_t ws_floats, void* stream);
int actmi_op_sum_batch(const float* src, int64_t batch_stride, int64_t ld, float* dst, int B, int R, int D, int accumulate,
                       void* stream);
int actmi_op_adamw(float* p, const float* g, float* m, float* v, int64_t n, float lr, float weight_decay, float beta1, float beta2,
                   float eps, int64_t step, void* stream);
const char* actmi_op_last_error(void);

int actmi_debug_tensor(actmi_handle h, const char* name, const float** dev_ptr, int64_t* numel);
int actmi_debug_stop_after(actmi_handle h, const char* stage);
int actmi_set_gemm_prec(actmi_handle h, int prec);
int actmi_set_train_prec(actmi_handle h, int prec);

#define ACTMI_FLAG_OUTPUT 1u
#define ACTMI_FLAG_WEIGHT 2u
#define ACTMI_FLAG_LOSS 4u
int actmi_get_flags(actmi_handle h, uint32_t* host_flags, int clear, void* stream);
int actmi_flags_ptr(actmi_handle h, void** dev_ptr);

int actmi_profile_enable(int on);
int actmi_profile_reset(void);
int actmi_profile_report(char* buf, int buflen);

#ifdef __cplusplus
}
#endif
#endif
```

Before: 1828 policy steps/s.

## Pre-split K/V into fp16 hi/lo in the GEMM epilogue and transpose-read V in attention

The QKV and cross-attention KV projection GEMMs can now write K and V in a pre-split fp16 hi/lo layout per head (c_split_hd), so the f16x3 attention kernel no longer splits K/V while staging them. A new attention variant (kv_fmt=1, HD=64) loads the pre-split tiles with plain vector copies into LDS and reads V with ds_read_tr16_b64 transposing loads instead of building a transposed V tile. This removes per-tile fp32-to-fp16 split work and the scattered transpose stores from the attention inner loop. In exchange it adds template variants, forbids split-K on these GEMMs, and only applies to f16x3 with head dim 64.

```diff
diff --git a/act-plus-plus_amd/actmi/lib.py b/act-plus-plus_amd/actmi/lib.py
--- a/act-plus-plus_amd/actmi/lib.py
+++ b/act-plus-plus_amd/actmi/lib.py
@@ -44,6 +44,7 @@
         ("Ax", C.c_void_p), ("kx_begin", C.c_int32), ("Hx", C.c_int32), ("Wx", C.c_int32), ("Cx", C.c_int32),
         ("stride_x", C.c_int32), ("gAx", C.c_int64),
         ("A_alt", C.c_void_p), ("alt_ncols", C.c_int32), ("k_tap_inner", C.c_int32),
+        ("c_split_from", C.c_int32), ("c_split_hd", C.c_int32),
     ]
 
 
@@ -52,7 +53,7 @@
                 ("dq", C.c_void_p), ("dk", C.c_void_p), ("dv", C.c_void_p)] + \
                [(n, C.c_int64) for n in ("q_bs", "q_rs", "k_bs", "k_rs", "v_bs", "v_rs", "dq_bs", "dq_rs", "dk_bs", "dk_rs", "dv_bs", "dv_rs")] + \
                [("kpm", C.c_void_p), ("kpm_bs", C.c_int64)] + [(n, C.c_int32) for n in ("B", "H", "Nq", "Nk", "HD")] + \
-               [("drop_p", C.c_float), ("drop_seed", C.c_uint64), ("delta_ws", C.c_void_p), ("do_scale", C.c_void_p), ("amax_out", C.c_void_p)]
+               [("drop_p", C.c_float), ("drop_seed", C.c_uint64), ("delta_ws", C.c_void_p), ("do_scale", C.c_void_p), ("amax_out", C.c_void_p), ("kv_fmt", C.c_int32)]
 
 
 class AttnDesc(C.Structure):
@@ -65,6 +66,7 @@
         ("B", C.c_int32), ("H", C.c_int32), ("Nq", C.c_int32), ("Nk", C.c_int32), ("HD", C.c_int32),
         ("scale", C.c_float), ("ws", C.c_void_p), ("ws_floats", C.c_int64),
         ("drop_p", C.c_float), ("drop_seed", C.c_uint64), ("prec", C.c_int32), ("causal", C.c_int32),
+        ("kv_fmt", C.c_int32),
     ]
 
 
diff --git a/act-plus-plus_amd/actmi/ops.py b/act-plus-plus_amd/actmi/ops.py
--- a/act-plus-plus_amd/actmi/ops.py
+++ b/act-plus-plus_amd/actmi/ops.py
@@ -52,7 +52,7 @@
 
 def gemm(A, W, bias=None, scale=None, res=None, res_mod=0, relu=False, a_add=None, add_mod=0, add_ncols=0, rowmap=None,
          out=None, out_rows=None, drop_p=0.0, drop_seed=0, prec=None, w_split=False, a_scale=0.0, b_scale=0.0,
-         a_scale_dev=None, b_scale_dev=None, splitk=0):
+         a_scale_dev=None, b_scale_dev=None, splitk=0, c_split_from=0, c_split_hd=0):
     lib = L.load()
     M, K = A.shape
     N = W.shape[0]
@@ -72,6 +72,7 @@
         d.splitk, d.split_stride = int(splitk), M * N
         d.prec, d.b_split, d.b_scale = PREC[prec], 1 if w_split else 0, float(w_split) if w_split else float(b_scale)
         d.a_scale = float(a_scale)
+        d.c_split_from, d.c_split_hd = int(c_split_from), int(c_split_hd)
         L.check(lib.actmi_op_gemm(C.byref(d), L.current_stream_ptr()), None, "op_gemm")
         if out is None:
             out = torch.empty((M, N), dtype=torch.float32, device=A.device)
@@ -100,6 +101,7 @@
     d.a_scale = float(a_scale)
     d.a_scale_dev = a_scale_dev.data_ptr() if a_scale_dev is not None else None
     d.b_scale_dev = b_scale_dev.data_ptr() if b_scale_dev is not None else None
+    d.c_split_from, d.c_split_hd = int(c_split_from), int(c_split_hd)
     L.check(lib.actmi_op_gemm(C.byref(d), L.current_stream_ptr()), None, "op_gemm")
     return out
 
@@ -244,7 +246,7 @@
 
 
 def attention(q, k, v, nheads, kpm=None, q_shared=False, want_lse=False, split=True, drop_p=0.0, drop_seed=0, prec=None,
-              causal=False):
+              causal=False, kv_fmt=0):
     lib = L.load()
     B, Nk, D = k.shape
     Nq = q.shape[-2]
@@ -267,11 +269,13 @@
     d.drop_p, d.drop_seed = float(drop_p), int(drop_seed)
     d.prec = PREC[prec]
     d.causal = 1 if causal else 0
+    d.kv_fmt = int(kv_fmt)
     L.check(lib.actmi_op_attention(C.byref(d), L.current_stream_ptr()), None, "op_attention")
     return (out, lse) if want_lse else out
 
 
-def attention_bwd(q, k, v, out, lse, dout, nheads, kpm=None, drop_p=0.0, drop_seed=0, do_scale=None, want_amax=False):
+def attention_bwd(q, k, v, out, lse, dout, nheads, kpm=None, drop_p=0.0, drop_seed=0, do_scale=None, want_amax=False,
+                  kv_fmt=0):
     lib = L.load()
     B, Nk, D = k.shape
     Nq = q.shape[1]
@@ -295,6 +299,7 @@
     d.delta_ws = ws.data_ptr()
     d.do_scale = do_scale.data_ptr() if do_scale is not None else None
     d.amax_out = amax.data_ptr() if amax is not None else None
+    d.kv_fmt = int(kv_fmt)
     L.check(lib.actmi_op_attention_bwd(C.byref(d), L.current_stream_ptr()), None, "op_attention_bwd")
     return (dq, dk, dv, amax) if want_amax else (dq, dk, dv)
 
diff --git a/act-plus-plus_amd/csrc/attn.hip b/act-plus-plus_amd/csrc/attn.hip
--- a/act-plus-plus_amd/csrc/attn.hip
+++ b/act-plus-plus_amd/csrc/attn.hip
@@ -9,6 +9,9 @@
 constexpr bool ATTN_NOPF = true;
 constexpr int KT = 64;
 typedef _Float16 h16x8 __attribute__((ext_vector_type(8)));
+typedef __fp16 tr_h16x4 __attribute__((__vector_size__(4 * sizeof(__fp16))));
+typedef __attribute__((address_space(3))) tr_h16x4 lds_h16x4;
+struct tr_pair { tr_h16x4 a, b; };
 
 __device__ __forceinline__ void attn_block_coords(int& bx, int& by, int& bz) {
     const int gx = gridDim.x, gy = gridDim.y;
@@ -206,15 +209,17 @@
     }
 }
 
-template <int HD>
+template <int HD, int KVS = 0>
 __global__ __launch_bounds__(256, 3) void attn_f16x3_kernel(AttnArgs p, int nsplit, int chunk) {
+    static_assert(!KVS || HD == 64, "the pre-split K / V loader is built for HD = 64");
     constexpr int NS = HD / 16;
     constexpr int DT = (HD + 31) / 32;
     constexpr int VD = DT * 32;
     constexpr int KROW = 4 * HD + 16;
     constexpr int VROW = 4 * KT + 16;
+    constexpr int VSROW = 4 * HD + 64;
     __shared__ __attribute__((aligned(16))) unsigned char s_k[KT * KROW];
-    __shared__ __attribute__((aligned(16))) unsigned char s_vt[VD * VROW];
+    __shared__ __attribute__((aligned(16))) unsigned char s_vt[KVS ? KT * VSROW : VD * VROW];
     __shared__ uint8_t s_dead[KT];
 
     const int t = threadIdx.x, lane = t & 63, wave = t >> 6;
@@ -262,10 +267,16 @@
     constexpr int NLK = (KT * C4 + 255) / 256;
     constexpr int NLV = (KT / 2 * C4 + 255) / 256;
     f32x4 pk[NLK], pv[NLV][2];
+    static_assert(!KVS || NLK == 2 * NLV, "the K and V copies of the pre-split loader share one item numbering");
     auto vc = [&](int e) { return ((e >> 5) % (C4 / 4)) * 4 + (e & 3); };
     auto vkp = [&](int e) { return ((e >> 5) / (C4 / 4)) * 8 + ((e >> 2) & 7); };
+    constexpr int RPP = 256 / C4;
+    static_assert(!KVS || (256 % C4 == 0 && KT * C4 == NLK * 256), "the pre-split loader covers the tile in whole passes");
+    const uint32_t koff = (uint32_t)(t / C4) * (uint32_t)p.k_rs + (t % C4) * 4;
+    const uint32_t voff = (uint32_t)(t / C4) * (uint32_t)p.v_rs + (t % C4) * 4;
     auto fetch = [&](int kt0) {
         const f32x4 z = {0.f, 0.f, 0.f, 0.f};
+        if constexpr (!KVS) {
 #pragma unroll
         for (int i = 0; i < NLK; ++i) {
             const int e = t + 256 * i;
@@ -275,6 +286,28 @@
             const f32x4 kv = *reinterpret_cast<const f32x4*>(Kb + (ok ? (int64_t)key * p.k_rs + c * 4 : 0));
             pk[i] = ok ? kv : z;
         }
+        }
+        if constexpr (KVS) {
+            const float* Kt = Kb + (int64_t)kt0 * p.k_rs;
+            const float* Vt = Vb + (int64_t)kt0 * p.v_rs;
+            if (kt0 + KT <= k_end) {
+#pragma unroll
+                for (int i = 0; i < NLK; ++i) {
+                    pk[i] = *reinterpret_cast<const f32x4*>(Kt + (int64_t)(i * RPP) * p.k_rs + koff);
+                    pv[i >> 1][i & 1] = *reinterpret_cast<const f32x4*>(Vt + (int64_t)(i * RPP) * p.v_rs + voff);
+                }
+            } else {
+#pragma unroll
+                for (int i = 0; i < NLK; ++i) {
+                    const bool ok = kt0 + t / C4 + i * RPP < k_end;
+                    const f32x4 kv = *reinterpret_cast<const f32x4*>(ok ? Kt + (int64_t)(i * RPP) * p.k_rs + koff : Kb);
+                    const f32x4 vv = *reinterpret_cast<const f32x4*>(ok ? Vt + (int64_t)(i * RPP) * p.v_rs + voff : Vb);
+                    pk[i] = ok ? kv : z;
+                    pv[i >> 1][i & 1] = ok ? vv : z;
+                }
+            }
+            return;
+        }
 #pragma unroll
         for (int i = 0; i < NLV; ++i) {
             const int e = t + 256 * i;
@@ -291,8 +324,16 @@
     if (!ATTN_NOPF) fetch(k_begin);
     for (int kt0 = k_begin; kt0 < k_end; kt0 += KT) {
         if (ATTN_NOPF) fetch(kt0);
-#pragma unroll
-        for (int i = 0; i < NLK; ++i) {
+        if constexpr (KVS) {
+#pragma unroll
+            for (int i = 0; i < NLK; ++i) {
+                const int kr = t / C4 + i * RPP, c = t % C4;
+                *reinterpret_cast<f32x4*>(s_k + kr * KROW + c * 16) = pk[i];
+                *reinterpret_cast<f32x4*>(s_vt + kr * VSROW + c * 16) = pv[i >> 1][i & 1];
+            }
+        }
+#pragma unroll
+        for (int i = 0; i < (KVS ? 0 : NLK); ++i) {
             const int e = t + 256 * i;
             if (e < KT * C4) {
                 const int kr = e / C4, c = e - kr * C4;
@@ -303,7 +344,7 @@
             }
         }
 #pragma unroll
-        for (int i = 0; i < NLV; ++i) {
+        for (int i = 0; i < (KVS ? 0 : NLV); ++i) {
             const int e = t + 256 * i;
             if (e < KT / 2 * C4) {
                 const int kp = vkp(e), c = vc(e);
@@ -399,8 +440,21 @@
                     const unsigned char* vrow = s_vt + (d * 32 + li) * VROW + sub * 64 + lh * 16;
 #pragma unroll
                     for (int g2 = 0; g2 < 2; ++g2) {
-                        const h16x8 vh = __builtin_bit_cast(h16x8, *reinterpret_cast<const f32x4*>(vrow + g2 * 32));
-                        const h16x8 vl = __builtin_bit_cast(h16x8, *reinterpret_cast<const f32x4*>(vrow + 2 * KT + g2 * 32));
+                        h16x8 vh, vl;
+                        if constexpr (KVS) {
+                            const lds_h16x4* vblk = reinterpret_cast<const lds_h16x4*>(
+                                (const __attribute__((address_space(3))) unsigned char*)s_vt +
+                                (sub * 32 + g2 * 16 + 4 * lh + ((lane >> 2) & 3)) * VSROW + (d * 32 + (lane & 16) + 4 * (lane & 3)) * 2);
+                            const tr_h16x4 h0 = __builtin_amdgcn_ds_read_tr16_b64_v4f16(const_cast<lds_h16x4*>(vblk));
+                            const tr_h16x4 h1 = __builtin_amdgcn_ds_read_tr16_b64_v4f16(const_cast<lds_h16x4*>(vblk + 8 * VSROW / 8));
+                            const tr_h16x4 l0 = __builtin_amdgcn_ds_read_tr16_b64_v4f16(const_cast<lds_h16x4*>(vblk + 2 * HD / 8));
+                            const tr_h16x4 l1 = __builtin_amdgcn_ds_read_tr16_b64_v4f16(const_cast<lds_h16x4*>(vblk + (8 * VSROW + 2 * HD) / 8));
+                            vh = __builtin_bit_cast(h16x8, tr_pair{h0, h1});
+                            vl = __builtin_bit_cast(h16x8, tr_pair{l0, l1});
+                        } else {
+                            vh = __builtin_bit_cast(h16x8, *reinterpret_cast<const f32x4*>(vrow + g2 * 32));
+                            vl = __builtin_bit_cast(h16x8, *reinterpret_cast<const f32x4*>(vrow + 2 * KT + g2 * 32));
+                        }
                         O[d] = __builtin_amdgcn_mfma_f32_32x32x16_f16(vl, ph[g2], O[d], 0, 0, 0);
                         O[d] = __builtin_amdgcn_mfma_f32_32x32x16_f16(vh, pl[g2], O[d], 0, 0, 0);
                         O[d] = __builtin_amdgcn_mfma_f32_32x32x16_f16(vh, ph[g2], O[d], 0, 0, 0);
@@ -488,6 +542,12 @@
     const int prec = a.prec ? a.prec : env_prec;
     if (prec != ACTMI_PREC_F32 && prec != ACTMI_PREC_F16X3) return fail("bad prec");
     const bool f16 = prec == ACTMI_PREC_F16X3;
+    if (a.kv_fmt != 0) {
+        if (a.kv_fmt != 1) return fail("bad kv_fmt");
+        if (!f16) return fail("kv_fmt 1 (pre-split K / V) needs prec f16x3");
+        if (a.HD != 64) return fail("kv_fmt 1 (pre-split K / V) needs head_dim 64");
+        if (a.k_rs < 0 || a.v_rs < 0 || a.k_rs >= (1 << 26) || a.v_rs >= (1 << 26)) return fail("kv_fmt 1: K / V row strides must be in [0, 2^26)");
+    }
     const int qblocks = (a.Nq + 127) / 128;
     const int tiles = (a.Nk + KT - 1) / KT;
     int nsplit = 1;
@@ -510,7 +570,10 @@
     }
     if (f16) {
         switch (a.HD) {
-            case 64: hipLaunchKernelGGL(attn_f16x3_kernel<64>, grid, dim3(256), 0, st, a, nsplit, chunk); break;
+            case 64:
+                if (a.kv_fmt) hipLaunchKernelGGL((attn_f16x3_kernel<64, 1>), grid, dim3(256), 0, st, a, nsplit, chunk);
+                else hipLaunchKernelGGL(attn_f16x3_kernel<64>, grid, dim3(256), 0, st, a, nsplit, chunk);
+                break;
             case 32: hipLaunchKernelGGL(attn_f16x3_kernel<32>, grid, dim3(256), 0, st, a, nsplit, chunk); break;
             case 16: hipLaunchKernelGGL(attn_f16x3_kernel<16>, grid, dim3(256), 0, st, a, nsplit, chunk); break;
             default: return fail("head_dim must be 16, 32 or 64");
diff --git a/act-plus-plus_amd/csrc/capi.hip b/act-plus-plus_amd/csrc/capi.hip
--- a/act-plus-plus_amd/csrc/capi.hip
+++ b/act-plus-plus_amd/csrc/capi.hip
@@ -272,6 +272,7 @@
 int actmi_op_attention_bwd(const actmi_attn_bwd_desc* d, void* stream) {
     g_op_error.clear();
     if (!d || !d->o || !d->delta_ws) { g_op_error = "attention_bwd: null descriptor / output / scratch"; return ACTMI_E_INVALID; }
+    if (d->kv_fmt != 0) { g_op_error = "attention_bwd: K and V must be fp32 (kv_fmt is a forward-only form)"; return ACTMI_E_INVALID; }
     AttnBwdArgs a{};
     a.Q = d->q; a.K = d->k; a.V = d->v; a.dO = d->d_o; a.lse = d->lse; a.dO_scale = d->do_scale;
     a.dQ = d->dq; a.dK = d->dk; a.dV = d->dv;
diff --git a/act-plus-plus_amd/csrc/engine.hip b/act-plus-plus_amd/csrc/engine.hip
--- a/act-plus-plus_amd/csrc/engine.hip
+++ b/act-plus-plus_amd/csrc/engine.hip
@@ -153,7 +153,8 @@
     constexpr int sk_target = 1536, sk_minnk = 12, sk_maxtiles = 768;
     constexpr int sk_target_long = 4864, sk_maxtiles_long = 1300, sk_long_nk = 128;
     if (ctx->fwd_splitk && ctx->splitk_ws && a.splitk <= 1 && a.tb == 0 && a.ta == 0 && (a.mode == 0 || a.mode == 1) &&
-        !a.rowmap && !a.C2 && !a.mask && a.drop_p == 0.f && a.res_mod == 0 && a.groups_inner == 0 && !a.stamps) {
+        !a.rowmap && !a.C2 && !a.mask && a.drop_p == 0.f && a.res_mod == 0 && a.groups_inner == 0 && !a.stamps &&
+        a.c_split_hd == 0 ) {
         const int groups = a.groups > 0 ? a.groups : 1;
         const int64_t tiles = (int64_t)((a.M + 63) / 64) * ((a.N + 63) / 64) * groups * (ws_half >= 0 ? ctx->policy_mult : 1);
         const int nk = (a.K + 31) / 32;
@@ -955,15 +956,17 @@
 }
 
 int engine_encoder_layer(actmi_ctx* ctx, const EncW& w, const TView& V, const float* pos, int B, int n, const uint8_t* kpm,
-                         hipStream_t st, bool xp_in, bool xp_out) {
+                         hipStream_t st, bool xp_in, bool xp_out, bool kv_split) {
     float* x = V.X;
     const actmi_config& g = ctx->cfg;
     const int D = g.hidden_dim, F = g.dim_feedforward, M = B * n;
     GemmArgs qkv = linear_args(x, D, M, D, w.attn.in_w, 3 * D, w.attn.in_b, V.QKV, 3 * D);
     if (xp_in) { qkv.A_alt = V.XP; qkv.alt_ncols = 2 * D; }
     else { qkv.A_add = pos; qkv.ld_add = D; qkv.add_mod = n; qkv.add_ncols = 2 * D; }
+    if (kv_split) { qkv.c_split_from = D; qkv.c_split_hd = D / g.nheads; }
     CHK(ctx_gemm(ctx, qkv, st, V.half));
     AttnArgs at = packed_self_attn_args(ctx, V.QKV, V.ATT, B, n);
+    at.kv_fmt = kv_split ? 1 : 0;
     at.kpm = kpm;
     at.ws = V.attn_ws; at.ws_floats = V.attn_ws_floats;
     at.prec = ctx->gemm_prec;
@@ -988,7 +991,7 @@
     return 0;
 }
 
-int engine_decoder_infer(actmi_ctx* ctx, const TView& V, int B, float* a_hat, hipStream_t st, bool xp_in) {
+int engine_decoder_infer(actmi_ctx* ctx, const TView& V, int B, float* a_hat, hipStream_t st, bool xp_in, bool kv_split) {
     const actmi_config& g = ctx->cfg;
     const int D = g.hidden_dim, F = g.dim_feedforward, Q = g.num_queries, N = ctx->N;
     const DecW& d = ctx->dec[0];
@@ -996,8 +999,10 @@
     GemmArgs kv = linear_args(V.X, D, B * N, D, d.cross.in_w + (int64_t)D * D, 2 * D, d.cross.in_b + D, KV, 2 * D);
     if (xp_in) { kv.A_alt = V.XP; kv.alt_ncols = D; }
     else { kv.A_add = ctx->pos_tokens; kv.ld_add = D; kv.add_mod = N; kv.add_ncols = D; }
+    if (kv_split) { kv.c_split_from = 0; kv.c_split_hd = D / g.nheads; }
     CHK(ctx_gemm(ctx, kv, st, V.half));
     AttnArgs at = cross_attn_args(ctx, ctx->dec_q, false, KV, V.dO, B);
+    at.kv_fmt = kv_split ? 1 : 0;
     at.ws = V.attn_ws; at.ws_floats = V.attn_ws_floats;
     at.prec = ctx->gemm_prec;
     CHK(launch_attention(at, st, &ctx->err));
@@ -1069,10 +1074,11 @@
     auto run_transformer = [&](int b0, int nb, hipStream_t ts, int half) -> int {
         const TView V = make_view(ctx, b0, nb, half);
         const bool xp_qkv = ((2 * D) % 128) == 0, xp_kv = (D % 128) == 0;
+        const bool kv_split = ctx->gemm_prec == ACTMI_PREC_F16X3 && xp_kv && D / g.nheads == 64;
         for (int l = 0; l < g.enc_layers; ++l)
             CHK(engine_encoder_layer(ctx, ctx->enc[l], V, ctx->pos_tokens, nb, N, nullptr, ts, l > 0 && xp_qkv,
-                                     l + 1 < g.enc_layers ? xp_qkv : xp_kv));
-        return engine_decoder_infer(ctx, V, nb, a_hat + (int64_t)b0 * g.num_queries * g.action_dim, ts, xp_kv);
+                                     l + 1 < g.enc_layers ? xp_qkv : xp_kv, kv_split));
+        return engine_decoder_infer(ctx, V, nb, a_hat + (int64_t)b0 * g.num_queries * g.action_dim, ts, xp_kv, kv_split);
     };
     const bool tpipe = ctx->cam_pipe && ctx->pipe_stream && B >= 2 && !prof_enabled() && ctx->stop_stage.empty();
     ctx->dbg["memory"] = {ctx->X, (int64_t)B * N * D};
diff --git a/act-plus-plus_amd/csrc/gemm.hip b/act-plus-plus_amd/csrc/gemm.hip
--- a/act-plus-plus_amd/csrc/gemm.hip
+++ b/act-plus-plus_amd/csrc/gemm.hip
@@ -39,7 +39,7 @@
 
 __device__ __forceinline__ f32x4 ld4(const float* p) { return *reinterpret_cast<const f32x4*>(p); }
 
-template <int BM, int BN, int WM, int WN, int AMODE, int BMODE, int PREC, int BSPLIT, int UNMASKED, int XS = 0>
+template <int BM, int BN, int WM, int WN, int AMODE, int BMODE, int PREC, int BSPLIT, int UNMASKED, int XS = 0, int CS = 0>
 __global__ __launch_bounds__((BM / WM) * (BN / WN) * 64, (PREC && BM * BN <= 128 * 64 && (AMODE == 0  || AMODE == 3 ) && !(AMODE == 0 && BMODE == 1)) ? 3 : 2)
     void gemm_f32_kernel(GemmArgs p, int tiles_m, int tiles_n) {
     constexpr int NT = (BM / WM) * (BN / WN) * 64;
@@ -720,6 +720,8 @@
             const f32x4 one4 = {1.f, 1.f, 1.f, 1.f};
             const f32x4 sc4 = scale ? ld4(scale + ncol) : one4;
             const f32x4 bi4 = bias ? ld4(bias + ncol) : zero4;
+            const int shd = (CS && n0 >= p.c_split_from) ? p.c_split_hd : 0;
+            const int sd = ncol & (shd - 1);
 #pragma unroll
             for (int i = 0; i < TM; ++i) {
 #pragma unroll
@@ -757,7 +759,14 @@
 #pragma unroll
                             for (int e = 0; e < 4; ++e) v[e] = 0.5f * v[e] * (1.f + erff(v[e] * 0.70710678118654752f));
                         }
-                        *reinterpret_cast<f32x4*>(C + (uint32_t)(m * (int)p.ldc + ncol)) = v;
+                        if (CS && shd != 0) {
+                            uint2 hi, lo;
+                            split16(v, hi, lo);
+                            unsigned char* hb = reinterpret_cast<unsigned char*>(C + (uint32_t)(m * (int)p.ldc + ncol - sd)) + 2 * sd;
+                            *reinterpret_cast<uint2*>(hb) = hi;
+                            *reinterpret_cast<uint2*>(hb + 2 * shd) = lo;
+                        } else
+                            *reinterpret_cast<f32x4*>(C + (uint32_t)(m * (int)p.ldc + ncol)) = v;
                         if (track) {
 #pragma unroll
                             for (int e = 0; e < 4; ++e) amx = max(amx, __float_as_uint(v[e]) & 0x7fffffffu);
@@ -864,12 +873,12 @@
     if (stamp && threadIdx.x == 0) stamp[3] = __builtin_amdgcn_s_memtime();
 }
 
-template <int BM, int BN, int WM, int WN, int AMODE, int BMODE, int PREC, int BSPLIT, int UNMASKED, int XS = 0>
+template <int BM, int BN, int WM, int WN, int AMODE, int BMODE, int PREC, int BSPLIT, int UNMASKED, int XS = 0, int CS = 0>
 int launch_cfg_u(const GemmArgs& a, hipStream_t st) {
     const int tiles_m = (a.M + BM - 1) / BM, tiles_n = (a.N + BN - 1) / BN;
     static const int lds_pad = getenv("ACTMI_GEMM_LDSPAD") ? atoi(getenv("ACTMI_GEMM_LDSPAD")) : 0;
     const int smem = 2 * stage_f4<BM, BN, PREC>() * 16 + lds_pad;
-    auto kern = gemm_f32_kernel<BM, BN, WM, WN, AMODE, BMODE, PREC, BSPLIT, UNMASKED, XS>;
+    auto kern = gemm_f32_kernel<BM, BN, WM, WN, AMODE, BMODE, PREC, BSPLIT, UNMASKED, XS, CS>;
     static bool attr_set = false;
     if (!attr_set) {
         hipError_t e = hipFuncSetAttribute(reinterpret_cast<const void*>(kern),
@@ -884,9 +893,9 @@
         static const bool by_shape = getenv("ACTMI_PROF_SHAPES") && getenv("ACTMI_PROF_SHAPES")[0] == '1';
         if (by_shape)
             snprintf(nm, sizeof(nm), "gemm_%s_kernel<%d,%d,%d,%d,%d,%d%s>[M=%d,N=%d,K=%d,g=%d,sk=%d,wgs=%d]", PREC == PREC_BF16 ? "bf16" : PREC ? "f16x3" : "f32",
-                     BM, BN, WM, WN, AMODE, BMODE, XS ? ",xs" : "", a.M, a.N, a.K, a.groups, splitk, tiles_m * tiles_n * a.groups * splitk);
+                     BM, BN, WM, WN, AMODE, BMODE, XS ? ",xs" : CS ? ",cs" : "", a.M, a.N, a.K, a.groups, splitk, tiles_m * tiles_n * a.groups * splitk);
         else
-            snprintf(nm, sizeof(nm), "gemm_%s_kernel<%d,%d,%d,%d,%d,%d%s>", PREC == PREC_BF16 ? "bf16" : PREC ? "f16x3" : "f32", BM, BN, WM, WN, AMODE, BMODE, XS ? ",xs" : "");
+            snprintf(nm, sizeof(nm), "gemm_%s_kernel<%d,%d,%d,%d,%d,%d%s>", PREC == PREC_BF16 ? "bf16" : PREC ? "f16x3" : "f32", BM, BN, WM, WN, AMODE, BMODE, XS ? ",xs" : CS ? ",cs" : "");
         const double g = a.groups;
         double abytes;
         if (AMODE == A_CONV) abytes = (double)(a.M / (a.Ho * a.Wo)) * a.H * a.W * a.Cin + (XS ? (double)a.M * a.Cx : 0.0);
@@ -903,12 +912,19 @@
 template <int BM, int BN, int WM, int WN, int AMODE, int BMODE, int PREC, int BSPLIT>
 int launch_cfg_b(const GemmArgs& a, hipStream_t st) {
     constexpr bool HOT = PREC != PREC_F32 && BMODE == B_N && (AMODE == A_N || AMODE == A_NADD || AMODE == A_CONV);
+    constexpr bool CAN_CS = PREC == PREC_F16X3 && BSPLIT == 1 && BMODE == B_N && (AMODE == A_N || AMODE == A_NADD);
+    if (a.c_split_hd && !CAN_CS) return -1003;
     if constexpr (HOT) {
         const bool one_a = (a.a_scale == 0.f || a.a_scale == 1.f) && !a.a_scale_dev;
         const bool one_b = BSPLIT || ((a.b_scale == 0.f || a.b_scale == 1.f) && !a.b_scale_dev);
         const bool unmasked_ok = (a.K % BK) == 0 && one_a && one_b && a.epi == 0 && !a.amax_out && !a.finite_flag;
         if constexpr (AMODE == A_CONV && BSPLIT == 1) {
             if (a.Ax) return unmasked_ok ? launch_cfg_u<BM, BN, WM, WN, AMODE, BMODE, PREC, BSPLIT, 1, 1>(a, st) : -1001;
+        }
+        if constexpr (CAN_CS) {
+            if (a.c_split_hd)
+                return unmasked_ok ? launch_cfg_u<BM, BN, WM, WN, AMODE, BMODE, PREC, BSPLIT, 1, 0, 1>(a, st)
+                                   : launch_cfg_u<BM, BN, WM, WN, AMODE, BMODE, PREC, BSPLIT, 0, 0, 1>(a, st);
         }
         if (unmasked_ok) return launch_cfg_u<BM, BN, WM, WN, AMODE, BMODE, PREC, BSPLIT, 1>(a, st);
     }
@@ -1020,6 +1036,19 @@
     if (a.relu == 2 && (a.rowmap || a.C2 || a.drop_p > 0.f || a.res_mod != 0)) return fail("GELU is only available in the plain epilogue");
     if (a.relu < 0 || a.relu > 2) return fail("bad activation");
     if (a.C2 && !a.scale2) return fail("C2 needs scale2");
+    if (a.c_split_hd != 0) {
+        const int hd = a.c_split_hd;
+        if (hd < 16 || hd > 128 || (hd & (hd - 1))) return fail("c_split_hd must be a power of two in 16..128");
+        if (a.c_split_from < 0 || (a.c_split_from % 128) || (a.N % 128) || a.c_split_from >= a.N)
+            return fail("c_split_from and N must be multiples of 128, c_split_from < N");
+        if (a.splitk > 1) return fail("the split output form does not combine with split-K (the combine pass writes fp32)");
+        if (a.rowmap || a.C2 || a.res || a.mask || a.epi != 0 || a.drop_p > 0.f || a.res_mod != 0)
+            return fail("the split output form needs the plain epilogue (scale / bias / activation only)");
+        if ((a.ldc & 3) || ((uintptr_t)a.C & 15) || (a.gC & 3) || (a.gC2 & 3) || (int64_t)a.M * a.ldc >= ((int64_t)1 << 31))
+            return fail("the split output form needs a 16-byte aligned C, ldc % 4 == 0 and M * ldc < 2^31");
+        if (((uintptr_t)a.scale & 15) || ((uintptr_t)a.bias & 15) || (a.gSB & 3))
+            return fail("the split output form needs 16-byte aligned scale / bias");
+    }
     int amode, bmode = a.tb;
     if (a.ta) {
         if (a.mode != 0) return fail("ta requires mode 0");
@@ -1087,6 +1116,7 @@
         if (rc == -1002) return fail("operand form combination not instantiated");
     } else if (prec == ACTMI_PREC_F16X3) { ACTMI_DISPATCH(PREC_F16X3) } else { ACTMI_DISPATCH(PREC_F32) }
 #undef ACTMI_DISPATCH
+    if (rc == -1003) return fail("the split output form (c_split_hd) needs prec f16x3, pre-split weights (b_split) and row-major A (mode 0, ta 0)");
     if (rc == -1001) return fail("a second source (Ax) needs prec f16x3, pre-split weights (b_split), K % 32 == 0 and a plain epilogue");
     if (rc != 0 && err) *err = std::string("gemm launch: ") + hipGetErrorString((hipError_t)rc);
     return rc == 0 ? 0 : -3;
diff --git a/include/actmi.h b/include/actmi.h
--- a/include/actmi.h
+++ b/include/actmi.h
@@ -105,6 +105,7 @@
     const float* A_alt;
     int32_t alt_ncols;
     int32_t k_tap_inner;
+    int32_t c_split_from, c_split_hd;
 } actmi_gemm_desc;
 
 typedef struct actmi_attn_desc {
@@ -122,6 +123,7 @@
     uint64_t drop_seed;
     int32_t prec;
     int32_t causal;
+    int32_t kv_fmt;
 } actmi_attn_desc;
 
 int actmi_version(void);
@@ -187,6 +189,7 @@
     float* delta_ws;
     const float* do_scale;
     uint32_t* amax_out;
+    int32_t kv_fmt;
 } actmi_attn_bwd_desc;
 int actmi_op_attention_bwd(const actmi_attn_bwd_desc* d, void* stream);
 int actmi_op_layernorm(const float* x, const float* res, int res_mod, const float* w, const float* b, const float* w2,
```

After: 1838 policy steps/s, median of 6. Within noise of the previous version (+0.5%).
